# lujiarui/Str2Str

Hardware: AMD Instinct MI355X
Metric: sampled conformations/sec (whole node), 256-res chain, 100 denoise steps (higher is better)
Workload: dtype f32 (matrix products on 2-way f16 split MFMA 'f16x3': 3 products per block, fp32 accumulate, fp32-equivalent); 1 GPU; configs[1]: single 256-residue synthetic chain, 128 replicas per GPU x 100 denoise steps (+1 self-conditioning forward), probability-flow ODE, seeded synthetic weights; n_res=256, replicas_per_gpu=128, denoise_steps=100, parallelism=replica-shard x1, arith=f16x3, rng=device

## Files before the change

### include/str2str_hip.h

```cpp
#ifndef STR2STR_HIP_H
#define STR2STR_HIP_H

#ifdef __cplusplus
extern "C" {
#endif

int s2s_abi_version(void);



int s2s_edge_transition(const float* edge, const float* node_ab, const float* node_p, const float* w1_packed,
                        const float* w2_packed, const float* wf_packed, const float* b2, const float* bf,
                        const float* ln_gamma, const float* ln_beta, const float* mask, float* out, int n_samples,
                        int n_res, float ln_eps, const float* proj_w_packed, const float* proj_bias_cat64,
                        float* proj_attn_bias, float* proj_pair_z, void* stream);

int s2s_edge_transition_f16x3(const float* edge, const float* node_ab, const float* node_p, const void* weight_stream,
                              const float* b2, const float* ln_gamma, const float* ln_beta,
                              const float* mask, float* out, int n_samples, int n_res, float ln_eps, int io_layout,
                              const float* proj_bias_cat64, float* proj_attn_bias, float* proj_pair_z, int prescale_exp,
                              int* range_words, void* stream);

int s2s_edge_embed(const float* node_a, const float* node_b, const float* rel_table, const float* bin_table,
                   const float* bin_lower, const long long* residue_idx, const float* ca_xyz, const float* w2_packed,
                   const float* w3_packed, const float* b2, const float* b3, const float* ln_gamma, const float* ln_beta,
                   const float* mask, float* out, int n_samples, int n_res, int rel_offset, int n_rel, int n_bins,
                   float ln_eps, const float* proj_w_packed, const float* proj_bias_cat64, float* proj_attn_bias,
                   float* proj_pair_z, void* stream);

int s2s_edge_embed_f16x3(const float* node_a, const float* node_b, const float* rel_table, const float* bin_table,
                         const float* bin_lower, const long long* residue_idx, const float* ca_xyz,
                         const void* weight_stream, const float* b2, const float* b3, const float* ln_gamma,
                         const float* ln_beta, const float* mask, float* out, int n_samples, int n_res, int rel_offset,
                         int n_rel, int n_bins, float ln_eps, int out_tiled, const float* proj_bias_cat64,
                         float* proj_attn_bias, float* proj_pair_z, int* range_words, void* stream);

int s2s_pair_project(const float* edge, const float* w_packed, const float* bias_cat64, float* attn_bias, float* pair_z,
                     int n_samples, int n_res, void* stream);


int s2s_ipa_prep_points(const float* rigids7, const float* q_pts_lin, const float* kv_pts_lin, float* q_pts, float* k_pts,
                        float* v_pts, long long n_frames, int n_heads, int n_qk_points, int n_v_points, int v_pts_stride,
                        void* stream);

int s2s_ipa_attention(const float* q, const float* kv, const float* q_pts, const float* k_pts, const float* v_pts64,
                      const float* attn_bias, float* logits_out, float* stats_out, const float* mask, const float* rigids7,
                      const float* head_w_scaled, float* out, int n_samples, int n_res, int n_heads, int c_hidden,
                      int n_qk_points, int n_v_points, int c_pair_z, float inf, float eps, void* stream);

int s2s_ipa_prep_points_f16(const float* rigids7, const float* q_pts_lin, const float* kv_pts_lin, const float* head_w_scaled,
                            void* qp_xp, void* kp_xp, void* vp_vf, float* q2, float* k2, int n_samples, int n_res, int n_heads,
                            int n_qk_points, int n_v_points, int c_hidden, const void* s_xp, void* k_shared, void* v_shared,
                            int* range_words, void* stream);
int s2s_ipa_attention_f16w(const void* q_xp, const void* k_xp, const void* v_vf, const void* qp_xp, const void* kp_xp,
                             const void* vp_vf, const float* q2, const float* k2, const float* attn_bias, float* logits_out,
                             float* stats_out, const float* mask, const float* rigids7, float* out, void* out_xp,
                             int out_xp_ksteps, int n_samples, int n_res, int n_heads, int c_hidden, int n_qk_points,
                             int n_v_points, int c_pair_z, float inf, float eps, int n_kv_heads, void* stream);

int s2s_ipa_opair(const float* logits, const float* stats, const float* pair_z, float* out, int n_samples, int n_res,
                  int n_heads, int c_pair_z, int out_row_stride, int out_col_offset, int logits_ld, void* stream);


int s2s_rigid_compose_update(const float* rigids7, const float* update6, const float* mask, float* out7,
                             long long n_frames, int update_ld, void* stream);

int s2s_torsion_head(const float* u, int u_ld, int normalize, const float* gt_sin_cos, long long gt_row_stride, const float* fixed_mask,
                     float eps, float* out2, long long n_rows, void* stream);

int s2s_rigid_scale_trans(const float* rigids7, float* out7, long long n_frames, float scale, int divide, void* stream);

int s2s_set_backbone_tables(const float* pos_21x5x3, const float* mask_21x5, const int* is_psi_group_21x5,
                            const float* default_frames_21x2x4x4);

int s2s_frames_to_backbone(const float* rigids7, const float* psi_sincos, const long long* aatype, float* atom14_bb5,
                           float* atom37, long long n_frames, void* stream);


int s2s_se3_step(const float* x0_7, const float* xt_7, const float* mask, const float* diffuse_mask,
                 const float* params8, const double* z_rot, const double* z_trans,
                 const double* rot_score_in, const double* trans_score_in, float* next7,
                 double* rot_score_out, double* trans_score_out, int n_samples, int n_res, double dt,
                 const double* dt_per_sample, double coordinate_scaling, int probability_flow, int center_trans,
                 double noise_scale, void* stream);

int s2s_embed_assemble(const float* t_img, long long t_img_rows, const float* node_const, long long node_const_rows, const float* fa, const float* fb,
                       long long n_rows, int n_res, void* h_xp, float* h_f32, float* node_a, float* node_b, int b_col_blocked,
                       int* range_words, void* stream);


int s2s_pack_planes(const float* x, long long n_rows, int ld, int col0, int n_cols, void* xp, int xp_ksteps, int xp_kstep0,
                    const float* row_scale, int* range_words, void* stream);

int s2s_node_linear(const void* xp, const void* w_packed, const float* bias, long long n_rows, int k_in, int n_out,
                    int tiles_per_block, const float* pre_scale, int relu, const float* pre_mask, const float* residual,
                    int residual_ld, const float* ln_gamma, const float* ln_beta, float ln_eps, const float* post_mask,
                    float* out_f32, int out_ld, int out_col0, void* out_xp, int out_xp_ksteps, int out_xp_kstep0,
                    int map_pad, int map_src, int* range_words, void* stream);

int s2s_node_linear_f32(const float* x, int x_ld, const float* w_packed, const float* bias, long long n_rows, int k_in, int n_out,
                        int tiles_per_block, const float* pre_scale, int relu, const float* pre_mask, const float* residual,
                        int residual_ld, const float* ln_gamma, const float* ln_beta, float ln_eps, const float* post_mask,
                        float* out_f32, int out_ld, int out_col0, void* stream);

int s2s_node_linear_vfrag(const void* xp, const void* w_packed, const float* bias, long long n_rows, int k_in, int n_out,
                          int tiles_per_head, void* out_vf, int map_pad, int map_src, int* range_words, void* stream);

typedef struct s2s_node_problem {
    const void* xp; const void* w_packed; const float* bias;
    long long n_rows; int k_in, n_out, tiles_per_block;
    int vfrag_tiles_per_head;
    float* out_f32; int out_ld, out_col0;
    void* out_xp; int out_xp_ksteps, out_xp_kstep0;
    void* out_vf;
    int map_pad, map_src, relu;
    const float* pre_scale;
} s2s_node_problem;
int s2s_node_linear_multi(const s2s_node_problem* problems, int n_problems, int* range_words, void* stream);

typedef struct s2s_chain_layer { const void* w_packed; const float* bias; int relu; } s2s_chain_layer;
int s2s_node_chain(const void* xp, const s2s_chain_layer* layers, int n_layers, long long n_rows, int width, int k_in0,
                   const float* mid_residual, int mid_residual_ld, float* mid_out_f32, int mid_out_ld, const float* mid_ln_gamma,
                   const float* mid_ln_beta, float mid_ln_eps, const float* pre_mask, const float* residual, int residual_ld, const float* ln_gamma, const float* ln_beta, float ln_eps,
                   const float* post_mask, float* out_f32, int out_ld, int out_col0, void* out_xp, int out_xp_ksteps,
                   int out_xp_kstep0, int* range_words, void* stream);

int s2s_row_layernorm(const float* x, int x_ld, long long n_rows, int n_cols, const float* ln_gamma, const float* ln_beta, float ln_eps,
                      const float* post_mask, float* out_f32, int out_ld, int out_col0, void* out_xp, int out_xp_ksteps,
                      int out_xp_kstep0, int* range_words, void* stream);

int s2s_encoder_attention(const float* qkv, const float* key_bias, float* out_f32, void* out_xp, int n_samples, int n_res,
                          int n_heads, int head_dim, int* range_words, void* stream);

int s2s_encoder_attention_f16x3(const float* qkv, const float* key_bias, float* out_f32, void* out_xp, int n_samples, int n_res,
                          int n_heads, int head_dim, int* range_words, void* stream);


int s2s_forward_marginal(const float* rigids0_4x4, const float* z_axis, const float* u01, const float* z_trans,
                         const double* cdf_rows, const int* cdf_row_of_sample, const float* omega_grid, int n_omega,
                         const float* params2, const float* diffuse_mask, float coordinate_scaling, float* rigids_t7,
                         int n_samples, int n_res, void* stream);


int s2s_ca_sample_stats(const float* ca, int n_samples, int n_res, float clash_bar, int k_exclusion, int* n_clash,
                        float* adjacent_max, double* radius_of_gyration, void* stream);

int s2s_ca_pairwise_distances(const float* ca, int n_samples, int n_res, int offset, float* out, void* stream);

int s2s_ca_pwd_js(const float* ref_ca, int n_ref, const float* pred_ca, int n_pred, int n_res, int offset, int n_bins,
                  double pseudo_count, double* js_per_channel, const double* ref_weights, const double* pred_weights, void* stream);


int s2s_ca_rmsd_matrix(const float* a, int n_a, const float* b, int n_b, int n_res, const float* weights, double* rmsd,
                       double* workspace, long long workspace_doubles, void* stream);

int s2s_ca_superpose(const float* mobile, int n_mobile, const float* target, int n_res, const float* weights, double* rmsd,
                     double* xform, void* stream);

int s2s_apply_xform(const float* points, const double* xform, int n_samples, long long n_points, float* out, void* stream);

#define S2S_TM_MAX_RES 800

int s2s_ca_tm_matrix(const float* a, int n_a, const float* b, int n_b, int n_res, double d0, double* tm, void* stream);

int s2s_ca_tm_superpose(const float* mobile, int n_mobile, const float* target, int n_res, double d0, double* tm, double* xform12,
                        void* stream);

#define S2S_LDDT_MAX_RES 1024
#define S2S_LDDT_LIST_SLOTS(n_res) (((long long)(n_res) * ((long long)(n_res) - 1) / 2 + 1) / 2 * 2)
#define S2S_LDDT_WORKSPACE_BYTES(n_a, n_res) ((long long)(n_a) * (12 * S2S_LDDT_LIST_SLOTS(n_res) + 8 + 4 * (long long)(n_res)))

int s2s_ca_lddt_matrix(const float* a, int n_a, const float* b, int n_b, int n_res, double cutoff, int min_seq_sep, double* lddt,
                       void* workspace, long long workspace_bytes, void* stream);

int s2s_ca_lddt_per_residue(const float* model, int n_model, const float* target, int n_res, double cutoff, int min_seq_sep,
                            double* per_res, double* total, void* workspace, long long workspace_bytes, void* stream);

#define S2S_VIOL_MAX_RES 1024

int s2s_backbone_violations(const float* atoms, int n, int n_res, const unsigned char* atom_exists, const int* aatype,
                            const int* residue_index, double tolerance_factor, double clash_tolerance, double* losses, double* fractions,
                            double* per_residue_loss, unsigned char* bond_mask, unsigned char* clash_atom_mask, int* n_clash_pairs,
                            void* stream);

#define S2S_SS_MAX_RES 704

int s2s_secondary_structure(const float* atoms, int n, int n_res, const int* aatype, const int* residue_index, unsigned char* ss,
                            int* n_hbonds, double* hb_energy, int* hb_partner, double* torsions, void* stream);

#define S2S_CLUSTER_MAX_N 65536

int s2s_cluster_adjacency(const double* values, int n_rows, int row0, int n, double cutoff, int at_least, unsigned long long* adj,
                          int* deg, void* stream);

int s2s_cluster_gromos(const unsigned long long* adj, int* deg, int n, int init, int n_rounds, int* labels, int* centres, int* sizes,
                       int* state, unsigned long long* live_ws, unsigned long long* members_ws, void* stream);

#define S2S_CONTACT_MAX_RES 1024
#define S2S_CONTACT_MAX_STRUCTURES 65535
#define S2S_CONTACT_LIST_SLOTS(n_res) ((long long)(n_res) > 1 ? (long long)(n_res) * ((long long)(n_res) - 1) / 2 : 1)

int s2s_ca_contact_map(const float* ca, int n, int n_res, double cutoff, int min_seq_sep, const double* weights, int* counts,
                       double* weighted, void* stream);

int s2s_ca_contact_stats(const float* ca, int n, int n_res, double cutoff, int min_seq_sep, int* n_contacts, long long* sep_sum,
                         void* stream);

int s2s_ca_native_contacts(const float* native, int n_res, double cutoff, int min_seq_sep, int* pairs, double* d0, int* n_pairs,
                           void* stream);

int s2s_ca_native_q(const float* ca, int n, int n_res, const int* pairs, const double* d0, int n_pairs, double beta, double lam,
                    double* q_soft, double* q_hard, int* hits, void* stream);

#define S2S_SASA_MAX_RES 512
#define S2S_SASA_MAX_POINTS 1024

int s2s_backbone_sasa(const float* atoms, int n, int n_res, const unsigned char* atom_exists, const double* radii, double probe,
                      const double* sphere, int n_points, int* counts, double* per_residue, double* total, void* stream);

#define S2S_SAXS_MAX_RES 1024
#define S2S_SAXS_MAX_Q 1024
#define S2S_SAXS_MAX_TYPES 64

int s2s_ca_scattering(const float* ca, int n, int n_res, const double* q, int n_q, const int* types, const double* table, int n_types,
                      double* intensity, double* inv_r_mean, void* stream);

#define S2S_PCA_MAX_RES 1024
#define S2S_PCA_WORKSPACE_DOUBLES(n_res, chunk) ((3ll * (n_res) + 47) / 48 * 48 * (((long long)(chunk) + 3) / 4 * 4))

int s2s_ca_aligned_mean(const float* x, int n, int n_res, const double* xform, const double* p, double* mean, void* stream);

int s2s_ca_covariance(const float* x, int n, int n_res, const double* xform, const double* p, const double* mean, double* cov,
                      double* workspace, long long workspace_doubles, void* stream);

int s2s_ca_project(const float* x, int n, int n_res, const double* xform, const double* mean, const double* components, int n_components,
                   double* proj, void* stream);


long long s2s_format_pdb_models(const float* atom37, int n_models, int n_res, const long long* aatype,
                                const long long* residue_index, const long long* chain_index, const double* b_factors,
                                int first_model_number, int add_end, char* out, long long out_capacity);

long long s2s_write_pdb_models(const char* path, int append, const float* atom37, int n_models, int n_res,
                               const long long* aatype, const long long* residue_index, const long long* chain_index,
                               const double* b_factors, int first_model_number, int add_end);

long long s2s_merge_pdb_files(const char* const* paths, int n_paths, const char* out_path);

int s2s_mt19937_discard(unsigned long long* state624, int* left, unsigned long long* next, unsigned long long n_outputs);

#ifdef __cplusplus
}
#endif
#endif
```

### str2str_amd/build.py

```python
from __future__ import annotations

import os
import shutil
import subprocess
import sys
from concurrent.futures import ThreadPoolExecutor

HERE = os.path.dirname(os.path.abspath(__file__))
ROOT = os.path.dirname(HERE)
CSRC = os.path.join(HERE, "csrc")
OBJ = os.path.join(CSRC, "build")
LIB = os.path.join(HERE, "libstr2str_hip.so")

ARCH = "gfx950"
COMMON = ["-O3", "-std=c++17", "-fPIC", f"--offload-arch={ARCH}", "-I", os.path.join(ROOT, "include"), "-I", CSRC,
          "-Wno-unused-result"]
UNITS = {
    "abi.hip": [],
    "pdb_format.cpp": [],
    "host_rng.cpp": [],
    "rigid_kernels.hip": ["-ffp-contract=off"],
    "se3_step.hip": ["-ffp-contract=off"],
    "forward_marginal.hip": ["-ffp-contract=off"],
    "ensemble_metrics.hip": ["-ffp-contract=off"],
    "ensemble_rmsd.hip": [],
    "ensemble_tm.hip": [],
    "ensemble_pca.hip": [],
    "ensemble_cluster.hip": [],
    "ensemble_lddt.hip": [],
    "ensemble_contacts.hip": ["-ffp-contract=off"],
    "ensemble_violations.hip": ["-ffp-contract=off"],
    "ensemble_ss.hip": ["-ffp-contract=off"],
    "ensemble_sasa.hip": ["-ffp-contract=off"],
    "ensemble_saxs.hip": ["-ffp-contract=off"],
    "pair_mlp.hip": ["-mllvm", "-pragma-unroll-threshold=10000000"],
    "pair_mlp_f16.hip": ["-mllvm", "-pragma-unroll-threshold=10000000", "-fno-slp-vectorize"],
    "pair_mlp_f16_b.hip": ["-mllvm", "-pragma-unroll-threshold=10000000", "-fno-slp-vectorize"],
    "pair_mlp_f16_c.hip": ["-mllvm", "-pragma-unroll-threshold=10000000", "-fno-slp-vectorize"],
    "ipa_attention.hip": ["-mllvm", "-pragma-unroll-threshold=10000000"],
    "ipa_attention_f16w.hip": ["-mllvm", "-pragma-unroll-threshold=10000000", "-fno-slp-vectorize"],
    "node_gemm.hip": ["-mllvm", "-pragma-unroll-threshold=10000000", "-fno-slp-vectorize"],
    "enc_attention.hip": ["-mllvm", "-pragma-unroll-threshold=10000000", "-ffp-contract=off", "-fno-slp-vectorize"],
}


def hipcc() -> str:
    for c in (os.environ.get("HIPCC"), shutil.which("hipcc"), "/opt/rocm/bin/hipcc"):
        if c and os.path.exists(c):
            return c
    raise RuntimeError("hipcc not found (set HIPCC)")


def _stale(out: str, deps) -> bool:
    if not os.path.exists(out):
        return True
    t = os.path.getmtime(out)
    return any(os.path.getmtime(d) > t for d in deps)


def build(force: bool = False, verbose: bool = True) -> str:
    os.makedirs(OBJ, exist_ok=True)
    cc = hipcc()
    headers = [os.path.join(CSRC, f) for f in os.listdir(CSRC) if f.endswith(".h")] + [
        os.path.join(ROOT, "include", "str2str_hip.h"), os.path.abspath(__file__)]

    def compile_one(item):
        src, extra = item
        s = os.path.join(CSRC, src)
        o = os.path.join(OBJ, os.path.splitext(src)[0] + ".o")
        inc = [os.path.join(CSRC, "pair_mlp_f16.hip")] if src.startswith("pair_mlp_f16_") else []
        if force or _stale(o, [s] + inc + headers):
            if src.endswith(".cpp"):
                cmd = [cc, "-x", "c++", "-c", s, "-o", o] + [c for c in COMMON if not c.startswith("--offload-arch")] + extra
            else:
                cmd = [cc, "-x", "hip", "-c", s, "-o", o] + COMMON + extra
            if verbose:
                print(" ".join(cmd), flush=True)
            subprocess.run(cmd, check=True)
        return o

    with ThreadPoolExecutor(max_workers=min(8, len(UNITS))) as ex:
        objs = list(ex.map(compile_one, UNITS.items()))
    for f in os.listdir(OBJ):
        if f.endswith(".o") and os.path.join(OBJ, f) not in objs:
            os.remove(os.path.join(OBJ, f))
    if force or _stale(LIB, objs):
        cmd = [cc, "-shared", "-fPIC", f"--offload-arch={ARCH}", "-o", LIB] + objs
        if verbose:
            print(" ".join(cmd), flush=True)
        subprocess.run(cmd, check=True)
    return LIB


if __name__ == "__main__":
    print(build(force="--force" in sys.argv))
```

### str2str_amd/csrc/pair_mlp_f16.hip

```cpp
#include <hip/hip_runtime.h>

#include <cstdlib>

#include "f16x3.h"
#include "range_flag.h"
#include "str2str_hip.h"

#ifndef S2S_PM_PART
#define S2S_PM_PART 1
#endif

namespace {

constexpr int kStageBytes = 32 * 1024;
constexpr int kStagesBase = 30;

__device__ __forceinline__ float relu1(float x) {
    float r;
    asm("v_max_f32 %0, 0, %1" : "=v"(r) : "v"(x));
    return r;
}

struct SlotDesc { int phase, t, a, b; };
constexpr SlotDesc slot_desc(int s) {
    if (s < 8) return {0, s / 4, s % 4, 0};
    if (s < 168) {
        const int tau = s - 8, blk = tau / 16, o = tau % 16;
        if (o < 12) return {1, blk, o / 6, o % 6};
        return {0, blk + 2, o - 12, 0};
    }
    if (s < 180) return {1, 10, (s - 168) / 6, (s - 168) % 6};
    if (s < 192) return {1, 11, (s - 180) % 2, (s - 180) / 2};

    if (s < 240) return {2, 0, (s - 192) / 2, (s - 192) % 2};
    return {3, 0, s - 240, 0};
}
constexpr int sched_slot(bool proj, int ns) { return !proj ? ns : (ns < 8 ? ns : (ns < 16 ? 240 + (ns - 8) : ns - 8)); }
constexpr int blob_stage(bool proj, int st) { return !proj ? st : (st == 0 ? 0 : (st == 1 ? 30 : st - 1)); }

#define S2S_LDS_BARRIER() asm volatile("s_waitcnt lgkmcnt(0)\n\ts_barrier" ::: "memory")
__device__ float s2s_one[1] = {1.0f};


template <bool PROJ, bool STAGE>
__global__ void __launch_bounds__(256) edge_transition_f16_kernel(
    const float* __restrict__ edge, const float* __restrict__ node_ab, const float* __restrict__ node_p,
    const char* __restrict__ wblob, const float* __restrict__ b2,
    const float* __restrict__ gamma, const float* __restrict__ beta, const float* __restrict__ mask,
    float* __restrict__ out, long long M, int N, float ln_eps, int io_layout, unsigned mask_stride, const float* __restrict__ proj_b,
    float* __restrict__ proj_bias_out, float* __restrict__ proj_pz_out, int* __restrict__ range_flag, float sk) {
    constexpr int kStages = kStagesBase + (PROJ ? 1 : 0);
    constexpr int kSlots = 8 * kStages;
    constexpr int kRing = PROJ ? 4 : 2, kAhead = PROJ ? 2 : 1;
    __shared__ __attribute__((aligned(16))) char s_w[kRing][kStageBytes];
    __shared__ __attribute__((aligned(16))) float s_vec[768 + 64];
    __shared__ __attribute__((aligned(16))) float s_rows[STAGE ? 4 * 2 * 384 : 4];
    const int lane = threadIdx.x & 63, h = lane >> 5, wave = threadIdx.x >> 6;

    const unsigned voff = wave * 8192 + lane * 16;
    typedef __attribute__((address_space(3))) char lds_char;
    lds_char* lds_image[2] = {(lds_char*)&s_w[0][lane * 16], (lds_char*)&s_w[kRing / 2][lane * 16]};
    asm volatile("" : "+v"(lds_image[0]), "+v"(lds_image[1]));
    auto ring_buf = [&](int r) -> lds_char* { return PROJ ? lds_image[r >> 1] + (r & 1) * kStageBytes : lds_image[r]; };
    const __amdgpu_buffer_rsrc_t wrsrc = __builtin_amdgcn_make_buffer_rsrc((void*)wblob, 0, kStages * kStageBytes, 0x00020000);
    auto ldw = [&](unsigned vo, int so) -> f32x4 {
        const u32x4 r = __builtin_amdgcn_raw_buffer_load_b128(wrsrc, vo, so, 0);
        return f32x4{__uint_as_float(r.x), __uint_as_float(r.y), __uint_as_float(r.z), __uint_as_float(r.w)};
    };
    f32x4 c0, c1, c2, c3;
    f32x4 e0, e1, e2, e3;
    typedef __attribute__((address_space(3))) f32x4 lds_f4;
    auto cp_load_a = [&](int stage) {
        const int so = blob_stage(PROJ, stage) * kStageBytes;
        c0 = ldw(voff, so); c1 = ldw(voff + 1024, so); c2 = ldw(voff + 2048, so); c3 = ldw(voff + 3072, so);
    };
    auto cp_load_b = [&](int stage) {
        const int so = blob_stage(PROJ, stage) * kStageBytes + 4096;
        e0 = ldw(voff, so); e1 = ldw(voff + 1024, so); e2 = ldw(voff + 2048, so); e3 = ldw(voff + 3072, so);
    };
    auto cp_store_a = [&](int par) {
        lds_char* d = ring_buf(par) + wave * 8192;
        *(lds_f4*)(d) = c0; *(lds_f4*)(d + 1024) = c1; *(lds_f4*)(d + 2048) = c2; *(lds_f4*)(d + 3072) = c3;
    };
    auto cp_store_b = [&](int par) {
        lds_char* d = ring_buf(par) + (wave * 8192 + 4096);
        *(lds_f4*)(d) = e0; *(lds_f4*)(d + 1024) = e1; *(lds_f4*)(d + 2048) = e2; *(lds_f4*)(d + 3072) = e3;
    };
    auto cp_load_piece = [&](auto grp, auto kc, int stage) {
        constexpr int k = decltype(kc)::value;
        const int so = blob_stage(PROJ, stage) * kStageBytes + (decltype(grp)::value ? 4096 : 0);
        const f32x4 v = ldw(voff + 1024 * k, so);
        if constexpr (decltype(grp)::value == 0) {
            if constexpr (k == 0) c0 = v; else if constexpr (k == 1) c1 = v; else if constexpr (k == 2) c2 = v; else c3 = v;
        } else {
            if constexpr (k == 0) e0 = v; else if constexpr (k == 1) e1 = v; else if constexpr (k == 2) e2 = v; else e3 = v;
        }
    };
    auto cp_store_piece = [&](auto grp, auto kc, int par) {
        constexpr int k = decltype(kc)::value;
        lds_char* d = ring_buf(par) + (wave * 8192 + (decltype(grp)::value ? 4096 : 0) + 1024 * k);
        if constexpr (decltype(grp)::value == 0)
            *(lds_f4*)(d) = k == 0 ? c0 : (k == 1 ? c1 : (k == 2 ? c2 : c3));
        else
            *(lds_f4*)(d) = k == 0 ? e0 : (k == 1 ? e1 : (k == 2 ? e2 : e3));
    };
    cp_load_a(0);
    cp_load_b(0);

    struct PairCtx {
        unsigned p, bi, bj, boff;
        unsigned r0, aoff;
        float em_i, em_j;
        bool valid;
    };
    const unsigned NNu = (unsigned)N * (unsigned)N;
    const long long NN = (long long)N * N;
    const unsigned n_magic = N >= 2 ? (unsigned)((1ull << 32) / (unsigned)N) : 0u;
    auto div_n = [&](unsigned x, unsigned& q, unsigned& r) {
        q = N >= 2 ? __umulhi(x, n_magic) : x;
        r = x - q * (unsigned)N;
        const bool fix = r >= (unsigned)N;
        q = fix ? q + 1 : q;
        r = fix ? r - (unsigned)N : r;
    };
    auto setup = [&](long long wg_tile) -> PairCtx {
        long long pl = (wg_tile * 4 + wave) * 32 + (lane & 31);
        PairCtx c;
        c.valid = pl < M;
        if (!c.valid) pl = M - 1;
        const unsigned p = (unsigned)pl;
        unsigned bi, j, bb, i;
        div_n(p, bi, j);
        div_n(bi, bb, i);
        c.p = p;
        c.bi = bi;
        c.bj = bb * (unsigned)N + j;
        c.r0 = (unsigned)__builtin_amdgcn_readfirstlane((int)bi);
        c.aoff = (unsigned)wave * 3072u + (bi != c.r0 ? 1536u : 0u) + 16u * (unsigned)h;
        c.boff = p + 7u * bb * NNu;
        c.em_i = mask[bi * mask_stride];
        c.em_j = mask[c.bj * mask_stride];
        return c;
    };
    const bool in_tiled = io_layout & 1, out_tiled = io_layout & 2, no_out = io_layout & 4;
    const int in_step = in_tiled ? 256 : 8, out_step = out_tiled ? 256 : 8;
    auto row_of = [&](const float* base, unsigned p, bool tiled) -> const float* {
        const unsigned blk = tiled ? p >> 5 : p, mul = tiled ? 4096u : 128u;
        const unsigned in_blk = tiled ? ((lane & 32) + (p & 31)) * 4 : 4 * h;
        return base + ((unsigned long long)blk * mul + in_blk);
    };
    auto erow_of = [&](const PairCtx& c) -> const float* { return row_of(edge, c.p, in_tiled); };
    auto ldrow = [&](const float* r, int g) -> float4 {
        const f32x4 v = __builtin_nontemporal_load(reinterpret_cast<const f32x4*>(r + g * in_step));
        return make_float4(v.x, v.y, v.z, v.w);
    };
    const long long n_wt = (M + 127) / 128;
    long long wt = blockIdx.x;
    PairCtx cur = setup(wt);

    f16x8 xpl[8][2];
    float amax = 0.f;
    const float inv1 = kInvWS * sk;
    auto split4 = [&](const float (&x)[4], f16x8& ph, f16x8& pm, int at) {
        split4_f16(x, ph, pm, at, amax);
    };
    {
        float4 xv[16];
#pragma unroll
        for (int i = 0; i < 16; ++i) xv[i] = ldrow(erow_of(cur), i);
        for (int i = threadIdx.x; i < 768; i += 256)
            s_vec[i] = i < 384 ? sk * b2[i] : (i < 512 ? 0.f : (i < 640 ? gamma[i - 512] : beta[i - 640]));
        if (PROJ && threadIdx.x < 64) s_vec[768 + threadIdx.x] = proj_b[threadIdx.x];
        cp_store_a(0);
        cp_load_a(1);
        cp_store_b(0);
        if constexpr (kAhead == 2) {
            cp_load_b(1);
            cp_store_a(1);
            cp_load_a(2);
            cp_store_b(1);
        }
#pragma unroll
        for (int i = 0; i < 16; ++i) {
            const float x[4] = {xv[i].x, xv[i].y, xv[i].z, xv[i].w};
            split4(x, xpl[i >> 1][0], xpl[i >> 1][1], 4 * (i & 1));
        }
    }

    f32x16 a1t[2];
    f32x16 a2[12];
    f32x16 a3[4];
    f32x16 pq[2];
    float sa[16];
    f32x4 g_st0, g_st1, g_st2;
    const unsigned n_node_rows = (unsigned)(M / N);
    auto stage_load = [&](const PairCtx& c) {
        if constexpr (STAGE) {
            const unsigned r1 = c.r0 + 1 < n_node_rows ? c.r0 + 1 : c.r0;
            auto piece = [&](int k) -> f32x4 {
                const unsigned o = (unsigned)k * 1024u + 16u * (unsigned)lane;
                const bool second = o >= 1536u;
                const float* src = node_ab + (unsigned long long)(second ? r1 : c.r0) * 896u + ((second ? o - 1536u : o) >> 2);
                const float4 v = *reinterpret_cast<const float4*>(src);
                return f32x4{v.x, v.y, v.z, v.w};
            };
            g_st0 = piece(0); g_st1 = piece(1); g_st2 = piece(2);
        }
    };
    auto stage_store = [&]() {
        if constexpr (STAGE) {
            typedef __attribute__((address_space(3))) f32x4 lds_v4;
            lds_v4* d = (lds_v4*)((__attribute__((address_space(3))) char*)s_rows + wave * 3072 + lane * 16);
            d[0] = g_st0; d[64] = g_st1; d[128] = g_st2;
        }
    };
    auto seeds_piece = [&](const PairCtx& c, int t, int rq) {
        if constexpr (STAGE) {
            const f32x4 x = *(const lds_f4*)((__attribute__((address_space(3))) const char*)s_rows + c.aoff + (32 * t + 8 * rq) * 4);
            sa[4 * rq + 0] = x[0]; sa[4 * rq + 1] = x[1]; sa[4 * rq + 2] = x[2]; sa[4 * rq + 3] = x[3];
        } else {
            const float4 x = ldg4(node_ab + (unsigned long long)c.bi * 896u + 32 * t, rq, h);
            sa[4 * rq + 0] = x.x; sa[4 * rq + 1] = x.y; sa[4 * rq + 2] = x.z; sa[4 * rq + 3] = x.w;
        }
    };
    auto seedc_piece = [&](const PairCtx& c, int t, int rq) {
        const float4 y = ldg4(node_ab + (unsigned long long)c.bj * 896u + 384 + 32 * t, rq, h);
        a1t[t & 1][4 * rq + 0] = y.x; a1t[t & 1][4 * rq + 1] = y.y; a1t[t & 1][4 * rq + 2] = y.z; a1t[t & 1][4 * rq + 3] = y.w;
    };
    auto seeds_load = [&](const PairCtx& c, int t) {
#pragma unroll
        for (int rq = 0; rq < 4; ++rq) seeds_piece(c, t, rq);
    };
    stage_load(cur);
    stage_store();
    seeds_load(cur, 0);
#pragma unroll
    for (int rq = 0; rq < 4; ++rq) { seedc_piece(cur, 0, rq); seedc_piece(cur, 1, rq); }

    f16x8 fr[2][4];
    f16x8 xp[2][2];
    auto fetch = [&](int par, int slot_in_stage, f16x8 (&f)[4]) {
        typedef __attribute__((address_space(3))) f16x8 lds_frag;
        const lds_frag* s = (const lds_frag*)ring_buf(par) + slot_in_stage * 4 * 64;
        f[0] = s[0]; f[2] = s[128]; f[3] = s[192]; f[1] = s[64];
    };
    auto s_quarter = [&](const f32x16& tile_acc, auto qc) {
        constexpr int qd = decltype(qc)::value;
        float x[4];
#pragma unroll
        for (int j = 0; j < 4; ++j) x[j] = fmaxf(__builtin_fmaf(tile_acc[4 * qd + j], inv1, sa[4 * qd + j]), 0.f);
        split4(x, xp[qd >> 1][0], xp[qd >> 1][1], 4 * (qd & 1));
    };
    auto s_half = [&](const f32x16& tile_acc, auto qc, auto hc) {
        constexpr int qd = decltype(qc)::value, j0 = 4 * qd + 2 * decltype(hc)::value;
        const float x0 = fmaxf(__builtin_fmaf(tile_acc[j0], inv1, sa[j0]), 0.f);
        const float x1 = fmaxf(__builtin_fmaf(tile_acc[j0 + 1], inv1, sa[j0 + 1]), 0.f);
        split2_f16(x0, x1, xp[qd >> 1][0], xp[qd >> 1][1], 4 * (qd & 1) + 2 * decltype(hc)::value, amax);
    };
    float rs[64];
    auto row_load2 = [&](const float* r, float (&dst)[64], int g0) {
#pragma unroll
        for (int g = g0; g < g0 + 2; ++g) {
            const float4 v = ldg4(r, g, h);
            dst[4 * g + 0] = v.x; dst[4 * g + 1] = v.y; dst[4 * g + 2] = v.z; dst[4 * g + 3] = v.w;
        }
    };
    const f32x16 zero16 = {0.f, 0.f, 0.f, 0.f, 0.f, 0.f, 0.f, 0.f, 0.f, 0.f, 0.f, 0.f, 0.f, 0.f, 0.f, 0.f};
    S2S_LDS_BARRIER();
    fetch(0, 0, fr[0]);

    PairCtx prv = cur;
    prv.valid = false;
    prv.em_i = 0.f;
    float ln_sum = 0.f, ln_var = 0.f, ln_mean = 0.f, ln_rstd = 0.f, ln_em = 0.f;
    float* ln_orow = out;
    f16x8 xln[8][2];
    auto ln_add = [&](auto qc) {
        constexpr int q = decltype(qc)::value, t = q / 4, rq = q % 4;
#pragma unroll
        for (int j = 0; j < 4; ++j) ln_sum += a3[t][4 * rq + j];
    };
    auto ln_dev = [&](auto qc) {
        constexpr int q = decltype(qc)::value, t = q / 4, rq = q % 4;
#pragma unroll
        for (int j = 0; j < 4; ++j) {
            const float dd = a3[t][4 * rq + j] - ln_mean;
            ln_var += dd * dd;
        }
    };
    auto ln_out = [&](auto qc, const float4& ga, const float4& be) {
        constexpr int q = decltype(qc)::value, t = q / 4, rq = q % 4;
        float4 o;
        o.x = ((a3[t][4 * rq + 0] - ln_mean) * ln_rstd * ga.x + be.x) * ln_em;
        o.y = ((a3[t][4 * rq + 1] - ln_mean) * ln_rstd * ga.y + be.y) * ln_em;
        o.z = ((a3[t][4 * rq + 2] - ln_mean) * ln_rstd * ga.z + be.z) * ln_em;
        o.w = ((a3[t][4 * rq + 3] - ln_mean) * ln_rstd * ga.w + be.w) * ln_em;
        if (prv.valid && !no_out) {
            __builtin_nontemporal_store(f32x4{o.x, o.y, o.z, o.w}, reinterpret_cast<f32x4*>(ln_orow + q * out_step));
        }
        if constexpr (PROJ) {
            const float x[4] = {o.x, o.y, o.z, o.w};
            split4(x, xln[2 * t + (rq >> 1)][0], xln[2 * t + (rq >> 1)][1], 4 * (rq & 1));
        }
    };
    auto proj_store = [&](auto gc) {
        constexpr int g = decltype(gc)::value;
        if (prv.valid) {
            const float4 bq = ldg4(s_vec + 768, g, h);
            if constexpr (g == 0) {
                float* o = proj_bias_out + ((unsigned long long)prv.boff + 4 * h * NN);
                o[0] = __builtin_fmaf(pq[0][0], kInvWS, bq.x);
                o[NN] = __builtin_fmaf(pq[0][1], kInvWS, bq.y);
                o[2 * NN] = __builtin_fmaf(pq[0][2], kInvWS, bq.z);
                o[3 * NN] = __builtin_fmaf(pq[0][3], kInvWS, bq.w);
            } else {
                constexpr int t = g >> 2, rq = g & 3;
                *reinterpret_cast<float4*>(proj_pz_out + (unsigned long long)prv.p * 32u + 8 * (g - 1) + 4 * h) =
                    make_float4(__builtin_fmaf(pq[t][4 * rq + 0], kInvWS, bq.x), __builtin_fmaf(pq[t][4 * rq + 1], kInvWS, bq.y),
                                __builtin_fmaf(pq[t][4 * rq + 2], kInvWS, bq.z), __builtin_fmaf(pq[t][4 * rq + 3], kInvWS, bq.w));
            }
        }
    };
#pragma unroll
    for (int t = 0; t < 4; ++t) a3[t] = zero16;

    constexpr int kHead = PROJ ? 16 : 15;
    long long wt_next = wt;
    bool has_next = false;
    PairCtx nxt = cur;
    float4 xv[16];
    f16x8 xpn[8][2];
    f16x8 xq[8][2];
    auto slot = [&](auto sc) {
        constexpr int ns = decltype(sc)::value;
        constexpr int s = sched_slot(PROJ, ns);
        constexpr SlotDesc d = slot_desc(s);
        constexpr int stage = ns / 8, ss = ns % 8, par = stage & (kRing - 1);
        constexpr int st_next = (stage + 1) % kStages, st_fill = (stage + kAhead) % kStages;
#ifdef S2S_ET_ALL_BARRIERS
        constexpr bool barrier_here = true;
#else
        constexpr bool barrier_here = !PROJ || (st_next & 1) == 0 || st_next == kStages - 2;
#endif

        if constexpr (ss < 7) {
            fetch(par, ss + 1, fr[(ns + 1) & 1]);
        } else {
            if constexpr (barrier_here) S2S_LDS_BARRIER();
            fetch(st_next & (kRing - 1), 0, fr[(ns + 1) & 1]);
        }
        constexpr int kXv0 = 208;
        if constexpr (s == kXv0) nxt = setup(has_next ? wt_next : wt);
        if constexpr (s == kXv0 + 3) stage_load(nxt);
        if constexpr (s == kXv0 + 8) stage_store();
        if constexpr (s > kXv0 && s <= kXv0 + 16 && ((s & 3) == 1 || (s & 3) == 2)) {
            constexpr int i = 4 * ((s - kXv0) / 4) + 2 * ((s & 3) - 1);
            const float* er = erow_of(nxt);
            xv[i] = ldrow(er, i);
            xv[i + 1] = ldrow(er, i + 1);
        }
        if constexpr (s == 236) seeds_load(nxt, 0);
        if constexpr (s == 237) { seedc_piece(nxt, 0, 0); seedc_piece(nxt, 0, 1); seedc_piece(nxt, 0, 2); seedc_piece(nxt, 0, 3); }
        if constexpr (s == 238) { seedc_piece(nxt, 1, 0); seedc_piece(nxt, 1, 1); seedc_piece(nxt, 1, 2); seedc_piece(nxt, 1, 3); }
        constexpr bool seeds_slot = d.phase == 1 && d.a == 1 && d.b == 0 && d.t + 1 < 12;
        if constexpr (s >= 184 && s < 192) row_load2(node_p + (unsigned long long)cur.bi * 128u, rs, 2 * (s - 184));
        constexpr int ep_blk = (s >= 184 && s < 192) ? 0 : ((s >= 192 && s < 224) ? 1 + (s - 192) / 16 : -1);
        constexpr int ep_q = ep_blk == 0 ? 2 * (s - 184) : (s - 192) % 16;
        float4 ep_b = {0.f, 0.f, 0.f, 0.f}, ep_b1 = {0.f, 0.f, 0.f, 0.f};
        if constexpr (ep_blk >= 0) ep_b = ldg4(s_vec + 128 * ep_blk, ep_q, h);
        if constexpr (ep_blk == 0) ep_b1 = ldg4(s_vec, ep_q + 1, h);
        constexpr int ln_k = ns == 7 ? 0 : ((PROJ && d.phase == 3 && d.a < 7) ? d.a + 1 : ((!PROJ && ns >= 8 && ns < 15) ? ns - 7 : -1));
        float4 lnv[4] = {};
        if constexpr (ln_k >= 0) {
#pragma unroll
            for (int k = 0; k < 2; ++k) { lnv[2 * k] = ldg4(s_vec + 512, 2 * ln_k + k, h); lnv[2 * k + 1] = ldg4(s_vec + 640, 2 * ln_k + k, h); }
        }
        constexpr int kGSlot = 182, kGPer = 2;
        if constexpr (s >= kGSlot && s < kGSlot + 16 / kGPer) {
#pragma unroll
            for (int u = 0; u < kGPer; ++u) {
                constexpr int p0 = (s - kGSlot) * kGPer;
                const int t3 = (p0 + u) / 4, rq = (p0 + u) % 4;
                const float4 v = ldg4(node_ab + (unsigned long long)cur.bj * 896u + 768 + 32 * t3, rq, h);
                a3[t3][4 * rq + 0] = v.x; a3[t3][4 * rq + 1] = v.y; a3[t3][4 * rq + 2] = v.z; a3[t3][4 * rq + 3] = v.w;
            }
        }
        __builtin_amdgcn_sched_barrier(0);

        const f16x8 (&f)[4] = fr[ns & 1];
        auto mfma_i = [&](auto ic) {
            constexpr int i = decltype(ic)::value;
            if constexpr (d.phase == 0) {
                f32x16& acc = a1t[d.t & 1];
                const f16x8 (&x)[2] = xpl[2 * d.a + (i >= 3)];
                constexpr int fa = (i == 0 ? 1 : (i < 3 ? 0 : (i == 3 ? 3 : 2))), xa = (i == 1 || i == 4) ? 1 : 0;
                acc = mfma_f16(f[fa], x[xa], acc);
            } else {
                constexpr bool fin = d.phase == 2, prj = d.phase == 3;
                constexpr bool first = i < 2 && (prj ? d.a == 0 : (fin ? false : (d.t == 0 && d.a == 0)));
                f32x16& t = prj ? pq[i & 1] : (fin ? a3[2 * d.b + (i & 1)] : a2[2 * d.b + (i & 1)]);
                const f16x8 (&x)[2] = prj ? xln[d.a] : (fin ? ((d.a >> 3) == 1 ? xq[d.a & 7] : xpl[d.a & 7]) : xp[d.a]);
                constexpr int fa = 2 * (i & 1) + (i < 2 ? 1 : 0), xa = (i == 2 || i == 3) ? 1 : 0;
                if constexpr (first) t = mfma_f16(f[fa], x[xa], zero16); else t = mfma_f16(f[fa], x[xa], t);
            }
        };
        auto ep_half = [&](auto qc, auto hc, const float4& bq) {
            constexpr int q = decltype(qc)::value, hh = decltype(hc)::value, t = q / 4, rq = q % 4, j0 = 4 * rq + 2 * hh, e0 = 4 * (rq & 1) + 2 * hh;
            const f32x16& a = a2[4 * (ep_blk < 0 ? 0 : ep_blk) + t];
            f16x8 (&P)[2] = ep_blk == 1 ? xq[2 * t + (rq >> 1)] : xpl[2 * t + (rq >> 1)];
            float r0 = 0.f, r1 = 0.f;
            if constexpr (ep_blk == 0) {
                const unsigned hw = __builtin_bit_cast(u32x4, P[0])[e0 / 2], lw = __builtin_bit_cast(u32x4, P[1])[e0 / 2];
                asm("v_fma_mix_f32 %0, %1, 1.0, %2 op_sel_hi:[1,0,1]" : "=v"(r0) : "v"(hw), "v"(lw));
                asm("v_fma_mix_f32 %0, %1, 1.0, %2 op_sel:[1,0,1] op_sel_hi:[1,0,1]" : "=v"(r1) : "v"(hw), "v"(lw));
            } else if constexpr (ep_blk == 1) {
                r0 = rs[16 * t + j0];
                r1 = rs[16 * t + j0 + 1];
            }
            float x0 = fmaxf(__builtin_fmaf(a[j0], kInvWS, hh ? bq.z : bq.x), 0.f), x1 = fmaxf(__builtin_fmaf(a[j0 + 1], kInvWS, hh ? bq.w : bq.y), 0.f);
            if constexpr (ep_blk != 2) {
                x0 = __builtin_fmaf(r0, sk, x0);
                x1 = __builtin_fmaf(r1, sk, x1);
            }
            split2_f16(x0, x1, P[0], P[1], e0, amax);
        };
        static_for<0, 6>([&](auto ic) {
            constexpr int i = decltype(ic)::value;
            mfma_i(ic);
            if constexpr (i < 4) {
                if constexpr (ss == 0) cp_load_piece(IC<1>{}, ic, st_fill);
                if constexpr (ss == 4) cp_load_piece(IC<0>{}, ic, (stage + kAhead + 1) % kStages);
                if constexpr (ss == 1) cp_store_piece(IC<0>{}, IC<3 - i>{}, st_fill & (kRing - 1));
                if constexpr (ss == 5) cp_store_piece(IC<1>{}, IC<3 - i>{}, st_fill & (kRing - 1));
            }
            if constexpr (seeds_slot && i < 4) seeds_piece(cur, d.t + 1, i);
            if constexpr (seeds_slot && i < 4 && d.t + 2 < 12) seedc_piece(cur, d.t + 2, i);
            if constexpr (d.phase == 0 && d.t >= 1 && (i == 2 || i == 4)) s_half(a1t[(d.t - 1) & 1], IC<d.a>{}, IC<(i - 2) / 2>{});
            if constexpr (ep_blk > 0 && (i == 2 || i == 4)) ep_half(IC<ep_q>{}, IC<(i - 2) / 2>{}, ep_b);
            if constexpr (ep_blk == 0 && i >= 1 && i <= 4) {
                if constexpr (i <= 2) ep_half(IC<ep_q>{}, IC<i - 1>{}, ep_b); else ep_half(IC<ep_q + 1>{}, IC<i - 3>{}, ep_b1);
            }
            if constexpr (s >= 228 && s < 236 && i >= 1 && i <= 4) {
                constexpr int k = s - 228, e = 2 * (i - 1);
                const float4 v = xv[2 * k + (e >> 2)];
                if constexpr ((e & 2) == 0) split2_f16(v.x, v.y, xpn[k][0], xpn[k][1], e, amax);
                else split2_f16(v.z, v.w, xpn[k][0], xpn[k][1], e, amax);
            }
            if constexpr (ns < 4 && i < 4) ln_add(IC<4 * ns + i>{});
            if constexpr (ns == 4 && i == 0) ln_mean = xhalf_sum(ln_sum) * (1.0f / 128);
            if constexpr ((ns == 4 || ns == 5) && (i == 1 || i == 3 || i == 5)) { ln_dev(IC<6 * (ns - 4) + i - 1>{}); ln_dev(IC<6 * (ns - 4) + i>{}); }
            if constexpr (ns == 6 && (i == 0 || i == 1)) { ln_dev(IC<12 + 2 * i>{}); ln_dev(IC<12 + 2 * i + 1>{}); }
            if constexpr (ns == 6 && i == 3) {
                ln_rstd = 1.0f / sqrtf(xhalf_sum(ln_var) * (1.0f / 128) + ln_eps * ((kWS * sk) * (kWS * sk)));
                ln_em = prv.em_i * prv.em_j;
                ln_orow = const_cast<float*>(row_of(out, prv.p, out_tiled));
                ln_sum = 0.f;
                ln_var = 0.f;
            }
            if constexpr (ln_k >= 0 && (i == 1 || i == 3)) ln_out(IC<2 * ln_k + (i - 1) / 2>{}, lnv[i - 1], lnv[i]);
            if constexpr (PROJ && ns == kHead && i < 5) proj_store(ic);
            __builtin_amdgcn_sched_barrier(0);
        });

        if constexpr (s == 179) {
            s_quarter(a1t[1], IC<0>{}); s_quarter(a1t[1], IC<1>{}); s_quarter(a1t[1], IC<2>{}); s_quarter(a1t[1], IC<3>{});
        }
    };
    for (;;) {
    wt_next = wt + gridDim.x;
    has_next = wt_next < n_wt;
    static_for<0, kSlots>(slot);

    prv = cur;
#pragma unroll
    for (int i = 0; i < 8; ++i) { xpl[i][0] = xpn[i][0]; xpl[i][1] = xpn[i][1]; }
    if (!has_next) break;
    cur = nxt;
    wt = wt_next;
    }
    static_for<0, kHead>(slot);
    if constexpr (PROJ) { proj_store(IC<0>{}); proj_store(IC<1>{}); proj_store(IC<2>{}); proj_store(IC<3>{}); proj_store(IC<4>{}); }
    s2s::range_report(range_flag, amax, s2s::kRangeEdgeTransition);
}


template <bool PROJ>
__global__ void __launch_bounds__(256) edge_embed_f16_kernel(
    const float* __restrict__ node_a, const float* __restrict__ node_b, const float* __restrict__ rel_tab,
    const float* __restrict__ bin_tab, const float* __restrict__ bin_lower, const long long* __restrict__ residue_idx,
    const float* __restrict__ ca, const char* __restrict__ wblob, const float* __restrict__ b2, const float* __restrict__ b3,
    const float* __restrict__ gamma, const float* __restrict__ beta, const float* __restrict__ mask, float* __restrict__ out,
    long long M, int N, int rel_off, int n_rel, int n_bins, float ln_eps, int out_tiled, const float* __restrict__ proj_b,
    float* __restrict__ proj_bias_out, float* __restrict__ proj_pz_out, int* __restrict__ range_flag) {
    constexpr int kStages = PROJ ? 5 : 4;
    constexpr int kSlots = 8 * kStages;
    __shared__ __attribute__((aligned(16))) char s_w[2][kStageBytes];
    __shared__ __attribute__((aligned(16))) float s_vec[512 + 64];
    __shared__ __attribute__((aligned(16))) float s_bins[64 + 4];
    const int lane = threadIdx.x & 63, h = lane >> 5, wave = threadIdx.x >> 6;

    const unsigned voff = wave * 8192 + lane * 16;
    typedef __attribute__((address_space(3))) char lds_char;
    lds_char* lds_image[2] = {(lds_char*)&s_w[0][lane * 16], (lds_char*)&s_w[1][lane * 16]};
    asm volatile("" : "+v"(lds_image[0]), "+v"(lds_image[1]));
    const __amdgpu_buffer_rsrc_t wrsrc = __builtin_amdgcn_make_buffer_rsrc((void*)wblob, 0, kStages * kStageBytes, 0x00020000);
    auto ldw = [&](unsigned vo, int so) -> f32x4 {
        const u32x4 r = __builtin_amdgcn_raw_buffer_load_b128(wrsrc, vo, so, 0);
        return f32x4{__uint_as_float(r.x), __uint_as_float(r.y), __uint_as_float(r.z), __uint_as_float(r.w)};
    };
    f32x4 c0, c1, c2, c3, e0, e1, e2, e3;
    typedef __attribute__((address_space(3))) f32x4 lds_f4;
    auto cp_load_a = [&](int stage) {
        const int so = stage * kStageBytes;
        c0 = ldw(voff, so); c1 = ldw(voff + 1024, so); c2 = ldw(voff + 2048, so); c3 = ldw(voff + 3072, so);
    };
    auto cp_load_b = [&](int stage) {
        const int so = stage * kStageBytes + 4096;
        e0 = ldw(voff, so); e1 = ldw(voff + 1024, so); e2 = ldw(voff + 2048, so); e3 = ldw(voff + 3072, so);
    };
    auto cp_store_a = [&](int par) {
        lds_char* d = lds_image[par] + wave * 8192;
        *(lds_f4*)(d + 3072) = c3; *(lds_f4*)(d + 2048) = c2; *(lds_f4*)(d + 1024) = c1; *(lds_f4*)(d) = c0;
    };
    auto cp_store_b = [&](int par) {
        lds_char* d = lds_image[par] + (wave * 8192 + 4096);
        *(lds_f4*)(d + 3072) = e3; *(lds_f4*)(d + 2048) = e2; *(lds_f4*)(d + 1024) = e1; *(lds_f4*)(d) = e0;
    };
    cp_load_a(0);
    cp_load_b(0);

    struct Ctx {
        const float* ra;
        unsigned vb, vr, vk;
        float kb;
        long long p, boff;
        float em;
        bool valid;
    };
    const long long NN = (long long)N * N;
    const __amdgpu_buffer_rsrc_t rs_b = __builtin_amdgcn_make_buffer_rsrc((void*)node_b, 0, (unsigned)(M / N * 512), 0x00020000);
    const __amdgpu_buffer_rsrc_t rs_r = __builtin_amdgcn_make_buffer_rsrc((void*)rel_tab, 0, n_rel * 512, 0x00020000);
    const __amdgpu_buffer_rsrc_t rs_k = __builtin_amdgcn_make_buffer_rsrc((void*)bin_tab, 0, n_bins * 512, 0x00020000);
    struct Raw {
        long long p, bi, bj, bb;
        float ax, ay, az, bx, by, bz;
        long long ii, ij;
        float mi, mj;
        bool valid;
    };
    const unsigned n_magic = N >= 2 ? (unsigned)((1ull << 32) / (unsigned)N) : 0u;
    auto div_n = [&](unsigned x, unsigned& q, unsigned& r) {
        q = N >= 2 ? __umulhi(x, n_magic) : x;
        r = x - q * (unsigned)N;
        const bool fix = r >= (unsigned)N;
        q = fix ? q + 1 : q;
        r = fix ? r - (unsigned)N : r;
    };
    const float* mask_or_any = mask ? mask : ca;
    auto setup_a = [&](long long wg_tile) -> Raw {
        long long p = (wg_tile * 4 + wave) * 32 + (lane & 31);
        Raw r;
        r.valid = p < M;
        p = r.valid ? p : M - 1;
        r.p = p;
        unsigned bi, j, bb, i;
        div_n((unsigned)p, bi, j);
        div_n(bi, bb, i);
        r.bi = bi; r.bb = bb; r.bj = bb * (unsigned)N + j;
        r.ax = ca[r.bi * 3 + 0]; r.ay = ca[r.bi * 3 + 1]; r.az = ca[r.bi * 3 + 2];
        r.bx = ca[r.bj * 3 + 0]; r.by = ca[r.bj * 3 + 1]; r.bz = ca[r.bj * 3 + 2];
        r.ii = residue_idx[r.bi];
        r.ij = residue_idx[r.bj];
        r.mi = mask_or_any[r.bi];
        r.mj = mask_or_any[r.bj];
        return r;
    };
    auto setup_b = [&](const Raw& r) -> Ctx {
        Ctx c;
        c.valid = r.valid;
        const float dx = r.ax - r.bx, dy = r.ay - r.by, dz = r.az - r.bz;
        const float dist = sqrtf(__fadd_rn(__fadd_rn(__fmul_rn(dx, dx), __fmul_rn(dy, dy)), __fmul_rn(dz, dz)));
        int cnt = 0;
#pragma unroll
        for (int u = 0; u < 8; ++u) {
            const float4 e = *reinterpret_cast<const float4*>(&s_bins[4 * u]);
            cnt += (e.x < dist) + (e.y < dist) + (e.z < dist) + (e.w < dist);
        }
        cnt = cnt > n_bins ? n_bins : cnt;
        const float up = s_bins[cnt];
        const int bin = (cnt >= 1 && dist < up) ? cnt - 1 : -1;
        long long d = r.ii - r.ij + rel_off;
        d = d < 0 ? 0 : (d >= n_rel ? n_rel - 1 : d);
        c.ra = node_a + r.bi * 128;
        const unsigned jj = (unsigned)(r.bj - r.bb * N);
        c.vb = ((unsigned)r.bb * 32u * (unsigned)N + (unsigned)h * (unsigned)N + jj) * 16u;
        c.vr = ((unsigned)h * (unsigned)n_rel + (unsigned)d) * 16u;
        c.vk = ((unsigned)h * (unsigned)n_bins + (unsigned)(bin < 0 ? 0 : bin)) * 16u;
        c.kb = bin < 0 ? 0.f : 1.f;
        c.p = r.p;
        c.boff = r.p + 7 * r.bb * NN;
        c.em = mask ? r.mi * r.mj : 1.0f;
        return c;
    };
    float amax = 0.f;
    auto split4 = [&](const float (&x)[4], f16x8& ph, f16x8& pm, int at) {
        split4_f16(x, ph, pm, at, amax);
    };
    float g1[64];
    auto row_set = [&](const float* r) {
#pragma unroll
        for (int G = 0; G < 16; ++G) {
            const float4 v = ldg4(r, G, h);
            g1[4 * G + 0] = v.x; g1[4 * G + 1] = v.y; g1[4 * G + 2] = v.z; g1[4 * G + 3] = v.w;
        }
    };
    float tmp[64];
    auto row_cb = [&](const __amdgpu_buffer_rsrc_t& rs, unsigned vo, int rows, float (&dst)[64], int G0, int G1) {
#pragma unroll
        for (int G = G0; G < G1; ++G) {
            const u32x4 v = __builtin_amdgcn_raw_buffer_load_b128(rs, vo, G * 32 * rows, 0);
            dst[4 * G + 0] = __uint_as_float(v.x); dst[4 * G + 1] = __uint_as_float(v.y);
            dst[4 * G + 2] = __uint_as_float(v.z); dst[4 * G + 3] = __uint_as_float(v.w);
        }
    };
    auto row_add = [&](float scale) {
#pragma unroll
        for (int i = 63; i >= 0; --i) {
            g1[i] = __fmaf_rn(scale, tmp[i], g1[i]);
            asm volatile("" : "+v"(g1[i]));
        }
    };
    auto g1_split = [&](f16x8 (&dst)[2], int ks) {
        const float x0[4] = {relu1(g1[8 * ks + 0]), relu1(g1[8 * ks + 1]), relu1(g1[8 * ks + 2]), relu1(g1[8 * ks + 3])};
        const float x1[4] = {relu1(g1[8 * ks + 4]), relu1(g1[8 * ks + 5]), relu1(g1[8 * ks + 6]), relu1(g1[8 * ks + 7])};
        split4(x0, dst[0], dst[1], 0);
        split4(x1, dst[0], dst[1], 4);
    };

    const long long n_wt = (M + 127) / 128;
    long long wt = blockIdx.x;
    if (threadIdx.x < 68) s_bins[threadIdx.x] = (int)threadIdx.x < n_bins ? bin_lower[threadIdx.x] : ((int)threadIdx.x == n_bins ? 1e8f : 3.0e38f);
    __syncthreads();
    Ctx cur = setup_b(setup_a(wt));
    f16x8 xp[8][2];
    {
        row_set(cur.ra);
        for (int i = threadIdx.x; i < 512; i += 256)
            s_vec[i] = i < 128 ? kWS * b2[i] : (i < 256 ? kWS * b3[i - 128] : (i < 384 ? gamma[i - 256] : beta[i - 384]));
        if (PROJ && threadIdx.x < 64) s_vec[512 + threadIdx.x] = proj_b[threadIdx.x];
        cp_store_a(0);
        cp_load_a(1);
        cp_store_b(0);
        row_cb(rs_b, cur.vb, N, tmp, 0, 16); row_add(1.0f);
        row_cb(rs_r, cur.vr, n_rel, tmp, 0, 16); row_add(1.0f);
        row_cb(rs_k, cur.vk, n_bins, tmp, 0, 16); row_add(cur.kb);
#pragma unroll
        for (int ks = 0; ks < 8; ++ks) g1_split(xp[ks], ks);
    }
    f32x16 a2[4], a3[4], pq[2];
    f16x8 fr[2][4];
    auto fetch = [&](int par, int slot_in_stage, f16x8 (&f)[4]) {
        typedef __attribute__((address_space(3))) f16x8 lds_frag;
        const lds_frag* s = (const lds_frag*)lds_image[par] + slot_in_stage * 4 * 64;
        f[0] = s[0]; f[2] = s[128]; f[3] = s[192]; f[1] = s[64];
    };
    const f32x16 zero16 = {0.f, 0.f, 0.f, 0.f, 0.f, 0.f, 0.f, 0.f, 0.f, 0.f, 0.f, 0.f, 0.f, 0.f, 0.f, 0.f};
    auto pin_frag = [&](f16x8 (&x)[2]) { asm volatile("" : "+v"(x[0]), "+v"(x[1])); };
    auto bias16 = [&](const float* vec, int t) -> f32x16 {
        const float4 b0 = ldg4(vec, 4 * t, h), b1 = ldg4(vec, 4 * t + 1, h), b2v = ldg4(vec, 4 * t + 2, h), b3v = ldg4(vec, 4 * t + 3, h);
        return f32x16{b0.x, b0.y, b0.z, b0.w, b1.x, b1.y, b1.z, b1.w, b2v.x, b2v.y, b2v.z, b2v.w, b3v.x, b3v.y, b3v.z, b3v.w};
    };
    auto l2_piece = [&](auto kc) {
        constexpr int k = decltype(kc)::value, t = k / 2;
#pragma unroll
        for (int u = 0; u < 2; ++u) {
            const int rq = 2 * (k & 1) + u;
            const float xx[4] = {relu1(a2[t][4 * rq + 0]) * kInvWS, relu1(a2[t][4 * rq + 1]) * kInvWS,
                                 relu1(a2[t][4 * rq + 2]) * kInvWS, relu1(a2[t][4 * rq + 3]) * kInvWS};
            split4(xx, xp[k][0], xp[k][1], 4 * u);
        }
        pin_frag(xp[k]);
    };
    float ln_mean = 0.f, ln_rstd = 0.f;
    const unsigned out_lane = out_tiled ? lane * 16u : (unsigned)((lane & 31) * 512 + h * 16), out_step = out_tiled ? 1024u : 32u;
    f16x8 xq[2][2];
    __amdgpu_buffer_rsrc_t rs_out;
    auto out_rsrc = [&](long long wg_tile) {
        const long long p0 = (wg_tile * 4 + __builtin_amdgcn_readfirstlane(wave)) * 32;
        const long long left = M - p0;
        rs_out = __builtin_amdgcn_make_buffer_rsrc((void*)(out + (p0 < M ? p0 : 0) * 128), 0,
                                                   (unsigned)(left <= 0 ? 0 : (left < 32 && !out_tiled ? left : 32)) * 512u, 0x00020000);
    };
    float4 lga[2], lbe[2];
    auto ln_load = [&](auto kc) {
        constexpr int k = decltype(kc)::value;
#pragma unroll
        for (int u = 0; u < 2; ++u) {
            const int g = 4 * (k / 2) + 2 * (k & 1) + u;
            lga[u] = ldg4(s_vec + 256, g, h);
            lbe[u] = ldg4(s_vec + 384, g, h);
        }
    };
    auto ln_piece = [&](auto kc, const Ctx& c) {
        constexpr int k = decltype(kc)::value, t = k / 2;
#pragma unroll
        for (int u = 0; u < 2; ++u) {
            const int rq = 2 * (k & 1) + u, g = 4 * t + rq;
            const float4 ga = lga[u], be = lbe[u];
            float4 o;
            o.x = __fmul_rn(__fmaf_rn(__fmul_rn(a3[t][4 * rq + 0] - ln_mean, ln_rstd), ga.x, be.x), c.em);
            o.y = __fmul_rn(__fmaf_rn(__fmul_rn(a3[t][4 * rq + 1] - ln_mean, ln_rstd), ga.y, be.y), c.em);
            o.z = __fmul_rn(__fmaf_rn(__fmul_rn(a3[t][4 * rq + 2] - ln_mean, ln_rstd), ga.z, be.z), c.em);
            o.w = __fmul_rn(__fmaf_rn(__fmul_rn(a3[t][4 * rq + 3] - ln_mean, ln_rstd), ga.w, be.w), c.em);
            __builtin_amdgcn_raw_buffer_store_b128(u32x4{__float_as_uint(o.x), __float_as_uint(o.y), __float_as_uint(o.z), __float_as_uint(o.w)},
                                                   rs_out, out_lane + (unsigned)g * out_step, 0, 0);
            if constexpr (PROJ) {
                const float xx[4] = {o.x, o.y, o.z, o.w};
                split4(xx, xq[k & 1][0], xq[k & 1][1], 4 * u);
            }
        }
        if constexpr (PROJ) pin_frag(xq[k & 1]);
    };
    auto row_load8 = [&](const float* r, float (&dst)[64], int half) {
#pragma unroll
        for (int G = 8 * half; G < 8 * half + 8; ++G) {
            const float4 v = ldg4(r, G, h);
            dst[4 * G + 0] = v.x; dst[4 * G + 1] = v.y; dst[4 * G + 2] = v.z; dst[4 * G + 3] = v.w;
        }
    };
    S2S_LDS_BARRIER();
    fetch(0, 0, fr[0]);
    f32x16 initA0 = bias16(s_vec, 0), initA1 = bias16(s_vec, 1), initB0, initB1;
    Raw nraw = setup_a(wt + gridDim.x < n_wt ? wt + gridDim.x : wt);

    for (;;) {
    const long long wt_next = wt + gridDim.x;
    const bool has_next = wt_next < n_wt;
    Ctx nxt = cur;
    f16x8 xl[2];
    static_for<0, kSlots>([&](auto sc) {
        constexpr int s = decltype(sc)::value;
        constexpr int stage = s / 8, ss = s % 8, par = stage & 1;
        constexpr int layer = s / 16;
        constexpr int ks = layer < 2 ? (s % 16) / 2 : s - 32;
        constexpr int pr = layer < 2 ? s % 2 : 0;
        if constexpr (s == kSlots - 1) { initA0 = bias16(s_vec, 0); initA1 = bias16(s_vec, 1); }
        if constexpr (s == 0) { initB0 = bias16(s_vec, 2); initB1 = bias16(s_vec, 3); }
        if constexpr (s == 15) { initA0 = bias16(s_vec + 128, 0); initA1 = bias16(s_vec + 128, 1); }
        if constexpr (s == 16) { initB0 = bias16(s_vec + 128, 2); initB1 = bias16(s_vec + 128, 3); }
        if constexpr (PROJ && s >= 31 && s < 39) ln_load(IC<s - 31>{});
        if constexpr (ss < 7) {
            fetch(par, ss + 1, fr[(s + 1) & 1]);
        } else {
            S2S_LDS_BARRIER();
            fetch(par ^ 1, 0, fr[(s + 1) & 1]);
        }
        if constexpr (s == 30) out_rsrc(wt);
        if constexpr (s == 5) row_load8(nxt.ra, g1, 0);
        if constexpr (s == 6) row_load8(nxt.ra, g1, 1);
        if constexpr (s == 7) row_cb(rs_b, nxt.vb, N, tmp, 0, 8);
        if constexpr (s == 8) row_cb(rs_b, nxt.vb, N, tmp, 8, 16);
        if constexpr (s == 13) row_cb(rs_r, nxt.vr, n_rel, tmp, 0, 8);
        if constexpr (s == 14) row_cb(rs_r, nxt.vr, n_rel, tmp, 8, 16);
        if constexpr (s == 18) row_cb(rs_k, nxt.vk, n_bins, tmp, 0, 8);
        if constexpr (s == 19) row_cb(rs_k, nxt.vk, n_bins, tmp, 8, 16);
        __builtin_amdgcn_sched_barrier(0);

        const f16x8 (&f)[4] = fr[s & 1];
        const f16x8 (&x)[2] = layer < 2 ? xp[ks] : xq[ks & 1];
        f32x16& t0 = layer == 0 ? a2[2 * pr] : (layer == 1 ? a3[2 * pr] : pq[0]);
        f32x16& t1 = layer == 0 ? a2[2 * pr + 1] : (layer == 1 ? a3[2 * pr + 1] : pq[1]);
        if constexpr (ks == 0) {
            if constexpr (layer < 2) {
                t0 = mfma_f16(f[1], x[0], pr == 0 ? initA0 : initB0); t1 = mfma_f16(f[3], x[0], pr == 0 ? initA1 : initB1);
            } else {
                t0 = mfma_f16(f[1], x[0], zero16); t1 = mfma_f16(f[3], x[0], zero16);
            }
        } else {
            t0 = mfma_f16(f[1], x[0], t0); t1 = mfma_f16(f[3], x[0], t1);
        }
        t0 = mfma_f16(f[0], x[1], t0); t1 = mfma_f16(f[2], x[1], t1);
        t0 = mfma_f16(f[0], x[0], t0); t1 = mfma_f16(f[2], x[0], t1);
        if constexpr (s == 1) nxt = setup_b(nraw);
        if constexpr (s == 26) nraw = setup_a(wt_next + gridDim.x < n_wt ? wt_next + gridDim.x : wt_next);
        if constexpr (s == 12) row_add(1.0f);
        if constexpr (s == 17) row_add(1.0f);
        if constexpr (s == 22) row_add(nxt.kb);
        if constexpr (s >= 16 && s <= 28 && s % 2 == 0) l2_piece(IC<(s - 14) / 2>{});
        if constexpr (s == 15) l2_piece(IC<0>{});
        if constexpr (s >= 24 && s < 31) { g1_split(xp[s - 24], s - 24); pin_frag(xp[s - 24]); }
        if constexpr (s == 23) { g1_split(xl, 7); pin_frag(xl); }
        if constexpr (PROJ && s >= 32 && s < 39) ln_piece(IC<s - 31>{}, cur);
        if constexpr (ss == 0) cp_load_b((stage + 1) % kStages);
        if constexpr (ss == 4) cp_load_a((stage + 2) % kStages);
        if constexpr (ss == 1) cp_store_a(par ^ 1);
        if constexpr (ss == 5) cp_store_b(par ^ 1);
        constexpr int copy_kind = (ss == 0 || ss == 4) ? 0x020 : ((ss == 1 || ss == 5) ? 0x200 : 0);
#pragma unroll
        for (int i = 0; i < 6; ++i) {
            __builtin_amdgcn_sched_group_barrier(0x008, 1, 0);
            if (copy_kind != 0 && i < 4) __builtin_amdgcn_sched_group_barrier(copy_kind, 1, 0);
            __builtin_amdgcn_sched_group_barrier(0x002, 8, 0);
        }
        __builtin_amdgcn_sched_barrier(0);

        if constexpr (s == 31) {
            float sum = 0.f;
#pragma unroll
            for (int t = 0; t < 4; ++t)
#pragma unroll
                for (int r = 0; r < 16; ++r) sum += a3[t][r];
            ln_mean = __fmul_rn(xhalf_sum(sum), 1.0f / 128);
            float var = 0.f;
#pragma unroll
            for (int t = 0; t < 4; ++t)
#pragma unroll
                for (int r = 0; r < 16; ++r) {
                    const float dd = a3[t][r] - ln_mean;
                    var = __fmaf_rn(dd, dd, var);
                }
            ln_rstd = 1.0f / sqrtf(__fmaf_rn(xhalf_sum(var), 1.0f / 128, ln_eps * (kWS * kWS)));
            if constexpr (PROJ) {
                ln_piece(IC<0>{}, cur);
            } else {
                static_for<0, 8>([&](auto kc) { ln_load(kc); ln_piece(kc, cur); });
            }
        }
    });
    if constexpr (PROJ) {
        if (cur.valid) {
            const float4 b0 = ldg4(s_vec + 512, 0, h);
            float* o = proj_bias_out + cur.boff + 4 * h * NN;
            o[0] = __builtin_fmaf(pq[0][0], kInvWS, b0.x);
            o[NN] = __builtin_fmaf(pq[0][1], kInvWS, b0.y);
            o[2 * NN] = __builtin_fmaf(pq[0][2], kInvWS, b0.z);
            o[3 * NN] = __builtin_fmaf(pq[0][3], kInvWS, b0.w);
#pragma unroll
            for (int g = 1; g <= 4; ++g) {
                const int t = g >> 2, rq = g & 3;
                const float4 bq = ldg4(s_vec + 512, g, h);
                *reinterpret_cast<float4*>(proj_pz_out + cur.p * 32 + 8 * (g - 1) + 4 * h) =
                    make_float4(__builtin_fmaf(pq[t][4 * rq + 0], kInvWS, bq.x), __builtin_fmaf(pq[t][4 * rq + 1], kInvWS, bq.y),
                                __builtin_fmaf(pq[t][4 * rq + 2], kInvWS, bq.z), __builtin_fmaf(pq[t][4 * rq + 3], kInvWS, bq.w));
            }
        }
    }
    if (!has_next) break;
    cur = nxt;
    wt = wt_next;
    xp[7][0] = xl[0]; xp[7][1] = xl[1];
    if constexpr (kStages % 2 == 1) {
        lds_char* sw = lds_image[0];
        lds_image[0] = lds_image[1];
        lds_image[1] = sw;
    }
    }
    s2s::range_report(range_flag, amax, s2s::kRangeEdgeEmbed);
}


long long tile_aligned_samples(long long NN) {
    long long q = 32;
    while (q > 1 && (NN * (32 / q)) % 32 != 0) q /= 2;
    return 32 / q;
}

int cu_count() {
    int dev = 0, n_cu = 0;
    if (hipGetDevice(&dev) != hipSuccess || hipDeviceGetAttribute(&n_cu, hipDeviceAttributeMultiprocessorCount, dev) != hipSuccess || n_cu <= 0)
        return 256;
    return n_cu;
}

template <bool STAGE>
int et_launch(const float* edge, const float* node_ab, const float* node_p, const void* weight_stream, const float* b2,
              const float* ln_gamma, const float* ln_beta, const float* mask, float* out, int n_samples, int n_res, float ln_eps,
              int io_layout, const float* proj_bias_cat64, float* proj_attn_bias, float* proj_pair_z, int prescale_exp, int* range_words,
              void* stream) {
    if (n_samples <= 0 || n_res <= 0) return 0;
    if ((io_layout & ~7) || ((io_layout & 4) && !proj_attn_bias) || (!(io_layout & 4) && !out)) return (int)hipErrorInvalidValue;
    if (prescale_exp < 0 || prescale_exp > 15) return (int)hipErrorInvalidValue;
    const float sk = ldexpf(1.0f, -prescale_exp);
    const long long NN = (long long)n_res * n_res;
    const char* cap_env = getenv("S2S_ET_MAX_PAIRS");
    long long cap = cap_env ? atoll(cap_env) : 0;
    if (cap <= 0 || cap > (1ll << 29) - 1) cap = (1ll << 29) - 1;
    long long chunk = cap / NN;
    if ((io_layout & 3) && chunk < n_samples) chunk -= chunk % tile_aligned_samples(NN);
    if (chunk < 1) return (int)hipErrorInvalidValue;
    const float* one = nullptr;
    if (hipGetSymbolAddress((void**)&one, HIP_SYMBOL(s2s_one)) != hipSuccess) return (int)hipErrorInvalidValue;
    const int n_cu = cu_count();
    for (long long b0 = 0; b0 < n_samples; b0 += chunk) {
        const long long nb = n_samples - b0 < chunk ? n_samples - b0 : chunk;
        const long long M = nb * NN, rows0 = b0 * n_res;
        const long long wg_tiles = (M + 127) / 128;
        const long long grid = wg_tiles < n_cu ? wg_tiles : n_cu;
        const float* e = edge + b0 * NN * 128;
        const float* nab = node_ab + rows0 * 896;
        const float* np = node_p + rows0 * 128;
        const float* mk = mask ? mask + rows0 : one;
        const unsigned mks = mask ? 1u : 0u;
        float* o = out ? out + b0 * NN * 128 : nullptr;
        auto k_proj = &edge_transition_f16_kernel<true, STAGE>;
        auto k_plain = &edge_transition_f16_kernel<false, STAGE>;
        if (proj_attn_bias)
            hipLaunchKernelGGL(k_proj, dim3((unsigned)grid), dim3(256), 0, (hipStream_t)stream, e, nab, np,
                               (const char*)weight_stream, b2, ln_gamma, ln_beta, mk, o, M, n_res, ln_eps, io_layout, mks, proj_bias_cat64,
                               proj_attn_bias + b0 * 8 * NN, proj_pair_z + b0 * NN * 32, range_words, sk);
        else
            hipLaunchKernelGGL(k_plain, dim3((unsigned)grid), dim3(256), 0, (hipStream_t)stream, e, nab, np,
                               (const char*)weight_stream, b2, ln_gamma, ln_beta, mk, o, M, n_res, ln_eps, io_layout, mks,
                               (const float*)nullptr, (float*)nullptr, (float*)nullptr, range_words, sk);
    }
    return (int)hipGetLastError();
}

}

#define S2S_ET_ARGS const float* edge, const float* node_ab, const float* node_p, const void* weight_stream, const float* b2, \
                    const float* ln_gamma, const float* ln_beta, const float* mask, float* out, int n_samples, int n_res, float ln_eps, \
                    int io_layout, const float* proj_bias_cat64, float* proj_attn_bias, float* proj_pair_z, int prescale_exp, \
                    int* range_words, void* stream
#define S2S_ET_PASS edge, node_ab, node_p, weight_stream, b2, ln_gamma, ln_beta, mask, out, n_samples, n_res, ln_eps, io_layout, \
                    proj_bias_cat64, proj_attn_bias, proj_pair_z, prescale_exp, range_words, stream
extern "C" __attribute__((visibility("hidden"))) int s2s_et_f16x3_short_chains(S2S_ET_ARGS);
#if S2S_PM_PART == 2
extern "C" int s2s_et_f16x3_short_chains(S2S_ET_ARGS) { return et_launch<false>(S2S_ET_PASS); }
#endif
#if S2S_PM_PART == 1
extern "C" int s2s_edge_transition_f16x3(S2S_ET_ARGS) {
    return n_res >= 32 ? et_launch<true>(S2S_ET_PASS) : s2s_et_f16x3_short_chains(S2S_ET_PASS);
}
#endif

#if S2S_PM_PART == 3
extern "C" int s2s_edge_embed_f16x3(const float* node_a, const float* node_b, const float* rel_table, const float* bin_table,
                                     const float* bin_lower, const long long* residue_idx, const float* ca_xyz,
                                     const void* weight_stream, const float* b2, const float* b3, const float* ln_gamma,
                                     const float* ln_beta, const float* mask, float* out, int n_samples, int n_res,
                                     int rel_offset, int n_rel, int n_bins, float ln_eps, int out_tiled, const float* proj_bias_cat64,
                                     float* proj_attn_bias, float* proj_pair_z, int* range_words, void* stream) {
    if (n_samples <= 0 || n_res <= 0) return 0;
    if (n_bins > 32 || (out_tiled & ~1)) return (int)hipErrorInvalidValue;
    const long long NN = (long long)n_res * n_res;
    if (NN >= (1ll << 31) || (long long)n_rel * 512 >= (1ll << 32)) return (int)hipErrorInvalidValue;
    const char* cap_env = getenv("S2S_EE_MAX_PAIRS");
    long long cap = cap_env ? atoll(cap_env) : 0;
    if (cap <= 0 || cap > (1ll << 31) - 1) cap = (1ll << 31) - 1;
    long long chunk = cap / NN;
    const long long rows_cap = ((1ll << 32) - 1) / ((long long)n_res * 512);
    if (rows_cap < chunk) chunk = rows_cap;
    if (out_tiled && chunk < n_samples) chunk -= chunk % tile_aligned_samples(NN);
    if (chunk < 1) return (int)hipErrorInvalidValue;
    const int n_cu = cu_count();
    for (long long b0 = 0; b0 < n_samples; b0 += chunk) {
        const long long nb = n_samples - b0 < chunk ? n_samples - b0 : chunk;
        const long long M = nb * NN, rows0 = b0 * n_res;
        const long long wg_tiles = (M + 127) / 128;
        const long long grid = wg_tiles < n_cu ? wg_tiles : n_cu;
        const float* na = node_a + rows0 * 128;
        const float* nbp = node_b + rows0 * 128;
        const long long* ridx = residue_idx + rows0;
        const float* cap = ca_xyz + rows0 * 3;
        const float* mk = mask ? mask + rows0 : nullptr;
        float* o = out + b0 * NN * 128;
        if (proj_attn_bias)
            hipLaunchKernelGGL(edge_embed_f16_kernel<true>, dim3((unsigned)grid), dim3(256), 0, (hipStream_t)stream, na, nbp,
                               rel_table, bin_table, bin_lower, ridx, cap, (const char*)weight_stream, b2, b3, ln_gamma, ln_beta,
                               mk, o, M, n_res, rel_offset, n_rel, n_bins, ln_eps, out_tiled, proj_bias_cat64,
                               proj_attn_bias + b0 * 8 * NN, proj_pair_z + b0 * NN * 32, range_words);
        else
            hipLaunchKernelGGL(edge_embed_f16_kernel<false>, dim3((unsigned)grid), dim3(256), 0, (hipStream_t)stream, na, nbp,
                               rel_table, bin_table, bin_lower, ridx, cap, (const char*)weight_stream, b2, b3, ln_gamma, ln_beta,
                               mk, o, M, n_res, rel_offset, n_rel, n_bins, ln_eps, out_tiled, (const float*)nullptr, (float*)nullptr,
                               (float*)nullptr, range_words);
    }
    return (int)hipGetLastError();
}
#endif
```

### str2str_amd/models/net/denoising_ipa.py

```python
from __future__ import annotations

import math
from functools import partial
from typing import Optional

import torch
import torch.nn.functional as F
from torch import nn

from ... import ops
from ...arith import default_arith
from ...common.all_atom import compute_backbone
from ...common.rigid_utils import Rigid
from .ipa import TranslationIPA
from .layers import DerivedCache, centred


def get_positional_embedding(indices: torch.Tensor, embedding_dim: int, max_len: int = 2056) -> torch.Tensor:
    K = torch.arange(embedding_dim // 2, device=indices.device)
    arg = indices[..., None] * math.pi / (max_len ** (2 * K[None] / embedding_dim))
    return torch.cat([torch.sin(arg), torch.cos(arg)], dim=-1)


def get_timestep_embedding(timesteps: torch.Tensor, embedding_dim: int, max_len: int = 10000) -> torch.Tensor:
    assert timesteps.ndim == 1
    timesteps = timesteps * max_len
    half = embedding_dim // 2
    freq = torch.exp(torch.arange(half, dtype=torch.float, device=timesteps.device) * -(math.log(max_len) / (half - 1)))
    emb = timesteps.float()[:, None] * freq[None, :]
    emb = torch.cat([torch.sin(emb), torch.cos(emb)], dim=1)
    if embedding_dim % 2 == 1:
        emb = F.pad(emb, (0, 1), mode="constant")
    return emb


class EmbeddingModule(nn.Module):
    launch_switches = ("arith", "node_arith")

    def __init__(self, init_embed_size: int, node_embed_size: int, edge_embed_size: int, num_bins: int = 22,
                 min_bin: float = 1e-5, max_bin: float = 20.0, self_conditioning: bool = True):
        super().__init__()
        pos_embed_size = t_embed_size = init_embed_size
        node_in = t_embed_size + 1 + pos_embed_size
        edge_in = (t_embed_size + 1) * 2 + pos_embed_size
        self.node_embed = nn.Sequential(
            nn.Linear(node_in, node_embed_size), nn.ReLU(), nn.Linear(node_embed_size, node_embed_size), nn.ReLU(),
            nn.Linear(node_embed_size, node_embed_size), nn.LayerNorm(node_embed_size),
        )
        self.self_conditioning = self_conditioning
        if self_conditioning:
            edge_in += num_bins
        self.edge_embed = nn.Sequential(
            nn.Linear(edge_in, edge_embed_size), nn.ReLU(), nn.Linear(edge_embed_size, edge_embed_size), nn.ReLU(),
            nn.Linear(edge_embed_size, edge_embed_size), nn.LayerNorm(edge_embed_size),
        )
        self.time_embed = partial(get_timestep_embedding, embedding_dim=t_embed_size)
        self.position_embed = partial(get_positional_embedding, embedding_dim=pos_embed_size)
        self._dims = (init_embed_size, num_bins, float(min_bin), float(max_bin), edge_embed_size)
        self._wcache, self._w16cache, self._proj_cache, self._idx_cache, self._fixed_cache = (DerivedCache() for _ in range(5))
        self.arith = default_arith()
        self.node_arith = default_arith()

    def _weights(self):
        e0, e2, e4 = self.edge_embed[0], self.edge_embed[2], self.edge_embed[4]
        ie, nb = self._dims[0], self._dims[1]
        t1 = ie + 1

        def build():
            w0 = e0.weight.float()
            n0 = self.node_embed[0]
            wn = n0.weight.float()
            out = {
                "w_row_t": w0[:, :ie].contiguous(), "w_row_f": w0[:, ie].contiguous(),
                "w_col_t": w0[:, t1:t1 + ie].contiguous(), "w_col_f": w0[:, t1 + ie].contiguous(),
                "w_rel": w0[:, 2 * t1:2 * t1 + ie].contiguous(), "b0": e0.bias.float().contiguous(),
                "wn_t": wn[:, :ie].contiguous(), "wn_f": wn[:, ie].contiguous(), "wn_pos": wn[:, t1:t1 + ie].contiguous(),
                "bn0": n0.bias.float().contiguous(),
                "w_t_cat": torch.cat([wn[:, :ie], w0[:, :ie], w0[:, t1:t1 + ie]], dim=0).contiguous(),
                "b_t_cat": torch.cat([n0.bias.float(), e0.bias.float(), torch.zeros_like(e0.bias.float())]).contiguous(),
                "w3c": centred(e4.weight), "b3c": centred(e4.bias),
                "w2p": ops.pack_weight(e2.weight.float()), "w3p": ops.pack_weight(centred(e4.weight)),
                "node_mlp": [ops.pack_node_layer(self.node_embed[2].weight, self.node_embed[2].bias),
                             ops.pack_node_layer(self.node_embed[4].weight, self.node_embed[4].bias, True)],
            }
            if self.self_conditioning:
                out["bin_tab"] = w0[:, 2 * t1 + ie:2 * t1 + ie + nb].t().contiguous()
            else:
                out["bin_tab"] = w0.new_zeros(1, w0.shape[0])
            out["bin_tab_cb"] = ops.column_blocked(out["bin_tab"])
            out["bin_lower"] = torch.linspace(self._dims[2], self._dims[3], nb).to(w0.device)
            return out

        ne = self.node_embed
        return self._wcache.get([e0.weight, e0.bias, e2.weight, e4.weight, e4.bias, ne[0].weight, ne[0].bias, ne[2].weight, ne[2].bias,
                                 ne[4].weight, ne[4].bias], build)

    def _fixed_terms(self, fixed_mask: torch.Tensor, w: dict, dev, node_pos: torch.Tensor):
        def build():
            fixed = fixed_mask.to(dev)[..., None].float()
            B, L = fixed.shape[:2]
            return ((fixed * w["wn_f"] + node_pos).contiguous(), (fixed * w["w_row_f"]).contiguous(),
                    ((fixed[:, None] * w["w_col_f"].view(1, 32, 1, 4)).expand(B, 32, L, 4).contiguous(), (fixed * w["w_col_f"]).contiguous()))

        return self._fixed_cache.get([fixed_mask, w["wn_f"], node_pos], build)

    def time_images(self, t_emb: torch.Tensor) -> torch.Tensor:
        w = self._weights()
        t_emb = t_emb.to(w["b0"].device).reshape(-1, t_emb.shape[-1]).float()
        return ((w["w_t_cat"][None] * t_emb[:, None, :]).sum(-1) + w["b_t_cat"]).contiguous()

    def _index_tables(self, residue_idx: torch.Tensor, w_rel: torch.Tensor, wn_pos: torch.Tensor):
        return self._tables(residue_idx, w_rel, wn_pos)[:4]

    def _tables(self, residue_idx, w_rel, wn_pos):
        def build():
            idx_cpu = residue_idx.detach().cpu()
            span = int(idx_cpu.max() - idx_cpu.min())
            d = torch.arange(-span, span + 1)
            dev = w_rel.device
            rel = _table_linear(self.position_embed(d).float().to(dev), w_rel)
            node_pos = _table_linear(self.position_embed(idx_cpu).float().to(dev), wn_pos)
            return rel, span, node_pos, residue_idx.to(dev).contiguous(), ops.column_blocked(rel)

        return self._idx_cache.get([residue_idx, w_rel, wn_pos], build)

    def forward(self, *args, **kw):
        node_embed, _, edge_embed, proj = self.embed(*args, **kw)
        return (node_embed, edge_embed) if proj is None else (node_embed, edge_embed, proj)

    def embed(self, residue_idx, t, fixed_mask, self_conditioning_ca, node_mask: Optional[torch.Tensor] = None,
              next_proj=None, t_emb: Optional[torch.Tensor] = None, edge_layout: str = "rowmajor", t_img: Optional[torch.Tensor] = None):
        w = self._weights()
        dev = w["b0"].device
        if dev.type != "cuda":
            raise ops.HipLibraryError("EmbeddingModule runs on the HIP device only (no CPU fallback)")
        if self._dims[4] != 128:
            raise ops.HipLibraryError("edge_embed kernel is built for edge_embed_size=128")
        B, L = residue_idx.shape
        rel_tab, span, node_pos, idx_dev, rel_cb = self._tables(residue_idx, w["w_rel"], w["wn_pos"])
        if t_img is not None:
            t_emb = None
        elif t_emb is not None:
            t_emb = t_emb.to(dev).reshape(-1, t_emb.shape[-1])
        else:
            t_u, t_inv = torch.unique(t.detach().reshape(-1), return_inverse=True)
            t_emb = self.time_embed(t_u)[t_inv].to(dev)
        ne = self.node_embed
        mask = None if node_mask is None else node_mask.to(dev).float().contiguous()
        nn_, ne_ = w["wn_t"].shape[0], w["w_row_t"].shape[0]
        single_t = t_img is not None or t_emb.shape[0] == 1
        M = B * L
        f16 = self.arith == "f16x3"
        if single_t:
            per_sample = t_img is not None and t_img.ndim == 2 and t_img.shape[0] == B and B > 1
            img = (t_img if per_sample else t_img.reshape(-1)) if t_img is not None else (w["w_t_cat"] * t_emb).sum(-1) + w["b_t_cat"]
            Fn, Fa, Fb = self._fixed_terms(fixed_mask, w, dev, node_pos)
            h_act, node_a, node_b = torch.ops.str2str_amd.embed_assemble(img.contiguous(), Fn, Fa, Fb[0] if f16 else Fb[1], B, L,
                                                                         self.node_arith == "f16x3", f16)
        else:
            fixed = fixed_mask.to(dev)[..., None].float()
            tl = lambda wt, b=None: _table_linear(t_emb, wt, b)
            h = F.relu(tl(w["wn_t"], w["bn0"])[:, None, :] + fixed * w["wn_f"] + node_pos)
            h_act = ops.to_act(h.reshape(M, -1).contiguous(), self.node_arith)
        nw = w["node_mlp"]
        node_embed, node_act = ops.node_apply_chain(h_act, nw, M, (True, False), ln=(ne[5].weight, ne[5].bias, ne[5].eps),
                                                          post_mask=None if mask is None else mask.reshape(M), want_xp=True)
        node_embed = node_embed.view(B, L, -1)
        if not single_t:
            node_a = (tl(w["w_row_t"], w["b0"])[:, None, :] + fixed * w["w_row_f"]).expand(B, L, -1).contiguous()
            if f16:
                node_b = (tl(w["w_col_t"]).view(-1, 32, 1, 4) + fixed[:, None] * w["w_col_f"].view(1, 32, 1, 4)).expand(B, 32, L, 4).contiguous()
            else:
                node_b = (tl(w["w_col_t"])[:, None, :] + fixed * w["w_col_f"]).expand(B, L, -1).contiguous()
        ca = self_conditioning_ca.to(dev).float().contiguous() if self.self_conditioning else node_a.new_zeros(B, L, 3)
        e2, e4, ln = self.edge_embed[2], self.edge_embed[4], self.edge_embed[5]
        if f16:
            e2w = e2.weight
            ws = self._w16cache.get([e2w, w["w3c"]], lambda: ops.pack_f16x3_embed_stream(e2w.float(), w["w3c"]))
            proj = None
            if next_proj is not None:
                stream = self._proj_cache.get([ws, next_proj["wp_f16x2"]], lambda: torch.cat([ws, next_proj["wp_f16x2"]]))
                proj = (stream, next_proj["b64"])
            edge_embed = ops.edge_embed_f16x3(node_a, node_b, rel_cb, w["bin_tab_cb"], w["bin_lower"], idx_dev, ca, ws, e2.bias,
                                              w["b3c"], ln.weight, ln.bias, mask, span, ln.eps, proj=proj, column_blocked_tables=True,
                                              out_layout=edge_layout)
        else:
            if edge_layout != "rowmajor":
                raise ops.HipLibraryError("EmbeddingModule: the tiled pair layout belongs to the f16x3 kernels")
            edge_embed = ops.edge_embed(node_a, node_b, rel_tab, w["bin_tab"], w["bin_lower"], idx_dev, ca, w["w2p"],
                                        w["w3p"], e2.bias, w["b3c"], ln.weight, ln.bias, mask, span, ln.eps,
                                        proj=None if next_proj is None else (next_proj["wp"], next_proj["b64"]))
        if next_proj is not None:
            edge_embed, *proj = edge_embed
            return node_embed, node_act, edge_embed, tuple(proj)
        return node_embed, node_act, edge_embed, None


def _table_linear(x: torch.Tensor, w: torch.Tensor, b: Optional[torch.Tensor] = None) -> torch.Tensor:
    layer = ops.pack_node_layer(w, b if b is not None else torch.zeros(w.shape[0], device=w.device))
    lead, n = x.shape[:-1], x.numel() // x.shape[-1]
    y, _ = ops.node_apply(x.reshape(n, x.shape[-1]).float().contiguous(), layer, n)
    return y[:, : w.shape[0]].reshape(*lead, w.shape[0]).contiguous()


class DenoisingNet(nn.Module):
    def __init__(self, embedder: nn.Module, translator: nn.Module):
        super().__init__()
        self.embedder = embedder
        self.translator = translator
        self.backbone_in_forward = True

    @staticmethod
    def blend_psi(psi: torch.Tensor, torsion_angles_sin_cos: torch.Tensor, fixed_mask: torch.Tensor) -> torch.Tensor:
        gt_psi = torsion_angles_sin_cos.to(psi.device)[..., 2, :]
        fixed_mask = fixed_mask.to(psi.device).type(torch.float)
        return gt_psi * fixed_mask[..., None] + psi * (1 - fixed_mask[..., None])

    def forward(self, batch: dict, as_tensor_7: bool = False, defer_psi_blend: bool = False) -> dict:
        dev = next(self.parameters()).device
        if dev.type != "cuda":
            raise ops.HipLibraryError(
                "DenoisingNet.forward needs the HIP device (MI355X): the sampling path has no CPU fallback")
        node_mask = batch["residue_mask"].to(dev).type(torch.float)
        fixed_mask = batch["fixed_mask"].to(dev).type(torch.float)
        fuse = getattr(self.translator, "fuse_pair_projection", False)
        et0 = self.translator.trunk["edge_transition_0"] if "edge_transition_0" in getattr(self.translator, "trunk", {}) else None
        tiled = fuse and getattr(self.embedder, "arith", None) == "f16x3" and getattr(et0, "arith", None) == "f16x3"
        node_embed, node_act, edge_embed, first_proj = self.embedder.embed(
            residue_idx=batch["residue_idx"], t=batch["t"], fixed_mask=fixed_mask, self_conditioning_ca=batch["sc_ca_t"], node_mask=node_mask,
            t_emb=batch.get("t_emb"), t_img=batch.get("t_img"), next_proj=self.translator.trunk["ipa_0"].pair_proj_weights() if fuse else None,
            **({"edge_layout": "tiled"} if tiled else {}))
        tb = dict(batch)
        tb["residue_mask"], tb["fixed_mask"] = node_mask, fixed_mask
        tb["rigids_t"] = batch["rigids_t"].to(dev)
        tb["_node_embed_act"] = node_act
        model_out = self.translator(node_embed, edge_embed, tb, **({"_first_proj": first_proj} if fuse else {}))
        if model_out.get("psi_blended") or defer_psi_blend:
            psi_pred = model_out["psi"]
        else:
            psi_pred = self.blend_psi(model_out["psi"], batch["torsion_angles_sin_cos"], fixed_mask)
        rigids_pred = model_out["out_rigids"]
        out = {"rigids": rigids_pred, "psi": psi_pred, "rigids7": model_out["out_rigids7"]}
        if defer_psi_blend and not model_out.get("psi_blended"):
            out["psi_deferred"] = True
        if self.backbone_in_forward:
            aatype = batch["aatype"].to(dev) if "aatype" in batch else None
            bb = compute_backbone(rigids_pred, psi_pred, aatype=aatype, _rigids7=model_out["out_rigids7"])
            out["atom37"], out["atom14"] = bb[0], bb[-1]
        if as_tensor_7:
            out["rigids"] = model_out["out_rigids7"]
        return out
```

### str2str_amd/ops/__init__.py

```python
from .attention import encoder_attention, ipa_attention, ipa_attention_f16, ipa_prep_points, ipa_prep_points_f16
from .binding import ABI_VERSION, EXPORTS, LIB_PATH, HipLibraryError, KernelTimer, WeightRangeError, load_library
from .ensemble import (CLUSTER_MAX_N, CONTACT_MAX_RES, LDDT_MAX_RES, PCA_MAX_RES, RMSD_LAUNCH_PAIRS, SASA_MAX_POINTS, SASA_MAX_RES, SAXS_MAX_Q, SAXS_MAX_RES,
                       SAXS_MAX_TYPES, SS_MAX_RES, TM_MAX_RES, VIOL_MAX_RES, apply_xform, backbone_sasa, backbone_violations, ca_aligned_mean, ca_contact_map, ca_covariance, ca_fit_transforms, ca_project, ca_contact_stats, ca_lddt_matrix, ca_native_contacts, ca_native_q, ca_lddt_per_residue, ca_pairwise_distances, ca_pwd_js, ca_rmsd_matrix,
                       ca_sample_stats, ca_scattering, ca_superpose, ca_tm_matrix, ca_tm_superpose, cluster_adjacency, cluster_gromos,
                       lddt_workspace_bytes, rmsd_row_chunk, secondary_structure, sphere_points)
from .geometry import forward_marginal, frames_to_backbone, rigid_compose_update, rigid_scale_trans, se3_step, torsion_head
from .hostio import (float64_normal_outputs, format_pdb_models, host_rng_can_discard, host_rng_discard_float64_normals,
                     host_rng_fast_forward_ok, merge_pdb_files, write_pdb_models)
from .node import (CHAIN_WIDTHS, NARROW_MAX_WORK, SMALL_ROWS, embed_assemble, ipa_projections, node_apply,
                   node_apply_chain, node_apply_multi, node_chain, node_linear, node_linear_f32, node_linear_multi, node_linear_vfrag,
                   pack_planes, row_layernorm, small_rows_variant, to_act)
from .packing import (NODE_TG, LazyDict, PairTiled, act_alloc, column_blocked, fragment_order, node_tiles, pack_f16x2_layer, pack_f16x3_embed_stream,
                      pack_f16x3_stream, pack_node_layer, pack_node_weight, pack_node_weight_f32, pack_weight, padded_len, pair_tiled,
                      pair_untiled, unpack_planes, vf_alloc, xp_alloc)
from .pair import edge_embed, edge_embed_f16x3, edge_transition, edge_transition_f16x3, pair_project
from .range_guard import (RANGE_BITS, RANGE_FAMILIES, range_families, range_flag, range_flag_names, range_flag_read, range_flag_reset,
                          range_headroom)
from .torch_ops import register_torch_ops

__all__ = [
    "ABI_VERSION", "EXPORTS", "LIB_PATH", "HipLibraryError", "KernelTimer", "WeightRangeError", "load_library",
    "RANGE_BITS", "RANGE_FAMILIES", "range_families", "range_flag", "range_flag_names", "range_flag_read", "range_flag_reset", "range_headroom",
    "NODE_TG", "LazyDict", "PairTiled", "act_alloc", "column_blocked", "fragment_order", "node_tiles", "pack_f16x2_layer", "pack_f16x3_embed_stream",
    "pack_f16x3_stream", "pack_node_layer", "pack_node_weight", "pack_node_weight_f32", "pack_weight", "padded_len", "pair_tiled", "pair_untiled",
    "unpack_planes", "vf_alloc", "xp_alloc",
    "edge_embed", "edge_embed_f16x3", "edge_transition", "edge_transition_f16x3", "pair_project",
    "encoder_attention", "ipa_attention", "ipa_attention_f16", "ipa_prep_points", "ipa_prep_points_f16",
    "CHAIN_WIDTHS", "NARROW_MAX_WORK", "SMALL_ROWS", "embed_assemble", "ipa_projections", "node_apply",
    "node_apply_chain", "node_apply_multi", "node_chain", "node_linear", "node_linear_f32", "node_linear_multi", "node_linear_vfrag", "pack_planes",
    "row_layernorm", "small_rows_variant", "to_act",
    "forward_marginal", "frames_to_backbone", "rigid_compose_update", "rigid_scale_trans", "se3_step", "torsion_head",
    "RMSD_LAUNCH_PAIRS", "apply_xform", "ca_pairwise_distances", "ca_pwd_js", "ca_rmsd_matrix", "ca_sample_stats", "ca_superpose", "rmsd_row_chunk",
    "TM_MAX_RES", "ca_tm_matrix", "ca_tm_superpose",
    "LDDT_MAX_RES", "ca_lddt_matrix", "ca_lddt_per_residue", "lddt_workspace_bytes",
    "VIOL_MAX_RES", "backbone_violations",
    "SS_MAX_RES", "secondary_structure",
    "SASA_MAX_POINTS", "SASA_MAX_RES", "backbone_sasa", "sphere_points",
    "SAXS_MAX_Q", "SAXS_MAX_RES", "SAXS_MAX_TYPES", "ca_scattering",
    "CONTACT_MAX_RES", "ca_contact_map", "ca_contact_stats", "ca_native_contacts", "ca_native_q",
    "PCA_MAX_RES", "ca_aligned_mean", "ca_covariance", "ca_fit_transforms", "ca_project",
    "CLUSTER_MAX_N", "cluster_adjacency", "cluster_gromos",
    "float64_normal_outputs", "format_pdb_models", "host_rng_can_discard", "host_rng_discard_float64_normals", "host_rng_fast_forward_ok",
    "merge_pdb_files", "write_pdb_models",
    "register_torch_ops",
]

register_torch_ops()
```

### str2str_amd/ops/binding.py

```python
import ctypes
import os
from typing import Optional

import torch

_PKG = os.path.dirname(os.path.dirname(os.path.abspath(__file__)))
LIB_PATH = os.environ.get("STR2STR_HIP_LIB") or os.path.join(_PKG, "libstr2str_hip.so")
ABI_VERSION = 40

_lib = None

_vp, _i, _f, _d, _ll = ctypes.c_void_p, ctypes.c_int, ctypes.c_float, ctypes.c_double, ctypes.c_longlong

_SIGNATURES = {
    "s2s_abi_version": [],
    "s2s_edge_transition": [_vp] * 12 + [_i, _i, _f, _vp, _vp, _vp, _vp, _vp],
    "s2s_edge_transition_f16x3": [_vp] * 9 + [_i, _i, _f, _i, _vp, _vp, _vp, _i, _vp, _vp],
    "s2s_edge_embed": [_vp] * 15 + [_i, _i, _i, _i, _i, _f, _vp, _vp, _vp, _vp, _vp],
    "s2s_edge_embed_f16x3": [_vp] * 14 + [_i, _i, _i, _i, _i, _f, _i, _vp, _vp, _vp, _vp, _vp],
    "s2s_pair_project": [_vp] * 5 + [_i, _i, _vp],
    "s2s_ipa_prep_points": [_vp] * 6 + [_ll, _i, _i, _i, _i, _vp],
    "s2s_ipa_attention": [_vp] * 12 + [_i, _i, _i, _i, _i, _i, _i, _f, _f, _vp],
    "s2s_ipa_opair": [_vp] * 4 + [_i, _i, _i, _i, _i, _i, _i, _vp],
    "s2s_ipa_prep_points_f16": [_vp] * 9 + [_i, _i, _i, _i, _i, _i, _vp, _vp, _vp, _vp, _vp],
    "s2s_ipa_attention_f16w": [_vp] * 15 + [_i] * 8 + [_f, _f, _i, _vp],
    "s2s_rigid_compose_update": [_vp] * 4 + [_ll, _i, _vp],
    "s2s_torsion_head": [_vp, _i, _i, _vp, _ll, _vp, _f, _vp, _ll, _vp],
    "s2s_rigid_scale_trans": [_vp, _vp, _ll, _f, _i, _vp],
    "s2s_set_backbone_tables": [_vp] * 4,
    "s2s_frames_to_backbone": [_vp] * 5 + [_ll, _vp],
    "s2s_se3_step": [_vp] * 12 + [_i, _i, _d, _vp, _d, _i, _i, _d, _vp],
    "s2s_forward_marginal": [_vp] * 7 + [_i, _vp, _vp, _f, _vp, _i, _i, _vp],
    "s2s_pack_planes": [_vp, _ll, _i, _i, _i, _vp, _i, _i, _vp, _vp, _vp],
    "s2s_node_linear": [_vp, _vp, _vp, _ll, _i, _i, _i, _vp, _i, _vp, _vp, _i, _vp, _vp, _f, _vp, _vp, _i, _i, _vp, _i, _i, _i, _i, _vp, _vp],
    "s2s_node_linear_f32": [_vp, _i, _vp, _vp, _ll, _i, _i, _i, _vp, _i, _vp, _vp, _i, _vp, _vp, _f, _vp, _vp, _i, _i, _vp],
    "s2s_node_linear_multi": [_vp, _i, _vp, _vp],
    "s2s_node_chain": [_vp, _vp, _i, _ll, _i, _i, _vp, _i, _vp, _i, _vp, _vp, _f, _vp, _vp, _i, _vp, _vp, _f, _vp, _vp, _i, _i, _vp, _i, _i, _vp, _vp],
    "s2s_embed_assemble": [_vp, _ll, _vp, _ll, _vp, _vp, _ll, _i, _vp, _vp, _vp, _vp, _i, _vp, _vp],
    "s2s_row_layernorm": [_vp, _i, _ll, _i, _vp, _vp, _f, _vp, _vp, _i, _i, _vp, _i, _i, _vp, _vp],
    "s2s_node_linear_vfrag": [_vp, _vp, _vp, _ll, _i, _i, _i, _vp, _i, _i, _vp, _vp],
    "s2s_encoder_attention": [_vp, _vp, _vp, _vp, _i, _i, _i, _i, _vp, _vp],
    "s2s_encoder_attention_f16x3": [_vp, _vp, _vp, _vp, _i, _i, _i, _i, _vp, _vp],
    "s2s_ca_sample_stats": [_vp, _i, _i, _f, _i, _vp, _vp, _vp, _vp],
    "s2s_ca_pairwise_distances": [_vp, _i, _i, _i, _vp, _vp],
    "s2s_ca_pwd_js": [_vp, _i, _vp, _i, _i, _i, _i, _d, _vp, _vp, _vp, _vp],
    "s2s_ca_rmsd_matrix": [_vp, _i, _vp, _i, _i, _vp, _vp, _vp, _ll, _vp],
    "s2s_ca_superpose": [_vp, _i, _vp, _i, _vp, _vp, _vp, _vp],
    "s2s_apply_xform": [_vp, _vp, _i, _ll, _vp, _vp],
    "s2s_ca_tm_matrix": [_vp, _i, _vp, _i, _i, _d, _vp, _vp],
    "s2s_ca_tm_superpose": [_vp, _i, _vp, _i, _d, _vp, _vp, _vp],
    "s2s_ca_lddt_matrix": [_vp, _i, _vp, _i, _i, _d, _i, _vp, _vp, _ll, _vp],
    "s2s_ca_lddt_per_residue": [_vp, _i, _vp, _i, _d, _i, _vp, _vp, _vp, _ll, _vp],
    "s2s_ca_contact_map": [_vp, _i, _i, _d, _i, _vp, _vp, _vp, _vp],
    "s2s_ca_contact_stats": [_vp, _i, _i, _d, _i, _vp, _vp, _vp],
    "s2s_ca_native_contacts": [_vp, _i, _d, _i, _vp, _vp, _vp, _vp],
    "s2s_ca_native_q": [_vp, _i, _i, _vp, _vp, _i, _d, _d, _vp, _vp, _vp, _vp],
    "s2s_backbone_violations": [_vp, _i, _i, _vp, _vp, _vp, _d, _d, _vp, _vp, _vp, _vp, _vp, _vp, _vp],
    "s2s_secondary_structure": [_vp, _i, _i, _vp, _vp, _vp, _vp, _vp, _vp, _vp, _vp],
    "s2s_backbone_sasa": [_vp, _i, _i, _vp, _vp, _d, _vp, _i, _vp, _vp, _vp, _vp],
    "s2s_ca_scattering": [_vp, _i, _i, _vp, _i, _vp, _vp, _i, _vp, _vp, _vp],
    "s2s_ca_aligned_mean": [_vp, _i, _i, _vp, _vp, _vp, _vp],
    "s2s_ca_covariance": [_vp, _i, _i, _vp, _vp, _vp, _vp, _vp, _ll, _vp],
    "s2s_ca_project": [_vp, _i, _i, _vp, _vp, _vp, _i, _vp, _vp],
    "s2s_cluster_adjacency": [_vp, _i, _i, _i, _d, _i, _vp, _vp, _vp],
    "s2s_cluster_gromos": [_vp, _vp, _i, _i, _i, _vp, _vp, _vp, _vp, _vp, _vp, _vp],
    "s2s_format_pdb_models": [_vp, _i, _i, _vp, _vp, _vp, _vp, _i, _i, _vp, _ll],
    "s2s_write_pdb_models": [ctypes.c_char_p, _i, _vp, _i, _i, _vp, _vp, _vp, _vp, _i, _i],
    "s2s_merge_pdb_files": [_vp, _i, ctypes.c_char_p],
    "s2s_mt19937_discard": [_vp, _vp, _vp, ctypes.c_ulonglong],
}
_LL_RETURN = ("s2s_format_pdb_models", "s2s_write_pdb_models", "s2s_merge_pdb_files")
EXPORTS = tuple(_SIGNATURES)


class HipLibraryError(RuntimeError):
    pass


class WeightRangeError(HipLibraryError):
    """A weight does not fit the f16x3 packing (|32 w| >= 65504)."""


class KernelTimer:

    active = None

    def __init__(self, *names):
        self.names = set(names)
        self.events = {n: [] for n in names}
        self.work = {n: [0, 0] for n in names}

    def __enter__(self):
        KernelTimer.active = self if self.names else None
        return self

    def __exit__(self, *exc):
        KernelTimer.active = None

    def total_ms(self, name):
        torch.cuda.synchronize()
        ev = self.events[name]
        return sum(a.elapsed_time(b) for a, b in ev), len(ev)

    def mean_ms(self, name):
        total, n = self.total_ms(name)
        return (total / n if n else float("nan")), n


def _timed(name, launch, flops=0, nbytes=0):
    kt = KernelTimer.active
    if kt is None or name not in kt.names:
        return launch()
    kt.work[name][0] += int(flops)
    kt.work[name][1] += int(nbytes)
    a, b = torch.cuda.Event(enable_timing=True), torch.cuda.Event(enable_timing=True)
    a.record()
    rc = launch()
    b.record()
    kt.events[name].append((a, b))
    return rc


def load_library(path: Optional[str] = None):
    global _lib
    if _lib is not None and path is None:
        return _lib
    p = path or LIB_PATH
    if not os.path.exists(p):
        raise HipLibraryError(f"{p} not found: the HIP kernels are not built. Run `python -m str2str_amd.build` "
                              "(hipcc --offload-arch=gfx950). There is no CPU fallback for the sampling path.")
    lib = ctypes.CDLL(p)
    for name, args in _SIGNATURES.items():
        fn = getattr(lib, name)
        fn.argtypes = args
        fn.restype = ctypes.c_longlong if name in _LL_RETURN else ctypes.c_int
    v = lib.s2s_abi_version()
    if v != ABI_VERSION:
        raise HipLibraryError(f"libstr2str_hip.so ABI {v} != expected {ABI_VERSION}; rebuild")
    if path is None:
        _lib = lib
    return lib


def _check(rc: int, what: str):
    if rc != 0:
        raise HipLibraryError(f"{what} failed with hipError_t {rc}")


def _p(t: Optional[torch.Tensor]):
    return None if t is None else ctypes.c_void_p(t.data_ptr())


def _stream():
    return ctypes.c_void_p(torch.cuda.current_stream().cuda_stream)


def _req(t: torch.Tensor, dtype=torch.float32, name="tensor") -> torch.Tensor:
    if not isinstance(t, torch.Tensor) or not t.is_cuda:
        raise HipLibraryError(f"{name}: expected a tensor on the HIP device (no CPU fallback), got "
                              f"{getattr(t, 'device', type(t))}")
    if t.dtype != dtype:
        raise HipLibraryError(f"{name}: expected dtype {dtype}, got {t.dtype}")
    if not t.is_contiguous():
        raise HipLibraryError(f"{name}: expected a contiguous tensor")
    return t


def _req_all(dtype=torch.float32, /, **tensors):
    for name, t in tensors.items():
        _req(t, dtype, name)


def _req_opt(dtype=torch.float32, /, **tensors):
    _req_all(dtype, **{name: t for name, t in tensors.items() if t is not None})


def _int_arg(v: Optional[int]) -> int:
    return -1 if v is None else v


def _opt_int(v: Optional[int]) -> Optional[int]:
    return None if v is None or v < 0 else v
```

### str2str_amd/ops/pair.py

```python
import torch

from .binding import HipLibraryError, _check, _p, _req, _req_all, _req_opt, _stream, _timed, load_library
from .packing import PairTiled, column_blocked
from .range_guard import range_flag


def _proj_outputs(proj, B, N, dev, dtype=torch.float32, name="proj.wp"):
    if proj is None:
        return None, None, None, None
    w, b64 = proj
    _req(w, dtype, name); _req(b64, name="proj.b64")
    return w, b64, torch.empty(B, 8, N, N, device=dev, dtype=torch.float32), torch.empty(B, N, N, 32, device=dev, dtype=torch.float32)


def edge_transition_f16x3(edge, node_ab, node_p, wstream, b2, gamma, beta, mask, ln_eps=1e-5, out=None, proj=None,
                          out_layout: str = "rowmajor", prescale_exp: int = 0, ab_kernel_form: bool = False):
    lib = load_library()
    B, N = edge.shape[0], edge.shape[1]
    in_tiled = isinstance(edge, PairTiled)
    if not 0 <= int(prescale_exp) <= 15:
        raise HipLibraryError(f"edge_transition_f16x3: prescale_exp {prescale_exp} outside 0 .. 15")
    if tuple(edge.shape) != (B, N, N, 128) or tuple(node_ab.shape) != (B, N, 896) or tuple(node_p.shape) != (B, N, 128):
        raise HipLibraryError(f"edge_transition_f16x3: bad shapes (edge {tuple(edge.shape)}, node_ab {tuple(node_ab.shape)}, node_p {tuple(node_p.shape)}): "
                              "edge is [B, N, N, 128], node_p [B, N, 128] and node_ab [B, N, 896] = EdgeTransition.node_parts (row half | column half | "
                              "j-side residual through the final layer; the 768-column form of earlier ABI versions is not accepted)")
    if not ab_kernel_form or prescale_exp:
        sc = node_ab.new_ones(896)
        sc[:384] = 2.0 ** -int(prescale_exp)
        sc[384:768] = 1.0 if ab_kernel_form else 32.0
        sc[768:] = (1.0 if ab_kernel_form else 32.0) * 2.0 ** -int(prescale_exp)
        node_ab = node_ab * sc
        if not ab_kernel_form:
            node_ab[..., 768:] -= node_ab[..., 768:].mean(dim=-1, keepdim=True)
    if out_layout not in ("rowmajor", "tiled", "none") or (out_layout == "none" and proj is None):
        raise HipLibraryError(f"edge_transition_f16x3: out_layout {out_layout!r}" + (" needs proj" if out_layout == "none" else ""))
    _req(edge.buf if in_tiled else edge, name="edge")
    _req_all(node_ab=node_ab, node_p=node_p, b2=b2, gamma=gamma, beta=beta)
    pw, pb, pbias, ppz = _proj_outputs(proj, B, N, edge.device, torch.int16, "wstream")
    wstream = _req(wstream, torch.int16, "wstream") if proj is None else pw
    if wstream.numel() * 2 != (31 if proj is not None else 30) * 32 * 1024:
        raise HipLibraryError("edge_transition_f16x3: weight stream has the wrong number of stages")
    _req_opt(mask=mask)
    if out_layout == "none":
        out = None
    elif out is None:
        out = PairTiled(B, N, edge.device) if out_layout == "tiled" else torch.empty(B, N, N, 128, device=edge.device, dtype=torch.float32)
    elif out.data_ptr() == edge.data_ptr():
        raise HipLibraryError("edge_transition: out may not alias edge")
    elif isinstance(out, PairTiled) != (out_layout == "tiled"):
        raise HipLibraryError("edge_transition_f16x3: out does not have the requested layout")
    io = (1 if in_tiled else 0) | {"rowmajor": 0, "tiled": 2, "none": 4}[out_layout]
    _check(_timed("s2s_edge_transition", lambda: lib.s2s_edge_transition_f16x3(
        _p(edge.buf if in_tiled else edge), _p(node_ab), _p(node_p), _p(wstream), _p(b2), _p(gamma), _p(beta), _p(mask),
        _p(out.buf if isinstance(out, PairTiled) else out), B, N, ln_eps, io, _p(pb), _p(pbias), _p(ppz), int(prescale_exp), _p(range_flag()),
        _stream())), "s2s_edge_transition_f16x3")
    return out if proj is None else (out, pbias, ppz)


def edge_transition(edge, node_ab, node_p, w1p, w2p, wfp, b2, bf, gamma, beta, mask, ln_eps=1e-5, out=None, proj=None):
    lib = load_library()
    B, N = edge.shape[0], edge.shape[1]
    _req(edge, name="edge")
    if edge.shape != (B, N, N, 128) or node_ab.shape != (B, N, 768) or node_p.shape != (B, N, 128):
        raise HipLibraryError(f"edge_transition: bad shapes {tuple(edge.shape)} {tuple(node_ab.shape)} {tuple(node_p.shape)}")
    _req_all(node_ab=node_ab, node_p=node_p, w1p=w1p, w2p=w2p, wfp=wfp, b2=b2, bf=bf, gamma=gamma, beta=beta)
    _req_opt(mask=mask)
    if out is None:
        out = torch.empty_like(edge)
    elif out.data_ptr() == edge.data_ptr():
        raise HipLibraryError("edge_transition: out may not alias edge")
    _req(out, name="out")
    pw, pb, pbias, ppz = _proj_outputs(proj, B, N, edge.device)
    _check(_timed("s2s_edge_transition", lambda: lib.s2s_edge_transition(
        _p(edge), _p(node_ab), _p(node_p), _p(w1p), _p(w2p), _p(wfp), _p(b2), _p(bf), _p(gamma), _p(beta), _p(mask),
        _p(out), B, N, ln_eps, _p(pw), _p(pb), _p(pbias), _p(ppz), _stream())), "s2s_edge_transition")
    return out if proj is None else (out, pbias, ppz)


def edge_embed(node_a, node_b, rel_table, bin_table, bin_lower, residue_idx, ca, w2p, w3p, b2, b3, gamma, beta, mask,
               rel_offset: int, ln_eps=1e-5, out=None, proj=None):
    lib = load_library()
    B, N = node_a.shape[0], node_a.shape[1]
    _req_all(node_a=node_a, node_b=node_b, rel_table=rel_table, bin_table=bin_table, bin_lower=bin_lower, ca=ca, w2p=w2p, w3p=w3p, b2=b2, b3=b3,
             gamma=gamma, beta=beta)
    _req(residue_idx, torch.int64, "residue_idx")
    _req_opt(mask=mask)
    out = torch.empty(B, N, N, 128, device=node_a.device, dtype=torch.float32) if out is None else out
    pw, pb, pbias, ppz = _proj_outputs(proj, B, N, node_a.device)
    _check(lib.s2s_edge_embed(_p(node_a), _p(node_b), _p(rel_table), _p(bin_table), _p(bin_lower), _p(residue_idx), _p(ca),
                              _p(w2p), _p(w3p), _p(b2), _p(b3), _p(gamma), _p(beta), _p(mask), _p(out), B, N,
                              int(rel_offset), rel_table.shape[0], bin_table.shape[0], ln_eps, _p(pw), _p(pb), _p(pbias),
                              _p(ppz), _stream()), "s2s_edge_embed")
    return out if proj is None else (out, pbias, ppz)


def edge_embed_f16x3(node_a, node_b, rel_table, bin_table, bin_lower, residue_idx, ca, wstream, b2, b3, gamma, beta, mask,
                     rel_offset: int, ln_eps=1e-5, out=None, proj=None, column_blocked_tables=False, out_layout: str = "rowmajor"):
    lib = load_library()
    B, N = node_a.shape[0], node_a.shape[1]
    if not column_blocked_tables:
        node_b, rel_table, bin_table = column_blocked(node_b), column_blocked(rel_table), column_blocked(bin_table)
    if node_b.shape != (B, 32, N, 4) or rel_table.shape[0] != 32 or bin_table.shape[0] != 32:
        raise HipLibraryError("edge_embed_f16x3: tables are not column-blocked [.., 32, rows, 4]")
    _req_all(node_a=node_a, node_b=node_b, rel_table=rel_table, bin_table=bin_table, bin_lower=bin_lower, ca=ca, b2=b2, b3=b3, gamma=gamma, beta=beta)
    _req(residue_idx, torch.int64, "residue_idx")
    pw, pb, pbias, ppz = _proj_outputs(proj, B, N, node_a.device, torch.int16, "wstream")
    wstream = _req(wstream, torch.int16, "wstream") if proj is None else pw
    if wstream.numel() * 2 != (5 if proj is not None else 4) * 32 * 1024:
        raise HipLibraryError("s2s_edge_embed_f16x3: weight stream has the wrong number of stages")
    _req_opt(mask=mask)
    if out_layout not in ("rowmajor", "tiled"):
        raise HipLibraryError(f"edge_embed_f16x3: out_layout {out_layout!r}")
    tiled = out_layout == "tiled"
    if out is None:
        out = PairTiled(B, N, node_a.device) if tiled else torch.empty(B, N, N, 128, device=node_a.device, dtype=torch.float32)
    elif isinstance(out, PairTiled) != tiled:
        raise HipLibraryError("edge_embed_f16x3: out does not have the requested layout")
    _check(_timed("s2s_edge_embed", lambda: lib.s2s_edge_embed_f16x3(
        _p(node_a), _p(node_b), _p(rel_table), _p(bin_table), _p(bin_lower), _p(residue_idx), _p(ca), _p(wstream), _p(b2), _p(b3),
        _p(gamma), _p(beta), _p(mask), _p(out.buf if tiled else out), B, N, int(rel_offset), rel_table.shape[1], bin_table.shape[1],
        ln_eps, 1 if tiled else 0, _p(pb), _p(pbias), _p(ppz), _p(range_flag()), _stream())), "s2s_edge_embed_f16x3")
    return out if proj is None else (out, pbias, ppz)


def pair_project(edge, wp, bias64, attn_bias=None, pair_z=None):
    lib = load_library()
    B, N = edge.shape[0], edge.shape[1]
    _req(edge, name="edge"); _req(wp, name="wp"); _req(bias64, name="bias64")
    attn_bias = torch.empty(B, 8, N, N, device=edge.device, dtype=torch.float32) if attn_bias is None else attn_bias
    pair_z = torch.empty(B, N, N, 32, device=edge.device, dtype=torch.float32) if pair_z is None else pair_z
    _check(lib.s2s_pair_project(_p(edge), _p(wp), _p(bias64), _p(attn_bias), _p(pair_z), B, N, _stream()), "s2s_pair_project")
    return attn_bias, pair_z
```

### str2str_amd/ops/torch_ops.py

```python
import torch

from .attention import encoder_attention, ipa_attention, ipa_attention_f16, ipa_prep_points, ipa_prep_points_f16
from .binding import _opt_int
from .geometry import forward_marginal, frames_to_backbone, rigid_compose_update, rigid_scale_trans, se3_step, torsion_head
from .node import (embed_assemble, ipa_projections, node_chain, node_linear, node_linear_f32, node_linear_multi, node_linear_vfrag, pack_planes,
                   row_layernorm)
from .packing import PairTiled
from .pair import edge_embed, edge_embed_f16x3, edge_transition, edge_transition_f16x3, pair_project

_registered = False


def _ln3(g, b, eps):
    return None if g is None else (g, b, eps)


def _op_node_linear(xp, wpk, bias, n_rows, k_in, n_out, tiles, pre_scale=None, relu=False, pre_mask=None, residual=None, ln_gamma=None,
                    ln_beta=None, ln_eps=0.0, post_mask=None, out_f32=None, out_col0=0, want_f32=True, out_xp=None, out_xp_k=-1,
                    out_xp_k0=0, want_xp=False, map_pad=0, map_src=0):
    return node_linear(xp, wpk, bias, n_rows, k_in, n_out, tiles, pre_scale=pre_scale, relu=relu, pre_mask=pre_mask, residual=residual,
                       ln=_ln3(ln_gamma, ln_beta, ln_eps), post_mask=post_mask, out_f32=out_f32, out_col0=out_col0, want_f32=want_f32,
                       out_xp=out_xp, out_xp_k=_opt_int(out_xp_k), out_xp_k0=out_xp_k0, want_xp=want_xp,
                       row_map=(map_pad, map_src) if map_pad else None)


def _op_node_linear_f32(x, wpk32, bias, n_rows, k_in, n_out, tiles, pre_scale=None, relu=False, pre_mask=None, residual=None, ln_gamma=None,
                        ln_beta=None, ln_eps=0.0, post_mask=None, out=None, out_col0=0):
    return node_linear_f32(x, wpk32, bias, n_rows, k_in, n_out, tiles, pre_scale=pre_scale, relu=relu, pre_mask=pre_mask,
                           residual=residual, ln=_ln3(ln_gamma, ln_beta, ln_eps), post_mask=post_mask, out=out, out_col0=out_col0)


def _op_edge_transition_f16x3_chain(edge, in_tiled, B, N, node_ab, node_p, wstream, b2, gamma, beta, mask, ln_eps, proj_bias64,
                                    out_layout, prescale_exp=0, ab_kernel_form=False):
    e = PairTiled(B, N, buf=edge) if in_tiled else edge
    r = edge_transition_f16x3(e, node_ab, node_p, wstream, b2, gamma, beta, mask, ln_eps,
                              proj=None if proj_bias64 is None else (wstream, proj_bias64), out_layout=out_layout, prescale_exp=prescale_exp,
                              ab_kernel_form=ab_kernel_form)
    z, bias, pz = r if proj_bias64 is not None else (r, None, None)
    return (z.buf if isinstance(z, PairTiled) else z), bias, pz


_TORCH_OPS = {
    "edge_transition(Tensor edge, Tensor node_ab, Tensor node_p, Tensor w1p, Tensor w2p, Tensor wfp, Tensor b2, "
    "Tensor bf, Tensor gamma, Tensor beta, Tensor? mask, float ln_eps) -> Tensor": lambda *a: edge_transition(*a),
    "edge_transition_f16x3(Tensor edge, Tensor node_ab, Tensor node_p, Tensor wstream, Tensor b2, "
    "Tensor gamma, Tensor beta, Tensor? mask, float ln_eps, int prescale_exp=0) -> Tensor":
        lambda e, nab, np_, ws, b2, g, b, m, eps, pe=0: edge_transition_f16x3(e, nab, np_, ws, b2, g, b, m, eps, prescale_exp=pe),
    "edge_transition_f16x3_chain(Tensor edge, bool in_tiled, int B, int N, Tensor node_ab, Tensor node_p, Tensor wstream, Tensor b2, "
    "Tensor gamma, Tensor beta, Tensor? mask, float ln_eps, Tensor? proj_bias64, str out_layout, int prescale_exp=0, "
    "bool ab_kernel_form=False) -> (Tensor?, Tensor?, Tensor?)": _op_edge_transition_f16x3_chain,
    "edge_embed(Tensor node_a, Tensor node_b, Tensor rel_table, Tensor bin_table, Tensor bin_lower, Tensor residue_idx, Tensor ca, "
    "Tensor w2p, Tensor w3p, Tensor b2, Tensor b3, Tensor gamma, Tensor beta, Tensor? mask, int rel_offset, float ln_eps) -> Tensor":
        lambda *a: edge_embed(*a),
    "edge_embed_f16x3(Tensor node_a, Tensor node_b, Tensor rel_table, Tensor bin_table, Tensor bin_lower, Tensor residue_idx, Tensor ca, "
    "Tensor wstream, Tensor b2, Tensor b3, Tensor gamma, Tensor beta, Tensor? mask, int rel_offset, float ln_eps) -> Tensor":
        lambda *a: edge_embed_f16x3(*a),
    "pair_project(Tensor edge, Tensor wp, Tensor bias64) -> (Tensor, Tensor)": lambda *a: pair_project(*a),
    "ipa_prep_points(Tensor rigids7, Tensor q_pts_lin, Tensor kv_pts_lin, int n_heads=8, int n_qk=8, int n_v=12) -> (Tensor, Tensor, Tensor)":
        lambda *a: ipa_prep_points(*a),
    "ipa_attention(Tensor q, Tensor kv, Tensor q_pts, Tensor k_pts, Tensor v_pts, Tensor attn_bias, Tensor pair_z, "
    "Tensor mask, Tensor rigids7, Tensor head_w) -> Tensor": lambda *a: ipa_attention(*a),
    "ipa_prep_points_f16(Tensor rigids7, Tensor q_pts_lin, Tensor kv_pts_lin, Tensor head_w, int n_heads=8, int n_qk=8, int n_v=12, "
    "int c_hidden=256) -> (Tensor, Tensor, Tensor, Tensor, Tensor)": lambda *a: ipa_prep_points_f16(*a),
    "ipa_prep_points_shared_kv(Tensor rigids7, Tensor q_pts_lin, Tensor kv_pts_lin, Tensor head_w, Tensor s_xp, int n_heads=8, int n_qk=8, "
    "int n_v=12, int c_hidden=256) -> (Tensor, Tensor, Tensor, Tensor, Tensor, Tensor?, Tensor)":
        lambda r7, qp, kvp, hw, s_xp, h=8, nq=8, nv=12, c=256: ipa_prep_points_f16(r7, qp, kvp, hw, h, nq, nv, c, s_xp),
    "ipa_attention_f16w(Tensor q_xp, Tensor k_xp, Tensor v_vf, Tensor qp_xp, Tensor kp_xp, Tensor vp_vf, Tensor q2, Tensor k2, "
    "Tensor(a!) attn_bias, Tensor pair_z, Tensor mask, Tensor rigids7, int n_heads=8, int c_hidden=256, int n_qk=8, int n_v=12, int c_pz=32, "
    "float inf=1e5, float eps=1e-8, bool logits_inplace=False) -> (Tensor, Tensor)":
        lambda q, k, v, qp, kp, vp, q2, k2, ab, pz, m, r7, *rest: ipa_attention_f16(q, k, v, (qp, kp, vp, q2, k2), ab, pz, m, r7, *rest),
    "encoder_attention(Tensor qkv, Tensor? key_bias, int n_samples, int n_res, int n_heads=4, bool want_f32=False, bool want_xp=True, "
    "str arith='f32') -> (Tensor?, Tensor?)": lambda *a: encoder_attention(*a),
    "node_linear(Tensor xp, Tensor wpk, Tensor? bias, int n_rows, int k_in, int n_out, int tiles, Tensor? pre_scale=None, bool relu=False, "
    "Tensor? pre_mask=None, Tensor? residual=None, Tensor? ln_gamma=None, Tensor? ln_beta=None, float ln_eps=0.0, Tensor? post_mask=None, "
    "Tensor(a!)? out_f32=None, int out_col0=0, bool want_f32=True, Tensor(b!)? out_xp=None, int out_xp_k=-1, int out_xp_k0=0, "
    "bool want_xp=False, int map_pad=0, int map_src=0) -> (Tensor?, Tensor?)": _op_node_linear,
    "node_linear_f32(Tensor x, Tensor wpk32, Tensor? bias, int n_rows, int k_in, int n_out, int tiles, Tensor? pre_scale=None, "
    "bool relu=False, Tensor? pre_mask=None, Tensor? residual=None, Tensor? ln_gamma=None, Tensor? ln_beta=None, float ln_eps=0.0, "
    "Tensor? post_mask=None, Tensor(a!)? out=None, int out_col0=0) -> Tensor": _op_node_linear_f32,
    "node_linear_vfrag(Tensor xp, Tensor wpk, Tensor? bias, int n_rows, int k_in, int n_out, int tiles_per_head=8, int map_pad=0, "
    "int map_src=0) -> Tensor":
        lambda xp, w, b, m, k, n, tph=8, mp=0, ms=0: node_linear_vfrag(xp, w, b, m, k, n, tph, row_map=(mp, ms) if mp else None),
    "ipa_projections(Tensor s_xp, Tensor[] q, Tensor[] k, Tensor[] v, Tensor[] qp, Tensor[] kvp, int[] dims, int n_rows, int n_rows_padded, "
    "int map_pad=0, int map_src=0) -> (Tensor, Tensor?, Tensor?, Tensor, Tensor)":
        lambda s_xp, q, k, v, qp, kvp, dims, m, mo, mp=0, ms=0: ipa_projections(
            s_xp, *[({"w": t[0], "b": t[1], "k": dims[3 * i], "n": dims[3 * i + 1], "tg": dims[3 * i + 2]} if len(t) else None)
                    for i, t in enumerate((q, k, v, qp, kvp))],
            m, mo, (mp, ms) if mp else None),
    "embed_assemble(Tensor t_img, Tensor node_const, Tensor fa, Tensor fb, int n_samples, int n_res, bool planes, bool b_col_blocked) "
    "-> (Tensor, Tensor, Tensor)": lambda *a: embed_assemble(*a),
    "node_linear_multi(Tensor xp, Tensor[] w, Tensor[] bias, Tensor[] pre_scale, int[] dims, Tensor(a!)[] out_f32, Tensor(b!)[] out_xp) -> ()":
        lambda *a: node_linear_multi(*a),
    "node_chain(Tensor xp, Tensor[] w_row, Tensor[] bias, bool[] relu, int n_rows, int width, Tensor? pre_mask=None, Tensor? residual=None, "
    "Tensor? ln_gamma=None, Tensor? ln_beta=None, float ln_eps=0.0, Tensor? post_mask=None, Tensor(a!)? out_f32=None, int out_col0=0, "
    "bool want_f32=True, Tensor(b!)? out_xp=None, int out_xp_k=-1, int out_xp_k0=0, bool want_xp=False, int k_in0=-1, "
    "Tensor? mid_residual=None, Tensor(c!)? mid_out_f32=None, Tensor? mid_ln_gamma=None, Tensor? mid_ln_beta=None, float mid_ln_eps=0.0) "
    "-> (Tensor?, Tensor?)":
        lambda xp, w, b, r, m, wd, pm=None, res=None, g=None, be=None, eps=0.0, pom=None, of=None, oc=0, wf=True, ox=None, ok=-1, ok0=0, wx=False,
        k0=-1, mr=None, mo=None, mg=None, mb=None, me=0.0: node_chain(
            xp, w, b, r, m, wd, pm, res, g, be, eps, pom, of, oc, wf, ox, _opt_int(ok), ok0, wx, _opt_int(k0), mr, mo, _ln3(mg, mb, me)),
    "row_layernorm(Tensor x, int n_rows, int n_cols, Tensor gamma, Tensor beta, float eps, Tensor? post_mask=None, Tensor(a!)? out_f32=None, "
    "int out_col0=0, bool want_f32=True, Tensor(b!)? out_xp=None, int out_xp_k=-1, int out_xp_k0=0, bool want_xp=False) -> (Tensor?, Tensor?)":
        lambda x, m, n, g, b, eps, pm=None, of=None, oc=0, wf=True, ox=None, ok=-1, ok0=0, wx=False: row_layernorm(
            x, m, n, g, b, eps, pm, of, oc, wf, ox, _opt_int(ok), ok0, wx),
    "pack_planes(Tensor x, int col0=0, int n_cols=-1, Tensor(a!)? out=None, int out_k=-1, int k0=0, Tensor? row_scale=None) -> Tensor":
        lambda x, c0=0, nc=-1, out=None, ok=-1, k0=0, rs=None: pack_planes(x, c0, _opt_int(nc), out, _opt_int(ok), k0, rs),
    "se3_step(Tensor x0_7, Tensor xt_7, Tensor mask, Tensor diffuse_mask, Tensor params8, float dt) -> Tensor":
        lambda x0, xt, m, dm, p8, dt: se3_step(x0, xt, m, dm, p8, dt)[0],
    "forward_marginal(Tensor? rigids0_4x4, Tensor z_axis, Tensor u01, Tensor z_trans, Tensor cdf_rows, Tensor row_of_sample, "
    "Tensor omega_grid, Tensor? params2, Tensor? diffuse_mask=None, float coordinate_scaling=0.1) -> Tensor":
        lambda *a: forward_marginal(*a),
    "rigid_compose_update(Tensor rigids7, Tensor update6, Tensor mask) -> Tensor": lambda *a: rigid_compose_update(*a),
    "rigid_scale_trans(Tensor rigids7, float scale, bool divide=False) -> Tensor": lambda *a: rigid_scale_trans(*a),
    "torsion_head(Tensor u, int n_rows, bool normalize=True, float eps=1e-8, Tensor? gt_sin_cos=None, Tensor? fixed_mask=None) -> Tensor":
        lambda *a: torsion_head(*a),
    "frames_to_backbone(Tensor rigids7, Tensor psi, Tensor? aatype) -> Tensor": lambda r, p, a: frames_to_backbone(r, p, a)[0],
}


def register_torch_ops():
    global _registered
    if _registered:
        return
    lib = torch.library.Library("str2str_amd", "DEF")
    impl = torch.library.Library("str2str_amd", "IMPL", "CUDA")
    for schema, fn in _TORCH_OPS.items():
        lib.define(schema)
        impl.impl(schema.split("(")[0], fn)
    register_torch_ops._libs = (lib, impl)
    _registered = True
```

### str2str_amd/sampler.py

```python
from __future__ import annotations

import contextlib
import logging
import os
from typing import Optional, Tuple

import numpy as np
import torch

from . import ops
from .arith import FAMILIES, net_arith, use_arith
from .common.all_atom import compute_backbone
from .common.rigid_utils import Rigid

_REPEAT_KEYS = ("aatype", "residue_mask", "fixed_mask", "residue_idx", "torsion_angles_sin_cos")
_log = logging.getLogger("str2str_amd.sampler")
_GRAPH_MAX_PAIRS = 1 << 16
_GRAPH_MIN_STEPS = 16


class _GraphedNet:

    def __init__(self, net, feats):
        self.feats = dict(feats)
        self.static = tuple(k for k in ("rigids_t", "sc_ca_t", "t_img") if k in feats)
        for k in self.static:
            self.feats[k] = feats[k].clone()
        side = torch.cuda.Stream()
        side.wait_stream(torch.cuda.current_stream())
        with torch.cuda.stream(side):
            for _ in range(2):
                _net_eval(net, self.feats, True)
        torch.cuda.current_stream().wait_stream(side)
        self.graph = torch.cuda.CUDAGraph()
        with torch.cuda.graph(self.graph):
            self.out = _net_eval(net, self.feats, True)
        self._pinned = _graph_read_tensors(net)

    def __call__(self, feats):
        for k in self.static:
            self.feats[k].copy_(feats[k])
        self.graph.replay()
        return self.out


def _graph_read_tensors(net):
    from .models.net.layers import DerivedCache

    def tensors(x, out):
        if torch.is_tensor(x):
            out.append(x)
        elif isinstance(x, dict):
            for v in x.values():
                tensors(v, out)
        elif isinstance(x, (list, tuple)):
            for v in x:
                tensors(v, out)
        return out

    keep = []
    for m in net.modules():
        for v in vars(m).values():
            if isinstance(v, DerivedCache):
                tensors(v.held(), keep)
    return keep


def _net_eval(net, feats, defer_psi: bool):
    if defer_psi and hasattr(net, "blend_psi"):
        return net(feats, as_tensor_7=False, defer_psi_blend=True)
    return net(feats, as_tensor_7=False)


_GRAPH_CACHE = {}
_GRAPH_CACHE_MAX = 4


def _graph_key(net, feats, b, N):
    import hashlib

    h = hashlib.sha1()
    for k in sorted(feats):
        v = feats[k]
        if k in ("rigids_t", "sc_ca_t", "t_img", "t") or not torch.is_tensor(v):
            continue
        h.update(k.encode()); h.update(str(tuple(v.shape)).encode()); h.update(v.detach().cpu().numpy().tobytes())
    modes = tuple((type(m).__name__, a, getattr(m, a)) for m in net.modules() for a in getattr(type(m), "launch_switches", ()))
    return (id(net), sum(p._version for p in net.parameters()), b, N, modes, h.hexdigest())


def _maybe_graph(net, feats, b, N, trace, n_steps):
    mode = os.environ.get("S2S_HIP_GRAPH", "auto")
    if mode == "0" or trace is not None or ops.KernelTimer.active is not None:
        return None
    if mode != "1" and (b * N * N > _GRAPH_MAX_PAIRS or n_steps < _GRAPH_MIN_STEPS):
        return None
    key = _graph_key(net, feats, b, N)
    hit = _GRAPH_CACHE.get(key)
    if hit is not None:
        return hit
    try:
        g = _GraphedNet(net, feats)
    except ops.HipLibraryError:
        raise
    except RuntimeError as e:
        _log.warning("HIP graph capture failed (%s); continuing with eager launches", repr(e)[:200])
        torch.cuda.synchronize()
        return None
    if len(_GRAPH_CACHE) >= _GRAPH_CACHE_MAX:
        _GRAPH_CACHE.pop(next(iter(_GRAPH_CACHE)))
    _GRAPH_CACHE[key] = g
    return g


def schedule(t_delta: float, num_timesteps: int, min_t: float):
    T = t_delta if t_delta > 0 else 1.0
    n = int(float(num_timesteps) * T)
    return T, n, 1.0 / n, np.linspace(min_t, T, n)[::-1]


def shard_range(total: int, rank: int, world: int) -> Tuple[int, int]:
    per = -(-total // world)
    lo = min(total, rank * per)
    return lo, min(total, lo + per)


def rank_chunk_slices(n_replica: int, replica_per_batch: int, rank: int, world: int):
    my_lo, my_hi = shard_range(n_replica, rank, world)
    sizes = [replica_per_batch] * (n_replica // replica_per_batch)
    if n_replica % replica_per_batch > 0:
        sizes.append(n_replica % replica_per_batch)
    out, c0 = [], 0
    for bsz in sizes:
        lo, hi = max(my_lo, c0) - c0, min(my_hi, c0 + bsz) - c0
        out.append((bsz, lo, hi) if hi > lo else (bsz, 0, 0))
        c0 += bsz
    return out


@torch.no_grad()
def denoise_loop(net, diffuser, feats: dict, rigids_t: torch.Tensor, ts, dt: float, *, min_t: float,
                 noise_scale: float = 1.0, probability_flow: bool = True, self_conditioning: bool = True,
                 center_mode: int = 1, host_noise=None, trace: Optional[list] = None):
    if float(ts[-1]) != min_t:
        raise ValueError(f"the schedule ends at t = {float(ts[-1])}, not at min_t = {min_t}: its last evaluation is the sample")
    return _guarded_pass(net, diffuser, [dict(rigids_t=rigids_t, ts=ts, dt=dt, feats=feats)], noise_scale=noise_scale,
                         probability_flow=probability_flow, self_conditioning=self_conditioning, center_mode=center_mode,
                         host_noise=host_noise, trace=trace)[0]


def _guarded_pass(net, diffuser, groups, *, probability_flow: bool, host_noise, trace: Optional[list] = None, **kw):
    def run_pass():
        return _denoise_pass(net, diffuser, groups, probability_flow=probability_flow, host_noise=host_noise, trace=trace, **kw)

    return _range_guarded(net, run_pass, groups[0]["rigids_t"].device, host_draws=host_noise is not None,
                          device_draws=host_noise is None and not probability_flow, trace=trace)[0]


def _range_guarded(net, run_pass, device, *, host_draws: bool, device_draws: bool, trace: Optional[list] = None):
    if net_arith(net) == "f32":
        out = run_pass()
        _require_finite(out[1], "fp32")
        return out
    demoted = set(getattr(net, "range_fallback", None) or ())
    rng_state = torch.cuda.get_rng_state(device) if device_draws else None
    host_state = torch.get_rng_state() if host_draws else None
    while True:
        if host_state is not None:
            torch.set_rng_state(host_state)
        ops.range_flag_reset(device)
        try:
            with use_arith(net, "f32", families=tuple(demoted)):
                out = run_pass()
            finite = bool(torch.isfinite(out[1]).all())
            bits = ops.range_flag_read(device)
            if bits == 0 and finite:
                return out
            new = set(ops.range_families(bits)) - demoted
            why = f"an activation left f16's safe range in the split-f16 kernels ({ops.range_flag_names(bits)}{'' if finite else '; non-finite frames'})"
            if "edge_transition" in new:
                e_now = _raise_edge_prescale(net)
                if e_now:
                    new.discard("edge_transition")
                    _log.warning("range guard: %s; the edge transitions keep the split-f16 kernel with a block exponent of %d on their "
                                 "hidden activations (planes of 2^-%d x the value: exact, same speed; usable range 2^%d) -- re-running this chunk",
                                 why, e_now, e_now, 15 + e_now)
                    net.range_prescale = {"edge_transition": e_now}
                    if not new:
                        if trace is not None:
                            del trace[:]
                        if rng_state is not None:
                            torch.cuda.set_rng_state(rng_state, device)
                        continue
        except ops.WeightRangeError as e:
            new = set(FAMILIES) - demoted
            if not new:
                raise
            why = f"a weight does not fit the split-f16 packing ({e})"
        if not new:
            if len(demoted) == len(FAMILIES):
                _require_finite(out[1], "fp32 (range fallback)")
                return out
            new = set(FAMILIES) - demoted
        demoted |= new
        _log.warning("range guard: %s; re-running this chunk with the %s kernels on exact fp32 and keeping them there (now in fp32: %s; "
                     "S2S_ARITH=f32 starts everything in fp32)", why, " + ".join(sorted(new)), ", ".join(sorted(demoted)))
        net.range_fallback = frozenset(demoted)
        if trace is not None:
            del trace[:]
        if rng_state is not None:
            torch.cuda.set_rng_state(rng_state, device)


def _raise_edge_prescale(net, step: int = 5, top: int = 15) -> int:
    mods = [m for m in net.modules() if hasattr(m, "prescale_exp") and getattr(m, "arith", None) == "f16x3"]
    cur = max((int(m.prescale_exp) for m in mods), default=top)
    if not mods or cur >= top:
        return 0
    for m in mods:
        m.prescale_exp = min(cur + step, top)
    return min(cur + step, top)


def _require_finite(rigids7, what):
    if not bool(torch.isfinite(rigids7).all()):
        raise ops.HipLibraryError(f"non-finite frames at the end of the trajectory in the {what} arithmetic: the network itself "
                                  "overflows fp32 on this input (weights / checkpoint?)")


@contextlib.contextmanager
def _backbone_deferred(net):
    keep = getattr(net, "backbone_in_forward", None)
    if keep is not None:
        net.backbone_in_forward = False
    try:
        yield
    finally:
        if keep is not None:
            net.backbone_in_forward = keep


def _denoise_pass(net, diffuser, groups, *, noise_scale: float, probability_flow: bool, self_conditioning: bool, center_mode: int,
                  host_noise, trace: Optional[list]):
    device = groups[0]["rigids_t"].device
    N = groups[0]["rigids_t"].shape[1]
    emb = net.embedder
    order = sorted(range(len(groups)), key=lambda k: -len(groups[k]["ts"]))
    n_max = len(groups[order[0]]["ts"])
    per_sample = len(groups) > 1
    timg, p8s, base, o = [], [], {}, 0
    for k in order:
        t_all = torch.as_tensor(np.ascontiguousarray(groups[k]["ts"], dtype=np.float64)).float()
        p8s.append(diffuser.step_params(t_all).to(device))
        timg.append(emb.time_images(emb.time_embed(t_all).to(device)))
        base[k] = o
        o += len(t_all)
    TIMG, P8 = (torch.cat(timg).contiguous(), torch.cat(p8s).contiguous()) if per_sample else (timg[0], p8s[0])
    defer_psi = trace is None

    def eager(f):
        return _net_eval(net, f, defer_psi)

    with _backbone_deferred(net):
        rig = sc = idx = dtv = feats = mask = diffuse_mask = graphed = None
        members, run = [], eager
        for g in range(n_max):
            joining = [k for k in order if n_max - len(groups[k]["ts"]) == g]
            for k in joining:
                rk = groups[k]["rigids_t"]
                bk = rk.shape[0]
                fk = dict(groups[k]["feats"])
                for m in ("residue_mask", "fixed_mask"):
                    fk[m] = fk[m].to(device).float().contiguous()
                fk.update(rigids_t=rk, sc_ca_t=torch.zeros(bk, N, 3, device=device), t=torch.zeros(bk), t_img=TIMG[base[k]])
                if not per_sample:
                    graphed = _maybe_graph(net, fk, bk, N, trace, n_max)
                    run = graphed if graphed is not None else eager
                sck = fk["sc_ca_t"]
                if self_conditioning:
                    sck = run(fk)["rigids7"][..., 4:].clone()
                rig = rk if rig is None else torch.cat([rig, rk])
                sc = sck if sc is None else torch.cat([sc, sck])
                if per_sample:
                    ik = torch.full((bk,), base[k], dtype=torch.int64, device=device)
                    dk = torch.full((bk,), float(groups[k]["dt"]), dtype=torch.float64, device=device)
                    idx = ik if idx is None else torch.cat([idx, ik])
                    dtv = dk if dtv is None else torch.cat([dtv, dk])
                members.append((k, bk, fk))
            b = rig.shape[0]
            if joining:
                if len(members) == 1:
                    feats = members[0][2]
                else:
                    feats = {key: torch.cat([f[key].to(device) for _, _, f in members]) for key in _REPEAT_KEYS if key in members[0][2]}
                    feats["t"] = torch.zeros(b)
                mask = feats["residue_mask"]
                diffuse_mask = ((1 - feats["fixed_mask"]) * mask).contiguous()
            feats["rigids_t"], feats["sc_ca_t"] = rig, sc
            feats["t_img"] = TIMG.index_select(0, idx) if per_sample else TIMG[g]
            out = run(feats)
            x0_7 = out["rigids7"]
            t = float(groups[order[0]]["ts"][g])
            if g == n_max - 1:
                if trace is not None:
                    trace.append(dict(t=t, rigids_t=rig, sc_ca_t=sc, x0=x0_7, psi=out["psi"]))
                break
            sc_in = sc
            if self_conditioning:
                sc = x0_7[..., 4:].clone() if graphed is not None else x0_7[..., 4:]
            z = host_noise() if host_noise is not None else None
            z_rot, z_trans = z if z is not None else (None, None)
            if not probability_flow and z_rot is None:
                z_rot = torch.randn(b, N, 3, dtype=torch.float64, device=device)
                z_trans = torch.randn(b, N, 3, dtype=torch.float64, device=device)
            p8, dt = (P8.index_select(0, idx), dtv) if per_sample else (P8[g].expand(b, 8).contiguous(), groups[0]["dt"])
            nxt, rs, tsc = diffuser.step(x0_7, rig, p8, dt, mask, diffuse_mask, center_trans=center_mode, noise_scale=noise_scale,
                                         probability_flow=probability_flow, z_rot=z_rot, z_trans=z_trans, want_scores=trace is not None)
            if trace is not None:
                trace.append(dict(t=t, rigids_t=rig, sc_ca_t=sc_in, x0=x0_7, psi=out["psi"], rot_score=rs, trans_score=tsc, next7=nxt))
            rig = nxt
            if per_sample:
                idx = idx + 1
        psi = out["psi"]
        if out.get("psi_deferred"):
            psi = net.blend_psi(psi, feats["torsion_angles_sin_cos"], feats["fixed_mask"])
        atom37 = compute_backbone(out["rigids"], psi, aatype=feats.get("aatype"), _rigids7=x0_7)[0]
    samples, o = [None] * len(groups), 0
    for k, bk, _ in members:
        samples[k] = (atom37[o:o + bk], x0_7[o:o + bk], psi[o:o + bk])
        o += bk
    return samples, x0_7


def _require_hip_device(device, net) -> torch.device:
    device = torch.device(device) if device is not None else next(net.parameters()).device
    if device.type != "cuda":
        raise ops.HipLibraryError("the sampler needs the HIP device (MI355X); there is no CPU fallback")
    return device


def _start_frames(diffuser, batch: dict, rigids_0: Rigid, t_delta: float, lo: int, hi: int, rng: str, device):
    B_total, N = rigids_0.shape[0], rigids_0.shape[1]
    b = hi - lo
    if rng == "device":
        if b == 0:
            return None
        if t_delta > 0:
            dmask = batch["residue_mask"].to(device).float().reshape(1, N).expand(b, N).contiguous()
            return diffuser.forward_marginal_device(rigids_0[lo:hi].to_tensor_4x4().to(device), t_delta, dmask)
        return diffuser.forward_marginal_device(None, None, shape=(b, N))
    nt, keep = int(os.environ.get("S2S_HOST_FM_THREADS", "1")), torch.get_num_threads()
    if nt > 0 and nt != keep:
        torch.set_num_threads(nt)
    try:
        if t_delta > 0:
            rigids_t = diffuser.forward_marginal(rigids_0=rigids_0.to(device="cpu"), t=t_delta * torch.ones(B_total),
                                                 diffuse_mask=batch["residue_mask"].cpu().repeat(B_total, 1),
                                                 as_tensor_7=True)["rigids_t"]
        else:
            rigids_t = diffuser.sample_prior(shape=rigids_0.shape, device="cpu", as_tensor_7=True)["rigids_t"]
    finally:
        if nt > 0 and nt != keep:
            torch.set_num_threads(keep)
    if b == 0:
        return None
    return rigids_t[lo:hi].to(device).float().contiguous()


def _burn_step_draws(B_total: int, N: int, n_draw_steps: int):
    if ops.host_rng_discard_float64_normals(B_total * N * 3, 2 * n_draw_steps):
        return
    for _ in range(n_draw_steps):
        torch.randn(B_total, N, 3, dtype=torch.float64)
        torch.randn(B_total, N, 3, dtype=torch.float64)


def _skips_unused_draws(probability_flow: bool, B_total: int, N: int) -> bool:
    return probability_flow and ops.host_rng_can_discard(B_total * N * 3)


def _chunk_rigids(gt_frames_4x4: torch.Tensor, bsz: int) -> Rigid:
    return Rigid.from_tensor_4x4(gt_frames_4x4.repeat(bsz, *(1,) * (gt_frames_4x4.ndim - 1)))


def _expand_features(batch: dict, b: int, device) -> dict:
    return {k: batch[k].to(device).repeat(b, *(1,) * (batch[k].ndim - 1)) for k in _REPEAT_KEYS if k in batch}


def _draw_entries(diffuser, batch: dict, rig0, N: int, scheds, entries, *, rng: str, probability_flow: bool, device):
    n_max = max(scheds[i][1] for i, _, _, _ in entries)
    starts, tail = {}, None
    for e, (i, bsz, lo, hi) in enumerate(entries):
        if hi == lo and rng == "device":
            continue
        t_delta, n = scheds[i][:2]
        r = _start_frames(diffuser, batch, rig0(bsz), t_delta, lo, hi, rng, device)
        if rng == "host":
            if e + 1 == len(entries) and n == n_max and not _skips_unused_draws(probability_flow, bsz, N):
                tail = (bsz, lo, hi, n - 1)
            else:
                _burn_step_draws(bsz, N, n - 1)
        if r is not None:
            starts.setdefault(i, []).append(r)
    if not starts and tail is not None:
        _burn_step_draws(tail[0], N, tail[3])
    return starts, tail


@torch.no_grad()
def _sample_batch(net, diffuser, batch: dict, rig0, N: int, scheds, entries, *, noise_scale: float, probability_flow: bool,
                  self_conditioning: bool, device, rng: str, trace: Optional[list] = None) -> dict:
    starts, tail = _draw_entries(diffuser, batch, rig0, N, scheds, entries, rng=rng, probability_flow=probability_flow, device=device)
    if not starts:
        return {}

    bsz, lo, hi = tail[:3] if tail is not None else (0, 0, 0)

    def host_noise():
        zr = torch.randn(bsz, N, 3, dtype=torch.float64)
        zt = torch.randn(bsz, N, 3, dtype=torch.float64)
        if probability_flow:
            return None
        return zr[lo:hi].to(device).contiguous(), zt[lo:hi].to(device).contiguous()

    groups = []
    for i, rs in starts.items():
        rigids_t = torch.cat(rs, dim=0) if len(rs) > 1 else rs[0]
        groups.append(dict(rigids_t=rigids_t, ts=scheds[i][3], dt=scheds[i][2], feats=_expand_features(batch, rigids_t.shape[0], device)))
    samples = _guarded_pass(net, diffuser, groups, noise_scale=noise_scale, probability_flow=probability_flow,
                            self_conditioning=self_conditioning, center_mode=1, host_noise=host_noise if tail is not None else None,
                            trace=trace)
    return dict(zip(starts, samples))


def forward_backward(net, diffuser, batch: dict, rigids_0: Rigid, t_delta: float, *, num_timesteps: int,
                     min_t: float = 0.01, noise_scale: float = 1.0, probability_flow: bool = True,
                     self_conditioning: bool = True, device=None, shard: Tuple[int, int] = (0, 1),
                     replica_slice: Optional[Tuple[int, int]] = None, rng: str = "host", trace: Optional[list] = None,
                     return_rigids: bool = False):
    device = _require_hip_device(device, net)
    B_total, N = rigids_0.shape[0], rigids_0.shape[1]
    lo, hi = replica_slice if replica_slice is not None else shard_range(B_total, *shard)
    if not (0 <= lo <= hi <= B_total):
        raise ValueError(f"replica_slice {(lo, hi)} outside the chunk of {B_total} replicas")
    T, n, dt, ts = schedule(t_delta, num_timesteps, min_t)
    out = _sample_batch(net, diffuser, batch, lambda bsz: rigids_0, N, [(t_delta, n, dt, ts)], [(0, B_total, lo, hi)],
                        noise_scale=noise_scale, probability_flow=probability_flow, self_conditioning=self_conditioning, device=device,
                        rng=rng, trace=trace)
    if not out:
        return torch.zeros(0, N, 37, 3, device=device)
    return out[0] if return_rigids else out[0][0]


_MERGE_MAX_PAIRS = 8 << 20


def merge_chunk_groups(chunks, N: int, *, mergeable: bool = True, max_pairs: int = None):
    max_pairs = _MERGE_MAX_PAIRS if max_pairs is None else max_pairs
    if not mergeable or os.environ.get("S2S_MERGE_CHUNKS", "1") == "0":
        return [[c] for c in chunks]
    groups, cur, cur_b = [], [], 0
    for c in chunks:
        b = c[2] - c[1]
        if cur and (cur_b + b) * N * N > max_pairs:
            groups.append(cur)
            cur, cur_b = [], 0
        cur.append(c)
        cur_b += b
    if cur:
        groups.append(cur)
    return groups


def merge_delta_groups(steps, b: int, N: int, max_pairs: int = None):
    max_pairs = _MERGE_MAX_PAIRS if max_pairs is None else max_pairs
    per = max(1, b) * N * N
    cap = 1 if os.environ.get("S2S_MERGE_DELTAS", "1") == "0" else max(1, max_pairs // per)
    return [list(range(i, min(i + cap, len(steps)))) for i in range(0, len(steps), cap)]


def _batch_plan(chunks, steps, N: int, *, merge_deltas: bool, merge_chunks: bool, max_pairs: int = None):
    b_rank = sum(hi - lo for _, lo, hi in chunks)
    plan = []
    for grp in (merge_delta_groups(steps, b_rank, N, max_pairs) if merge_deltas else [[i] for i in range(len(steps))]):
        if len(grp) > 1:
            plan.append((grp, [[(i, *c) for i in grp for c in chunks]]))
        else:
            plan.append((grp, [[(grp[0], *c) for c in cg] for cg in merge_chunk_groups(chunks, N, mergeable=merge_chunks, max_pairs=max_pairs)]))
    return plan


def forward_backward_chunks(net, diffuser, batch: dict, gt_frames_4x4: torch.Tensor, chunks, t_delta: float, *, num_timesteps: int,
                            min_t: float = 0.01, noise_scale: float = 1.0, probability_flow: bool = True,
                            self_conditioning: bool = True, device=None, rng: str = "host", max_pairs: int = None):
    return forward_backward_deltas(net, diffuser, batch, gt_frames_4x4, chunks, [t_delta], num_timesteps=num_timesteps, min_t=min_t,
                                   noise_scale=noise_scale, probability_flow=probability_flow, self_conditioning=self_conditioning,
                                   device=device, rng=rng, max_pairs=max_pairs)[0]


def forward_backward_deltas(net, diffuser, batch: dict, gt_frames_4x4: torch.Tensor, chunks, delta_range, **kw):
    delta_range = list(delta_range)
    out = [None] * len(delta_range)
    for idx, a37s in iter_forward_backward_deltas(net, diffuser, batch, gt_frames_4x4, chunks, delta_range, **kw):
        for i, a in zip(idx, a37s):
            out[i] = a
    return out


def iter_forward_backward_deltas(net, diffuser, batch: dict, gt_frames_4x4: torch.Tensor, chunks, delta_range, *, num_timesteps: int,
                                 min_t: float = 0.01, noise_scale: float = 1.0, probability_flow: bool = True,
                                 self_conditioning: bool = True, device=None, rng: str = "host", max_pairs: int = None):
    device = _require_hip_device(device, net)
    N = gt_frames_4x4.shape[-3]
    scheds = [(float(t),) + schedule(float(t), num_timesteps, min_t)[1:] for t in delta_range]
    merge_deltas = probability_flow and len(scheds) > 1 and sum(hi - lo for _, lo, hi in chunks) > 0 and all(s[0] > 0 for s in scheds) \
        and hasattr(getattr(net, "embedder", None), "time_images")
    plan = _batch_plan(chunks, [s[1] for s in scheds], N, merge_deltas=merge_deltas, merge_chunks=probability_flow or rng == "device",
                       max_pairs=max_pairs)
    for grp, batches in plan:
        pieces = {i: [] for i in grp}
        for entries in batches:
            done = _sample_batch(net, diffuser, batch, lambda bsz: _chunk_rigids(gt_frames_4x4, bsz), N, scheds, entries,
                                 noise_scale=noise_scale, probability_flow=probability_flow, self_conditioning=self_conditioning,
                                 device=device, rng=rng)
            for i, sample in done.items():
                pieces[i].append(sample[0])
        yield grp, [(torch.cat(p, dim=0) if len(p) > 1 else p[0]) if p else torch.zeros(0, N, 37, 3, device=device) for p in pieces.values()]


def forward_flops(n_res: int) -> float:
    return 2251264.0 * n_res * n_res + 3.24e7 * n_res


def plan_mixed_work(lengths, replicas: int, world: int = 1, *, max_pairs: int = 24 << 20, ms_per_mpair: float = 10.7,
                    launch_floor_ms: float = 4.0):
    lengths = [int(x) for x in lengths]
    items = []
    for k, L in enumerate(lengths):
        for r in range(world):
            lo, hi = shard_range(replicas, r, world)
            if hi > lo:
                items.append((forward_flops(L) * (hi - lo), k, lo, hi))
    items.sort(key=lambda it: (-it[0], it[1], it[2]))
    load = [0.0] * world
    mine = [[] for _ in range(world)]
    for w, k, lo, hi in items:
        r = min(range(world), key=lambda q: (load[q], q))
        load[r] += w
        mine[r].append((k, lo, hi))
    plan = []
    for r in range(world):
        cost = lambda pairs: max(launch_floor_ms, ms_per_mpair * pairs / float(1 << 20))
        batches, cur, cur_b, n_pad = [], [], 0, 0
        for k, lo, hi in sorted(mine[r], key=lambda it: (-lengths[it[0]], it[0], it[1])):
            L, b = lengths[k], hi - lo
            if cur:
                merged = (cur_b + b) * n_pad * n_pad
                if merged > max_pairs or cost(merged) > 1.05 * (cost(cur_b * n_pad * n_pad) + cost(b * L * L)):
                    batches.append({"n_pad": n_pad, "items": cur})
                    cur, cur_b = [], 0
            if not cur:
                n_pad = L
            cur.append((k, lo, hi)); cur_b += b
        if cur:
            batches.append({"n_pad": n_pad, "items": cur})
        plan.append(batches)
    return plan


def mixed_batch_seed(base_seed: int, t_delta: float, chain: int, replica_lo: int) -> int:
    return (int(base_seed) * 1000003 + int(round(float(t_delta) * 1000)) * 998244353 + int(chain) * 7919 + int(replica_lo) * 104729
            + 12345) % (2 ** 63 - 1)


@torch.no_grad()
def sample_mixed_lengths(net, diffuser, targets, replicas: int, t_delta: float, *, num_timesteps: int,
                         min_t: float = 0.01, noise_scale: float = 1.0, probability_flow: bool = True,
                         self_conditioning: bool = True, device=None, rigids_t_init=None, shard: Tuple[int, int] = (0, 1),
                         rng: str = "host", max_pairs: int = 24 << 20, plan=None, seed_base: Optional[int] = None):
    device = torch.device(device) if device is not None else next(net.parameters()).device
    lengths = [int(t["aatype"].shape[1]) for t in targets]
    rank, world = shard
    if plan is None:
        plan = plan_mixed_work(lengths, replicas, world, max_pairs=max_pairs)
    T, n, dt, ts = schedule(t_delta, num_timesteps, min_t)
    pieces = [[] for _ in targets]
    tr = net.translator
    keep = tr.exact_padding
    tr.exact_padding = True
    base_seed = int(torch.initial_seed()) if seed_base is None else int(seed_base)
    host_states = (torch.get_rng_state(), np.random.get_state()) if rng == "host" else None
    try:
        for batch in plan[rank]:
            n_pad = batch["n_pad"]
            if rng == "host":
                ti0, lo0, _ = batch["items"][0]
                item_seed = mixed_batch_seed(base_seed, t_delta, ti0, lo0)
                torch.random.default_generator.manual_seed(item_seed)
                np.random.seed(item_seed % (2 ** 32))
            rows, r_t = {k: [] for k in _REPEAT_KEYS}, []
            for ti, lo, hi in batch["items"]:
                tg, L, b = targets[ti], lengths[ti], hi - lo
                for k in _REPEAT_KEYS:
                    v = tg[k]
                    pad = torch.zeros((1, n_pad - L) + tuple(v.shape[2:]), dtype=v.dtype)
                    if k == "residue_idx" and L < n_pad:
                        pad = pad + v[:, -1:]
                    rows[k].append(torch.cat([v.cpu(), pad], dim=1).repeat(b, *(1,) * (v.ndim - 1)))
                gt4 = tg["rigidgroups_gt_frames"][..., 0, :, :]
                if rigids_t_init is not None:
                    rt = rigids_t_init[ti][lo:hi].to(device).float()
                else:
                    rt = _start_frames(diffuser, tg, _chunk_rigids(gt4, b), t_delta, 0, b, rng, device)
                ident = torch.zeros(b, n_pad - L, 7, device=device)
                ident[..., 0] = 1.0
                r_t.append(torch.cat([rt, ident], dim=1))
            feats = {k: torch.cat(v, dim=0).to(device) for k, v in rows.items()}
            rigids_t = torch.cat(r_t, dim=0).contiguous()
            atom37, _, _ = denoise_loop(net, diffuser, feats, rigids_t, ts, dt, min_t=min_t, noise_scale=noise_scale,
                                        probability_flow=probability_flow, self_conditioning=self_conditioning, center_mode=2)
            o = 0
            for ti, lo, hi in batch["items"]:
                pieces[ti].append((lo, atom37[o:o + hi - lo, :lengths[ti]].clone()))
                o += hi - lo
    finally:
        tr.exact_padding = keep
        if host_states is not None:
            torch.set_rng_state(host_states[0])
            np.random.set_state(host_states[1])
    return [sorted(p, key=lambda x: x[0]) for p in pieces]
```

Baseline: 30.22 conformations/s.

## Compute edge embedding per class table then expand to pairs

When all replicas share one timestep and the fixed mask is 0/1, the edge-embed MLP depends only on (fixed_a, fixed_b, relative offset, distance bin). The new path runs the f16x3 MLP once per class into a small table, then a gather kernel expands it to every pair and writes the projection outputs. This replaces an MLP over B*N*N pairs with one over a few thousand rows plus a memory-bound gather. It adds eligibility checks, an extra launch, and a table allocation.

```diff
diff --git a/include/str2str_hip.h b/include/str2str_hip.h
--- a/include/str2str_hip.h
+++ b/include/str2str_hip.h
@@ -34,6 +34,15 @@
                          const float* ln_beta, const float* mask, float* out, int n_samples, int n_res, int rel_offset,
                          int n_rel, int n_bins, float ln_eps, int out_tiled, const float* proj_bias_cat64,
                          float* proj_attn_bias, float* proj_pair_z, int* range_words, void* stream);
+
+int s2s_edge_embed_classes_f16x3(const float* node_a2, const float* node_b2, const float* rel_table, const float* bin_table,
+                                 const void* weight_stream, const float* b2, const float* b3, const float* ln_gamma,
+                                 const float* ln_beta, float* table, int n_fixed, int n_rel, int n_bins, float ln_eps,
+                                 const float* proj_bias_cat64, int* range_words, void* stream);
+int s2s_edge_embed_expand(const float* table, const int* fixed_cls, const float* bin_lower, const long long* residue_idx,
+                          const float* ca_xyz, const float* mask, const float* proj_bias_cat64, float* out, int out_tiled,
+                          float* proj_attn_bias, float* proj_pair_z, int n_samples, int n_res, int rel_offset, int n_rel,
+                          int n_bins, void* stream);
 
 int s2s_pair_project(const float* edge, const float* w_packed, const float* bias_cat64, float* attn_bias, float* pair_z,
                      int n_samples, int n_res, void* stream);
diff --git a/str2str_amd/build.py b/str2str_amd/build.py
--- a/str2str_amd/build.py
+++ b/str2str_amd/build.py
@@ -37,6 +37,8 @@
     "pair_mlp_f16.hip": ["-mllvm", "-pragma-unroll-threshold=10000000", "-fno-slp-vectorize"],
     "pair_mlp_f16_b.hip": ["-mllvm", "-pragma-unroll-threshold=10000000", "-fno-slp-vectorize"],
     "pair_mlp_f16_c.hip": ["-mllvm", "-pragma-unroll-threshold=10000000", "-fno-slp-vectorize"],
+    "pair_mlp_f16_d.hip": ["-mllvm", "-pragma-unroll-threshold=10000000", "-fno-slp-vectorize"],
+    "pair_embed_expand.hip": [],
     "ipa_attention.hip": ["-mllvm", "-pragma-unroll-threshold=10000000"],
     "ipa_attention_f16w.hip": ["-mllvm", "-pragma-unroll-threshold=10000000", "-fno-slp-vectorize"],
     "node_gemm.hip": ["-mllvm", "-pragma-unroll-threshold=10000000", "-fno-slp-vectorize"],
diff --git a/str2str_amd/csrc/edge_embed_class.h b/str2str_amd/csrc/edge_embed_class.h
--- /dev/null
+++ b/str2str_amd/csrc/edge_embed_class.h
@@ -0,0 +1,38 @@
+#pragma once
+#include <hip/hip_runtime.h>
+
+namespace s2s {
+
+constexpr int kEeBinSlots = 64 + 4;
+constexpr int kEeRecProj = 168;
+constexpr int kEeRecPlain = 128;
+
+__device__ __forceinline__ void ee_fill_bins(float* s_bins, const float* __restrict__ bin_lower, int n_bins) {
+    if (threadIdx.x < kEeBinSlots)
+        s_bins[threadIdx.x] = (int)threadIdx.x < n_bins ? bin_lower[threadIdx.x] : ((int)threadIdx.x == n_bins ? 1e8f : 3.0e38f);
+}
+
+__device__ __forceinline__ int ee_pair_bin(const float* s_bins, int n_bins, float ax, float ay, float az, float bx, float by, float bz) {
+    const float dx = ax - bx, dy = ay - by, dz = az - bz;
+    const float dist = sqrtf(__fmaf_rn(dz, dz, __fmaf_rn(dx, dx, __fmul_rn(dy, dy))));
+    int cnt = 0;
+#pragma unroll
+    for (int u = 0; u < 8; ++u) {
+        const float4 e = *reinterpret_cast<const float4*>(&s_bins[4 * u]);
+        cnt += (e.x < dist) + (e.y < dist) + (e.z < dist) + (e.w < dist);
+    }
+    cnt = cnt > n_bins ? n_bins : cnt;
+    const float up = s_bins[cnt];
+    return (cnt >= 1 && dist < up) ? cnt - 1 : -1;
+}
+
+__device__ __forceinline__ long long ee_rel_row(long long idx_i, long long idx_j, int rel_off, int n_rel) {
+    long long d = idx_i - idx_j + rel_off;
+    return d < 0 ? 0 : (d >= n_rel ? n_rel - 1 : d);
+}
+
+__device__ __forceinline__ unsigned ee_class_row(unsigned fa, unsigned fb, unsigned d, int bin, int n_rel, int n_bins) {
+    return ((fa * 2u + fb) * (unsigned)n_rel + d) * (unsigned)(n_bins + 1) + (unsigned)(bin + 1);
+}
+
+}
diff --git a/str2str_amd/csrc/pair_embed_expand.hip b/str2str_amd/csrc/pair_embed_expand.hip
--- /dev/null
+++ b/str2str_amd/csrc/pair_embed_expand.hip
@@ -0,0 +1,126 @@
+#include <hip/hip_runtime.h>
+
+#include <cstdlib>
+
+#include "edge_embed_class.h"
+#include "str2str_hip.h"
+
+namespace {
+
+typedef float f32x4 __attribute__((ext_vector_type(4)));
+
+template <bool PROJ>
+__global__ void __launch_bounds__(256) edge_embed_expand_kernel(
+    const float* __restrict__ table, const int* __restrict__ fixed_cls, const float* __restrict__ bin_lower,
+    const long long* __restrict__ residue_idx, const float* __restrict__ ca, const float* __restrict__ mask,
+    const float* __restrict__ proj_b, float* __restrict__ out, float* __restrict__ attn_bias, float* __restrict__ pair_z,
+    long long M, int N, int rel_off, int n_rel, int n_bins, int out_tiled) {
+    constexpr unsigned kRec = PROJ ? s2s::kEeRecProj : s2s::kEeRecPlain;
+    __shared__ __attribute__((aligned(16))) float s_bins[s2s::kEeBinSlots];
+    const unsigned lane = threadIdx.x & 63, h = lane >> 5, wave = threadIdx.x >> 6;
+    s2s::ee_fill_bins(s_bins, bin_lower, n_bins);
+    __syncthreads();
+    const long long p0 = ((long long)blockIdx.x * 4 + wave) * 32;
+    if (p0 >= M) return;
+    long long pl = p0 + (lane & 31);
+    const bool valid = pl < M;
+    pl = valid ? pl : M - 1;
+    const unsigned p = (unsigned)pl;
+    const unsigned bi = p / (unsigned)N, j = p - bi * (unsigned)N, bb = bi / (unsigned)N, bj = bb * (unsigned)N + j;
+    const int bin = s2s::ee_pair_bin(s_bins, n_bins, ca[bi * 3 + 0], ca[bi * 3 + 1], ca[bi * 3 + 2], ca[bj * 3 + 0], ca[bj * 3 + 1], ca[bj * 3 + 2]);
+    const unsigned d = (unsigned)s2s::ee_rel_row(residue_idx[bi], residue_idx[bj], rel_off, n_rel);
+    const unsigned row = s2s::ee_class_row((unsigned)fixed_cls[bi], (unsigned)fixed_cls[bj], d, bin, n_rel, n_bins);
+    const float em = mask ? __fmul_rn(mask[bi], mask[bj]) : 1.0f;
+    const float* rec = table + (unsigned long long)row * kRec;
+
+    if (out_tiled) {
+        float* o = out + (unsigned long long)(p0 >> 5) * 4096u + lane * 4u;
+        f32x4 v[16];
+#pragma unroll
+        for (int g = 0; g < 16; ++g) v[g] = *reinterpret_cast<const f32x4*>(rec + 8 * g + 4 * h);
+#pragma unroll
+        for (int g = 0; g < 16; ++g) {
+            const f32x4 w = {__fmul_rn(v[g].x, em), __fmul_rn(v[g].y, em), __fmul_rn(v[g].z, em), __fmul_rn(v[g].w, em)};
+            __builtin_nontemporal_store(w, reinterpret_cast<f32x4*>(o + g * 256));
+        }
+    } else {
+        const unsigned c = lane & 31;
+        f32x4 v[16];
+        float e[16];
+#pragma unroll
+        for (int it = 0; it < 16; ++it) {
+            const int n = 2 * it + (int)h;
+            const unsigned rn = (unsigned)__shfl((int)row, n, 64);
+            e[it] = __shfl(em, n, 64);
+            v[it] = *reinterpret_cast<const f32x4*>(table + (unsigned long long)rn * kRec + 4 * c);
+        }
+#pragma unroll
+        for (int it = 0; it < 16; ++it) {
+            const long long pn = p0 + 2 * it + h;
+            const f32x4 w = {__fmul_rn(v[it].x, e[it]), __fmul_rn(v[it].y, e[it]), __fmul_rn(v[it].z, e[it]), __fmul_rn(v[it].w, e[it])};
+            if (pn < M) __builtin_nontemporal_store(w, reinterpret_cast<f32x4*>(out + (unsigned long long)pn * 128u + 4 * c));
+        }
+    }
+    if constexpr (PROJ) {
+        {
+            f32x4 a = *reinterpret_cast<const f32x4*>(rec + 128 + 4 * h);
+            const f32x4 b = *reinterpret_cast<const f32x4*>(proj_b + 4 * h);
+            a = em == 0.f ? b : a;
+            const long long NN = (long long)N * N;
+            float* o = attn_bias + ((unsigned long long)p + 7ull * bb * (unsigned long long)NN + 4ull * h * (unsigned long long)NN);
+            if (valid) { o[0] = a.x; o[NN] = a.y; o[2 * NN] = a.z; o[3 * NN] = a.w; }
+        }
+        const unsigned c = lane & 7;
+        const f32x4 b = *reinterpret_cast<const f32x4*>(proj_b + 8 + 4 * c);
+#pragma unroll
+        for (int it = 0; it < 4; ++it) {
+            const int n = 8 * it + (int)(lane >> 3);
+            const unsigned rn = (unsigned)__shfl((int)row, n, 64);
+            const float en = __shfl(em, n, 64);
+            f32x4 a = *reinterpret_cast<const f32x4*>(table + (unsigned long long)rn * kRec + 136 + 4 * c);
+            a = en == 0.f ? b : a;
+            const long long pn = p0 + n;
+            if (pn < M) *reinterpret_cast<f32x4*>(pair_z + (unsigned long long)pn * 32u + 4 * c) = a;
+        }
+    }
+}
+
+long long tile_aligned_samples(long long NN) {
+    long long q = 32;
+    while (q > 1 && (NN * (32 / q)) % 32 != 0) q /= 2;
+    return 32 / q;
+}
+
+}
+
+extern "C" int s2s_edge_embed_expand(const float* table, const int* fixed_cls, const float* bin_lower, const long long* residue_idx,
+                                     const float* ca_xyz, const float* mask, const float* proj_bias_cat64, float* out, int out_tiled,
+                                     float* proj_attn_bias, float* proj_pair_z, int n_samples, int n_res, int rel_offset, int n_rel,
+                                     int n_bins, void* stream) {
+    if (n_samples <= 0 || n_res <= 0) return 0;
+    if (n_bins < 1 || n_bins > 32 || (out_tiled & ~1) || n_rel < 1) return (int)hipErrorInvalidValue;
+    if ((proj_attn_bias != nullptr) != (proj_pair_z != nullptr) || (proj_attn_bias && !proj_bias_cat64)) return (int)hipErrorInvalidValue;
+    const long long NN = (long long)n_res * n_res;
+    if (NN >= (1ll << 31)) return (int)hipErrorInvalidValue;
+    const char* cap_env = getenv("S2S_EE_MAX_PAIRS");
+    long long cap = cap_env ? atoll(cap_env) : 0;
+    if (cap <= 0 || cap > (1ll << 31) - 1) cap = (1ll << 31) - 1;
+    long long chunk = cap / NN;
+    if (out_tiled && chunk < n_samples) chunk -= chunk % tile_aligned_samples(NN);
+    if (chunk < 1) return (int)hipErrorInvalidValue;
+    for (long long b0 = 0; b0 < n_samples; b0 += chunk) {
+        const long long nb = n_samples - b0 < chunk ? n_samples - b0 : chunk;
+        const long long M = nb * NN, rows0 = b0 * n_res;
+        const unsigned grid = (unsigned)((M + 127) / 128);
+        const float* mk = mask ? mask + rows0 : nullptr;
+        if (proj_attn_bias)
+            hipLaunchKernelGGL(edge_embed_expand_kernel<true>, dim3(grid), dim3(256), 0, (hipStream_t)stream, table, fixed_cls + rows0,
+                               bin_lower, residue_idx + rows0, ca_xyz + rows0 * 3, mk, proj_bias_cat64, out + b0 * NN * 128, proj_attn_bias + b0 * 8 * NN,
+                               proj_pair_z + b0 * NN * 32, M, n_res, rel_offset, n_rel, n_bins, out_tiled);
+        else
+            hipLaunchKernelGGL(edge_embed_expand_kernel<false>, dim3(grid), dim3(256), 0, (hipStream_t)stream, table, fixed_cls + rows0,
+                               bin_lower, residue_idx + rows0, ca_xyz + rows0 * 3, mk, (const float*)nullptr, out + b0 * NN * 128, (float*)nullptr,
+                               (float*)nullptr, M, n_res, rel_offset, n_rel, n_bins, out_tiled);
+    }
+    return (int)hipGetLastError();
+}
diff --git a/str2str_amd/csrc/pair_mlp_f16.hip b/str2str_amd/csrc/pair_mlp_f16.hip
--- a/str2str_amd/csrc/pair_mlp_f16.hip
+++ b/str2str_amd/csrc/pair_mlp_f16.hip
@@ -2,6 +2,7 @@
 
 #include <cstdlib>
 
+#include "edge_embed_class.h"
 #include "f16x3.h"
 #include "range_flag.h"
 #include "str2str_hip.h"
@@ -484,7 +485,7 @@
 }
 
 
-template <bool PROJ>
+template <bool PROJ, bool TABLE = false>
 __global__ void __launch_bounds__(256) edge_embed_f16_kernel(
     const float* __restrict__ node_a, const float* __restrict__ node_b, const float* __restrict__ rel_tab,
     const float* __restrict__ bin_tab, const float* __restrict__ bin_lower, const long long* __restrict__ residue_idx,
@@ -496,7 +497,7 @@
     constexpr int kSlots = 8 * kStages;
     __shared__ __attribute__((aligned(16))) char s_w[2][kStageBytes];
     __shared__ __attribute__((aligned(16))) float s_vec[512 + 64];
-    __shared__ __attribute__((aligned(16))) float s_bins[64 + 4];
+    __shared__ __attribute__((aligned(16))) float s_bins[s2s::kEeBinSlots];
     const int lane = threadIdx.x & 63, h = lane >> 5, wave = threadIdx.x >> 6;
 
     const unsigned voff = wave * 8192 + lane * 16;
@@ -538,7 +539,7 @@
         bool valid;
     };
     const long long NN = (long long)N * N;
-    const __amdgpu_buffer_rsrc_t rs_b = __builtin_amdgcn_make_buffer_rsrc((void*)node_b, 0, (unsigned)(M / N * 512), 0x00020000);
+    const __amdgpu_buffer_rsrc_t rs_b = __builtin_amdgcn_make_buffer_rsrc((void*)node_b, 0, (unsigned)((TABLE ? (long long)N : M / N) * 512), 0x00020000);
     const __amdgpu_buffer_rsrc_t rs_r = __builtin_amdgcn_make_buffer_rsrc((void*)rel_tab, 0, n_rel * 512, 0x00020000);
     const __amdgpu_buffer_rsrc_t rs_k = __builtin_amdgcn_make_buffer_rsrc((void*)bin_tab, 0, n_bins * 512, 0x00020000);
     struct Raw {
@@ -563,6 +564,14 @@
         r.valid = p < M;
         p = r.valid ? p : M - 1;
         r.p = p;
+        if constexpr (TABLE) {
+            const unsigned nb1 = (unsigned)n_bins + 1u, q = (unsigned)p / nb1, cls = q / (unsigned)n_rel;
+            r.bi = cls >> 1; r.bj = cls & 1u; r.bb = 0;
+            r.ii = q - cls * (unsigned)n_rel; r.ij = (unsigned)p - q * nb1;
+            r.ax = r.ay = r.az = r.bx = r.by = r.bz = 0.f;
+            r.mi = r.mj = 1.f;
+            return r;
+        }
         unsigned bi, j, bb, i;
         div_n((unsigned)p, bi, j);
         div_n(bi, bb, i);
@@ -578,19 +587,8 @@
     auto setup_b = [&](const Raw& r) -> Ctx {
         Ctx c;
         c.valid = r.valid;
-        const float dx = r.ax - r.bx, dy = r.ay - r.by, dz = r.az - r.bz;
-        const float dist = sqrtf(__fadd_rn(__fadd_rn(__fmul_rn(dx, dx), __fmul_rn(dy, dy)), __fmul_rn(dz, dz)));
-        int cnt = 0;
-#pragma unroll
-        for (int u = 0; u < 8; ++u) {
-            const float4 e = *reinterpret_cast<const float4*>(&s_bins[4 * u]);
-            cnt += (e.x < dist) + (e.y < dist) + (e.z < dist) + (e.w < dist);
-        }
-        cnt = cnt > n_bins ? n_bins : cnt;
-        const float up = s_bins[cnt];
-        const int bin = (cnt >= 1 && dist < up) ? cnt - 1 : -1;
-        long long d = r.ii - r.ij + rel_off;
-        d = d < 0 ? 0 : (d >= n_rel ? n_rel - 1 : d);
+        const int bin = TABLE ? (int)r.ij - 1 : s2s::ee_pair_bin(s_bins, n_bins, r.ax, r.ay, r.az, r.bx, r.by, r.bz);
+        const long long d = TABLE ? r.ii : s2s::ee_rel_row(r.ii, r.ij, rel_off, n_rel);
         c.ra = node_a + r.bi * 128;
         const unsigned jj = (unsigned)(r.bj - r.bb * N);
         c.vb = ((unsigned)r.bb * 32u * (unsigned)N + (unsigned)h * (unsigned)N + jj) * 16u;
@@ -599,7 +597,7 @@
         c.kb = bin < 0 ? 0.f : 1.f;
         c.p = r.p;
         c.boff = r.p + 7 * r.bb * NN;
-        c.em = mask ? r.mi * r.mj : 1.0f;
+        c.em = (!TABLE && mask) ? r.mi * r.mj : 1.0f;
         return c;
     };
     float amax = 0.f;
@@ -639,7 +637,7 @@
 
     const long long n_wt = (M + 127) / 128;
     long long wt = blockIdx.x;
-    if (threadIdx.x < 68) s_bins[threadIdx.x] = (int)threadIdx.x < n_bins ? bin_lower[threadIdx.x] : ((int)threadIdx.x == n_bins ? 1e8f : 3.0e38f);
+    if constexpr (!TABLE) s2s::ee_fill_bins(s_bins, bin_lower, n_bins);
     __syncthreads();
     Ctx cur = setup_b(setup_a(wt));
     f16x8 xp[8][2];
@@ -682,14 +680,15 @@
         pin_frag(xp[k]);
     };
     float ln_mean = 0.f, ln_rstd = 0.f;
-    const unsigned out_lane = out_tiled ? lane * 16u : (unsigned)((lane & 31) * 512 + h * 16), out_step = out_tiled ? 1024u : 32u;
+    constexpr unsigned kRec = TABLE ? (PROJ ? s2s::kEeRecProj : s2s::kEeRecPlain) : 128u;
+    const unsigned out_lane = out_tiled ? lane * 16u : (unsigned)((lane & 31) * (kRec * 4) + h * 16), out_step = out_tiled ? 1024u : 32u;
     f16x8 xq[2][2];
     __amdgpu_buffer_rsrc_t rs_out;
     auto out_rsrc = [&](long long wg_tile) {
         const long long p0 = (wg_tile * 4 + __builtin_amdgcn_readfirstlane(wave)) * 32;
         const long long left = M - p0;
-        rs_out = __builtin_amdgcn_make_buffer_rsrc((void*)(out + (p0 < M ? p0 : 0) * 128), 0,
-                                                   (unsigned)(left <= 0 ? 0 : (left < 32 && !out_tiled ? left : 32)) * 512u, 0x00020000);
+        rs_out = __builtin_amdgcn_make_buffer_rsrc((void*)(out + (p0 < M ? p0 : 0) * kRec), 0,
+                                                   (unsigned)(left <= 0 ? 0 : (left < 32 && !out_tiled ? left : 32)) * (kRec * 4u), 0x00020000);
     };
     float4 lga[2], lbe[2];
     auto ln_load = [&](auto kc) {
@@ -830,16 +829,18 @@
     if constexpr (PROJ) {
         if (cur.valid) {
             const float4 b0 = ldg4(s_vec + 512, 0, h);
-            float* o = proj_bias_out + cur.boff + 4 * h * NN;
+            float* o = TABLE ? out + cur.p * kRec + 128 + 4 * h : proj_bias_out + cur.boff + 4 * h * NN;
+            const long long hs = TABLE ? 1 : NN;
+            float* pz = TABLE ? out + cur.p * kRec + 136 : proj_pz_out + cur.p * 32;
             o[0] = __builtin_fmaf(pq[0][0], kInvWS, b0.x);
-            o[NN] = __builtin_fmaf(pq[0][1], kInvWS, b0.y);
-            o[2 * NN] = __builtin_fmaf(pq[0][2], kInvWS, b0.z);
-            o[3 * NN] = __builtin_fmaf(pq[0][3], kInvWS, b0.w);
+            o[hs] = __builtin_fmaf(pq[0][1], kInvWS, b0.y);
+            o[2 * hs] = __builtin_fmaf(pq[0][2], kInvWS, b0.z);
+            o[3 * hs] = __builtin_fmaf(pq[0][3], kInvWS, b0.w);
 #pragma unroll
             for (int g = 1; g <= 4; ++g) {
                 const int t = g >> 2, rq = g & 3;
                 const float4 bq = ldg4(s_vec + 512, g, h);
-                *reinterpret_cast<float4*>(proj_pz_out + cur.p * 32 + 8 * (g - 1) + 4 * h) =
+                *reinterpret_cast<float4*>(pz + 8 * (g - 1) + 4 * h) =
                     make_float4(__builtin_fmaf(pq[t][4 * rq + 0], kInvWS, bq.x), __builtin_fmaf(pq[t][4 * rq + 1], kInvWS, bq.y),
                                 __builtin_fmaf(pq[t][4 * rq + 2], kInvWS, bq.z), __builtin_fmaf(pq[t][4 * rq + 3], kInvWS, bq.w));
             }
@@ -979,3 +980,28 @@
     return (int)hipGetLastError();
 }
 #endif
+
+#if S2S_PM_PART == 4
+extern "C" int s2s_edge_embed_classes_f16x3(const float* node_a2, const float* node_b2, const float* rel_table, const float* bin_table,
+                                             const void* weight_stream, const float* b2, const float* b3, const float* ln_gamma,
+                                             const float* ln_beta, float* table, int n_fixed, int n_rel, int n_bins, float ln_eps,
+                                             const float* proj_bias_cat64, int* range_words, void* stream) {
+    if (n_fixed < 1 || n_fixed > 2 || n_rel < 1 || n_bins < 1 || n_bins > 32) return (int)hipErrorInvalidValue;
+    const long long M = (long long)(n_fixed == 2 ? 4 : 1) * n_rel * (n_bins + 1);
+    if (M * s2s::kEeRecProj * 4 >= (1ll << 32) || (long long)n_rel * 512 >= (1ll << 32)) return (int)hipErrorInvalidValue;
+    const long long wg_tiles = (M + 127) / 128;
+    const int n_cu = cu_count();
+    const long long grid = wg_tiles < n_cu ? wg_tiles : n_cu;
+    if (proj_bias_cat64)
+        hipLaunchKernelGGL((edge_embed_f16_kernel<true, true>), dim3((unsigned)grid), dim3(256), 0, (hipStream_t)stream, node_a2, node_b2,
+                           rel_table, bin_table, (const float*)nullptr, (const long long*)nullptr, (const float*)nullptr,
+                           (const char*)weight_stream, b2, b3, ln_gamma, ln_beta, (const float*)nullptr, table, M, n_fixed, 0, n_rel, n_bins,
+                           ln_eps, 0, proj_bias_cat64, (float*)nullptr, (float*)nullptr, range_words);
+    else
+        hipLaunchKernelGGL((edge_embed_f16_kernel<false, true>), dim3((unsigned)grid), dim3(256), 0, (hipStream_t)stream, node_a2, node_b2,
+                           rel_table, bin_table, (const float*)nullptr, (const long long*)nullptr, (const float*)nullptr,
+                           (const char*)weight_stream, b2, b3, ln_gamma, ln_beta, (const float*)nullptr, table, M, n_fixed, 0, n_rel, n_bins,
+                           ln_eps, 0, (const float*)nullptr, (float*)nullptr, (float*)nullptr, range_words);
+    return (int)hipGetLastError();
+}
+#endif
diff --git a/str2str_amd/csrc/pair_mlp_f16_d.hip b/str2str_amd/csrc/pair_mlp_f16_d.hip
--- /dev/null
+++ b/str2str_amd/csrc/pair_mlp_f16_d.hip
@@ -0,0 +1,2 @@
+#define S2S_PM_PART 4
+#include "pair_mlp_f16.hip"
diff --git a/str2str_amd/models/net/denoising_ipa.py b/str2str_amd/models/net/denoising_ipa.py
--- a/str2str_amd/models/net/denoising_ipa.py
+++ b/str2str_amd/models/net/denoising_ipa.py
@@ -1,6 +1,7 @@
 from __future__ import annotations
 
 import math
+import os
 from functools import partial
 from typing import Optional
 
@@ -36,6 +37,7 @@
 
 class EmbeddingModule(nn.Module):
     launch_switches = ("arith", "node_arith")
+    launch_modes = ("ee_classes",)
 
     def __init__(self, init_embed_size: int, node_embed_size: int, edge_embed_size: int, num_bins: int = 22,
                  min_bin: float = 1e-5, max_bin: float = 20.0, self_conditioning: bool = True):
@@ -60,6 +62,10 @@
         self._wcache, self._w16cache, self._proj_cache, self._idx_cache, self._fixed_cache = (DerivedCache() for _ in range(5))
         self.arith = default_arith()
         self.node_arith = default_arith()
+        self.ee_classes = os.environ.get("S2S_EE_CLASSES", "auto")
+        if self.ee_classes not in ("auto", "0", "1"):
+            raise ValueError(f"S2S_EE_CLASSES={self.ee_classes!r}: expected auto, 0 or 1")
+        self._mask01_cache = DerivedCache()
 
     def _weights(self):
         e0, e2, e4 = self.edge_embed[0], self.edge_embed[2], self.edge_embed[4]
@@ -99,10 +105,24 @@
         def build():
             fixed = fixed_mask.to(dev)[..., None].float()
             B, L = fixed.shape[:2]
+            vals = torch.unique(fixed).cpu().tolist()
+            cls = None
+            if vals and all(v in (0.0, 1.0) for v in vals):
+                f2 = torch.tensor(vals, device=dev, dtype=torch.float32).view(1, -1, 1)
+                cls = {"n_fixed": len(vals),
+                       "fixed_cls": ((fixed[..., 0] > 0) if len(vals) == 2 else torch.zeros_like(fixed[..., 0])).to(torch.int32).contiguous(),
+                       "fa2": (f2 * w["w_row_f"]).contiguous(),
+                       "fb2": (f2[:, None] * w["w_col_f"].view(1, 32, 1, 4)).expand(1, 32, len(vals), 4).contiguous(),
+                       "nc2": torch.zeros(len(vals), w["wn_f"].shape[0], device=dev)}
             return ((fixed * w["wn_f"] + node_pos).contiguous(), (fixed * w["w_row_f"]).contiguous(),
-                    ((fixed[:, None] * w["w_col_f"].view(1, 32, 1, 4)).expand(B, 32, L, 4).contiguous(), (fixed * w["w_col_f"]).contiguous()))
+                    ((fixed[:, None] * w["w_col_f"].view(1, 32, 1, 4)).expand(B, 32, L, 4).contiguous(), (fixed * w["w_col_f"]).contiguous()), cls)
 
         return self._fixed_cache.get([fixed_mask, w["wn_f"], node_pos], build)
+
+    def _mask_is_01(self, node_mask: Optional[torch.Tensor]) -> bool:
+        if node_mask is None:
+            return True
+        return self._mask01_cache.get([node_mask], lambda: (bool(((node_mask == 0) | (node_mask == 1)).all()),))[0]
 
     def time_images(self, t_emb: torch.Tensor) -> torch.Tensor:
         w = self._weights()
@@ -151,10 +171,11 @@
         single_t = t_img is not None or t_emb.shape[0] == 1
         M = B * L
         f16 = self.arith == "f16x3"
+        cls = None
         if single_t:
             per_sample = t_img is not None and t_img.ndim == 2 and t_img.shape[0] == B and B > 1
             img = (t_img if per_sample else t_img.reshape(-1)) if t_img is not None else (w["w_t_cat"] * t_emb).sum(-1) + w["b_t_cat"]
-            Fn, Fa, Fb = self._fixed_terms(fixed_mask, w, dev, node_pos)
+            Fn, Fa, Fb, cls = self._fixed_terms(fixed_mask, w, dev, node_pos)
             h_act, node_a, node_b = torch.ops.str2str_amd.embed_assemble(img.contiguous(), Fn, Fa, Fb[0] if f16 else Fb[1], B, L,
                                                                          self.node_arith == "f16x3", f16)
         else:
@@ -181,9 +202,19 @@
             if next_proj is not None:
                 stream = self._proj_cache.get([ws, next_proj["wp_f16x2"]], lambda: torch.cat([ws, next_proj["wp_f16x2"]]))
                 proj = (stream, next_proj["b64"])
-            edge_embed = ops.edge_embed_f16x3(node_a, node_b, rel_cb, w["bin_tab_cb"], w["bin_lower"], idx_dev, ca, ws, e2.bias,
-                                              w["b3c"], ln.weight, ln.bias, mask, span, ln.eps, proj=proj, column_blocked_tables=True,
-                                              out_layout=edge_layout)
+            by_class = cls is not None and ops.edge_embed_classes_eligible(
+                self.ee_classes, self.arith, single_t and not per_sample, cls["n_fixed"], self._mask_is_01(node_mask), rel_cb.shape[1],
+                w["bin_tab_cb"].shape[1], B, L)
+            if by_class:
+                _, node_a2, node_b2 = torch.ops.str2str_amd.embed_assemble(img.contiguous(), cls["nc2"], cls["fa2"], cls["fb2"], 1,
+                                                                           cls["n_fixed"], False, True)
+                edge_embed = ops.edge_embed_classes_f16x3(node_a2, node_b2, cls["fixed_cls"], rel_cb, w["bin_tab_cb"], w["bin_lower"], idx_dev,
+                                                          ca, ws, e2.bias, w["b3c"], ln.weight, ln.bias, mask, span, ln.eps, proj=proj,
+                                                          out_layout=edge_layout)
+            else:
+                edge_embed = ops.edge_embed_f16x3(node_a, node_b, rel_cb, w["bin_tab_cb"], w["bin_lower"], idx_dev, ca, ws, e2.bias,
+                                                  w["b3c"], ln.weight, ln.bias, mask, span, ln.eps, proj=proj, column_blocked_tables=True,
+                                                  out_layout=edge_layout)
         else:
             if edge_layout != "rowmajor":
                 raise ops.HipLibraryError("EmbeddingModule: the tiled pair layout belongs to the f16x3 kernels")
diff --git a/str2str_amd/ops/__init__.py b/str2str_amd/ops/__init__.py
--- a/str2str_amd/ops/__init__.py
+++ b/str2str_amd/ops/__init__.py
@@ -13,7 +13,8 @@
 from .packing import (NODE_TG, LazyDict, PairTiled, act_alloc, column_blocked, fragment_order, node_tiles, pack_f16x2_layer, pack_f16x3_embed_stream,
                       pack_f16x3_stream, pack_node_layer, pack_node_weight, pack_node_weight_f32, pack_weight, padded_len, pair_tiled,
                       pair_untiled, unpack_planes, vf_alloc, xp_alloc)
-from .pair import edge_embed, edge_embed_f16x3, edge_transition, edge_transition_f16x3, pair_project
+from .pair import (EE_CLASS_R, edge_embed, edge_embed_class_of_row, edge_embed_class_row, edge_embed_class_rows, edge_embed_classes_eligible,
+                   edge_embed_classes_f16x3, edge_embed_f16x3, edge_transition, edge_transition_f16x3, pair_project)
 from .range_guard import (RANGE_BITS, RANGE_FAMILIES, range_families, range_flag, range_flag_names, range_flag_read, range_flag_reset,
                           range_headroom)
 from .torch_ops import register_torch_ops
@@ -25,6 +26,7 @@
     "pack_f16x3_stream", "pack_node_layer", "pack_node_weight", "pack_node_weight_f32", "pack_weight", "padded_len", "pair_tiled", "pair_untiled",
     "unpack_planes", "vf_alloc", "xp_alloc",
     "edge_embed", "edge_embed_f16x3", "edge_transition", "edge_transition_f16x3", "pair_project",
+    "EE_CLASS_R", "edge_embed_class_of_row", "edge_embed_class_row", "edge_embed_class_rows", "edge_embed_classes_eligible", "edge_embed_classes_f16x3",
     "encoder_attention", "ipa_attention", "ipa_attention_f16", "ipa_prep_points", "ipa_prep_points_f16",
     "CHAIN_WIDTHS", "NARROW_MAX_WORK", "SMALL_ROWS", "embed_assemble", "ipa_projections", "node_apply",
     "node_apply_chain", "node_apply_multi", "node_chain", "node_linear", "node_linear_f32", "node_linear_multi", "node_linear_vfrag", "pack_planes",
diff --git a/str2str_amd/ops/binding.py b/str2str_amd/ops/binding.py
--- a/str2str_amd/ops/binding.py
+++ b/str2str_amd/ops/binding.py
@@ -18,6 +18,8 @@
     "s2s_edge_transition_f16x3": [_vp] * 9 + [_i, _i, _f, _i, _vp, _vp, _vp, _i, _vp, _vp],
     "s2s_edge_embed": [_vp] * 15 + [_i, _i, _i, _i, _i, _f, _vp, _vp, _vp, _vp, _vp],
     "s2s_edge_embed_f16x3": [_vp] * 14 + [_i, _i, _i, _i, _i, _f, _i, _vp, _vp, _vp, _vp, _vp],
+    "s2s_edge_embed_classes_f16x3": [_vp] * 10 + [_i, _i, _i, _f, _vp, _vp, _vp],
+    "s2s_edge_embed_expand": [_vp] * 8 + [_i, _vp, _vp, _i, _i, _i, _i, _i, _vp],
     "s2s_pair_project": [_vp] * 5 + [_i, _i, _vp],
     "s2s_ipa_prep_points": [_vp] * 6 + [_ll, _i, _i, _i, _i, _vp],
     "s2s_ipa_attention": [_vp] * 12 + [_i, _i, _i, _i, _i, _i, _i, _f, _f, _vp],
diff --git a/str2str_amd/ops/pair.py b/str2str_amd/ops/pair.py
--- a/str2str_amd/ops/pair.py
+++ b/str2str_amd/ops/pair.py
@@ -123,6 +123,76 @@
     return out if proj is None else (out, pbias, ppz)
 
 
+EE_CLASS_R = 12
+
+
+def edge_embed_class_rows(n_fixed: int, n_rel: int, n_bins: int) -> int:
+    if n_fixed not in (1, 2):
+        raise HipLibraryError(f"edge_embed classes: {n_fixed} fixed-mask values (a 0/1 mask has one or two)")
+    return (4 if n_fixed == 2 else 1) * n_rel * (n_bins + 1)
+
+
+def edge_embed_class_row(fa: int, fb: int, d: int, bin_: int, n_rel: int, n_bins: int) -> int:
+    return ((fa * 2 + fb) * n_rel + d) * (n_bins + 1) + (bin_ + 1)
+
+
+def edge_embed_class_of_row(r: int, n_rel: int, n_bins: int):
+    q, b1 = divmod(r, n_bins + 1)
+    c, d = divmod(q, n_rel)
+    return c >> 1, c & 1, d, b1 - 1
+
+
+def edge_embed_classes_eligible(mode: str, arith: str, one_timestep: bool, n_fixed, mask_is_01: bool, n_rel: int, n_bins: int,
+                                B: int, N: int, R: int = EE_CLASS_R) -> bool:
+    if mode not in ("auto", "0", "1"):
+        raise ValueError(f"S2S_EE_CLASSES={mode!r}: expected auto, 0 or 1")
+    if mode == "0" or arith != "f16x3" or not one_timestep or n_fixed not in (1, 2) or not mask_is_01:
+        return False
+    rows = edge_embed_class_rows(n_fixed, n_rel, n_bins)
+    if rows * 168 * 4 >= 2 ** 32:
+        return False
+    return mode == "1" or rows * R <= B * N * N
+
+
+def edge_embed_classes_f16x3(node_a2, node_b2, fixed_cls, rel_table, bin_table, bin_lower, residue_idx, ca, wstream, b2, b3, gamma, beta,
+                             mask, rel_offset: int, ln_eps=1e-5, out=None, proj=None, out_layout: str = "rowmajor"):
+    lib = load_library()
+    B, N = fixed_cls.shape
+    n_fixed, n_rel, n_bins = node_a2.numel() // 128, rel_table.shape[1], bin_table.shape[1]
+    if node_b2.numel() != n_fixed * 128 or rel_table.shape[0] != 32 or bin_table.shape[0] != 32:
+        raise HipLibraryError("edge_embed_classes_f16x3: operands are not [n_fixed,128] / column-blocked [32, rows, 4]")
+    rows = edge_embed_class_rows(n_fixed, n_rel, n_bins)
+    _req_all(node_a2=node_a2, node_b2=node_b2, rel_table=rel_table, bin_table=bin_table, bin_lower=bin_lower, ca=ca, b2=b2, b3=b3, gamma=gamma,
+             beta=beta)
+    _req(residue_idx, torch.int64, "residue_idx"); _req(fixed_cls, torch.int32, "fixed_cls")
+    if tuple(residue_idx.shape) != (B, N) or ca.numel() != B * N * 3:
+        raise HipLibraryError("edge_embed_classes_f16x3: residue_idx / ca do not match fixed_cls [B, N]")
+    dev = node_a2.device
+    pw, pb, pbias, ppz = _proj_outputs(proj, B, N, dev, torch.int16, "wstream")
+    wstream = _req(wstream, torch.int16, "wstream") if proj is None else pw
+    if wstream.numel() * 2 != (5 if proj is not None else 4) * 32 * 1024:
+        raise HipLibraryError("s2s_edge_embed_classes_f16x3: weight stream has the wrong number of stages")
+    _req_opt(mask=mask)
+    if out_layout not in ("rowmajor", "tiled"):
+        raise HipLibraryError(f"edge_embed_classes_f16x3: out_layout {out_layout!r}")
+    tiled = out_layout == "tiled"
+    if out is None:
+        out = PairTiled(B, N, dev) if tiled else torch.empty(B, N, N, 128, device=dev, dtype=torch.float32)
+    elif isinstance(out, PairTiled) != tiled:
+        raise HipLibraryError("edge_embed_classes_f16x3: out does not have the requested layout")
+    table = torch.empty(rows, 168 if proj is not None else 128, device=dev, dtype=torch.float32)
+
+    def launch():
+        rc = lib.s2s_edge_embed_classes_f16x3(_p(node_a2), _p(node_b2), _p(rel_table), _p(bin_table), _p(wstream), _p(b2), _p(b3), _p(gamma),
+                                              _p(beta), _p(table), n_fixed, n_rel, n_bins, ln_eps, _p(pb), _p(range_flag()), _stream())
+        return rc or lib.s2s_edge_embed_expand(_p(table), _p(fixed_cls), _p(bin_lower), _p(residue_idx), _p(ca), _p(mask), _p(pb),
+                                               _p(out.buf if tiled else out), 1 if tiled else 0, _p(pbias), _p(ppz), B, N, int(rel_offset),
+                                               n_rel, n_bins, _stream())
+
+    _check(_timed("s2s_edge_embed", launch), "s2s_edge_embed_classes_f16x3 / s2s_edge_embed_expand")
+    return out if proj is None else (out, pbias, ppz)
+
+
 def pair_project(edge, wp, bias64, attn_bias=None, pair_z=None):
     lib = load_library()
     B, N = edge.shape[0], edge.shape[1]
diff --git a/str2str_amd/ops/torch_ops.py b/str2str_amd/ops/torch_ops.py
--- a/str2str_amd/ops/torch_ops.py
+++ b/str2str_amd/ops/torch_ops.py
@@ -6,7 +6,7 @@
 from .node import (embed_assemble, ipa_projections, node_chain, node_linear, node_linear_f32, node_linear_multi, node_linear_vfrag, pack_planes,
                    row_layernorm)
 from .packing import PairTiled
-from .pair import edge_embed, edge_embed_f16x3, edge_transition, edge_transition_f16x3, pair_project
+from .pair import edge_embed, edge_embed_classes_f16x3, edge_embed_f16x3, edge_transition, edge_transition_f16x3, pair_project
 
 _registered = False
 
@@ -55,6 +55,9 @@
     "edge_embed_f16x3(Tensor node_a, Tensor node_b, Tensor rel_table, Tensor bin_table, Tensor bin_lower, Tensor residue_idx, Tensor ca, "
     "Tensor wstream, Tensor b2, Tensor b3, Tensor gamma, Tensor beta, Tensor? mask, int rel_offset, float ln_eps) -> Tensor":
         lambda *a: edge_embed_f16x3(*a),
+    "edge_embed_classes_f16x3(Tensor node_a2, Tensor node_b2, Tensor fixed_cls, Tensor rel_table, Tensor bin_table, Tensor bin_lower, "
+    "Tensor residue_idx, Tensor ca, Tensor wstream, Tensor b2, Tensor b3, Tensor gamma, Tensor beta, Tensor? mask, int rel_offset, "
+    "float ln_eps) -> Tensor": lambda *a: edge_embed_classes_f16x3(*a),
     "pair_project(Tensor edge, Tensor wp, Tensor bias64) -> (Tensor, Tensor)": lambda *a: pair_project(*a),
     "ipa_prep_points(Tensor rigids7, Tensor q_pts_lin, Tensor kv_pts_lin, int n_heads=8, int n_qk=8, int n_v=12) -> (Tensor, Tensor, Tensor)":
         lambda *a: ipa_prep_points(*a),
diff --git a/str2str_amd/sampler.py b/str2str_amd/sampler.py
--- a/str2str_amd/sampler.py
+++ b/str2str_amd/sampler.py
@@ -85,7 +85,8 @@
         if k in ("rigids_t", "sc_ca_t", "t_img", "t") or not torch.is_tensor(v):
             continue
         h.update(k.encode()); h.update(str(tuple(v.shape)).encode()); h.update(v.detach().cpu().numpy().tobytes())
-    modes = tuple((type(m).__name__, a, getattr(m, a)) for m in net.modules() for a in getattr(type(m), "launch_switches", ()))
+    modes = tuple((type(m).__name__, a, getattr(m, a)) for m in net.modules()
+                  for a in getattr(type(m), "launch_switches", ()) + getattr(type(m), "launch_modes", ()))
     return (id(net), sum(p._version for p in net.parameters()), b, N, modes, h.hexdigest())
 
 
```

Result: faster. 31.63 conformations/s, median of 6 (+4.7%).
